# luoao-kddi/SCP

Measured on AMD Instinct MI355X. Metric: KITTI frames/sec encode (SCP-EHEM, level 16) + bpp match vs ref, higher is better.
Workload: dtype f32 (dense layers and attention as bf16x3 split on bf16 MFMA, feature kNN as f16x3 split on f16 MFMA, fp32 accumulate; position kNN / CDF in fp32); 1 GPU; SCP-EHEM KITTI-like synthetic 120k-pt frames, --spher --mullevel lidar_level=16 (BASELINE.json configs[2]), seeded random weights; nodes_per_frame=577403, windows_per_frame=100, frames_per_gpu=46, frames_in_flight=4, frames_per_launch_sequence=1, transform=host-numpy on a prefetch thread (strict identity: the reference's integers), parallelism=frame-sharded x1, rank_cores=256, rank_cores_pinned=False

## Files before the change

### include/scp.h

```cpp
#ifndef SCP_H
#define SCP_H
#include <stddef.h>
#include <stdint.h>

#ifdef __cplusplus
extern "C" {
#endif

#define SCP_API __attribute__((visibility("default")))

#define SCP_OK 0
#define SCP_EINVAL (-1)
#define SCP_ENOMEM (-2)
#define SCP_ESMALL (-3)
#define SCP_EHIP (-4)
#define SCP_ESTATE (-5)

#define SCP_MAX_DEPTH 21
#define SCP_MAX_SEGMENTS 62

#define SCP_ABI_VERSION 220
SCP_API int scp_version(void);
SCP_API int scp_last_hip_error(void);
SCP_API int scp_device_count(void);
// ... 279 lines not shown

enum { SCP_TIE_MEAN_NORMAL = 0, SCP_TIE_PLANE_ERROR = 1 };
SCP_API int scp_estimate_normals_f64(const double *xyz, int64_t n, double radius, int32_t max_nn, const double *view, double *normals,
                                     int32_t *count, int32_t *idx, void *stream);
SCP_API int scp_nn_tieset_f64(int32_t mode, const double *q, int64_t nq, const double *p, int64_t np, const double *dmin, const double *nrm,
                              double *out, void *stream);

#define SCP_DIST_MAX_RINGS 64
#define SCP_DIST_MAX_BINS 4096
#define SCP_DIST_MAX_POINTS (1ll << 30)
enum { SCP_DIST_FLAG_AXIS = 1, SCP_DIST_FLAG_GROUP_CLAMPED = 2, SCP_DIST_FLAG_NO_NEIGHBOUR = 4 };
typedef struct scp_dist_seg {
    int64_t rows, axis_rows;
    double sum_sq, sum_r2, sum_phi2, sum_theta2, sum_r, max_sq;
    int64_t hist[64];
} scp_dist_seg;
SCP_API int scp_nn_error_split_f64(const double *a, int64_t na, const double *b, int64_t nb, const double *view, const double *edges_sq,
                                   int32_t n_rings, const int32_t *group , int32_t n_groups, int32_t *idx_out, double *d2_out,
                                   double *comp_out , int32_t *bin_out, uint8_t *flag_out, void *stream);
SCP_API int scp_dist_segments_f64(const double *d2, const double *comp, const uint8_t *flag, const int64_t *order , int64_t n,
                                  const int64_t *seg_off, int32_t n_bins, scp_dist_seg *out, void *stream);

#define SCP_SHARE_MAX_NODES (1ll << 30)
typedef struct scp_share_seg {
    int64_t leaves;
    double ideal_bits, table_bits, max_ideal_bits;
} scp_share_seg;
SCP_API int64_t scp_rate_leaf_share_workspace_bytes(int64_t total_nodes, int32_t nseg);
SCP_API int scp_rate_leaf_share(const uint8_t *occ, const uint8_t *level, const int32_t *parent, int64_t total_nodes, const double *bits_ideal,
                                const double *bits_table, const int64_t *segs , int32_t nseg, int64_t total_leaves,
                                int64_t *leaves, double *cost_ideal, double *cost_table, void *workspace, int64_t workspace_bytes, void *stream);
SCP_API int scp_ring_bins_f64(const double *xyz, int64_t n, const double *view, const double *edges_sq, int32_t n_rings,
                              const int32_t *group , int32_t n_groups, int32_t *bin_out, uint8_t *flag_out , void *stream);
SCP_API int scp_share_segments_f64(const double *cost_ideal, const double *cost_table, const int64_t *order , int64_t n,
                                   const int64_t *seg_off, int32_t n_bins, scp_share_seg *out, void *stream);

SCP_API int64_t scp_rate_depth_share_workspace_bytes(int64_t total_nodes, int32_t nseg);
SCP_API int scp_rate_depth_share(const uint8_t *occ, const uint8_t *level, const int32_t *parent, int64_t total_nodes, const double *bits_ideal,
                                 const double *bits_table, const int64_t *segs , int32_t nseg, int64_t total_leaves,
                                 int32_t max_drop, int64_t *leaves, double *cost_ideal, double *cost_table, void *workspace,
                                 int64_t workspace_bytes, void *stream);
SCP_API int scp_share_segments_depth_f64(const double *cost_ideal, const double *cost_table, const int64_t *order , int64_t n,
                                         const int64_t *seg_off, int32_t n_bins, int32_t n_depths, int64_t plane_stride, scp_share_seg *out,
                                         void *stream);

SCP_API int scp_embed_gather(const uint8_t *ctx, const float *pos, const int64_t *inmap, int64_t n_tokens, const float *occ_enc,
                     const float *level_enc, const float *octant_enc, float *x, float *pos_out, int64_t *occ_self, int64_t rows,
                     void *stream);

SCP_API int scp_packed_plan_sizes(const int64_t *lengths, int32_t W, int64_t *rows_out);
SCP_API int scp_packed_plan(const int64_t *lengths, int32_t W, int64_t *tables_dev, void *const *outs, int32_t n_outs, void *stream);

SCP_API int scp_decode_expand(const int64_t *sym, const int64_t *cum, const int32_t *pos, const uint8_t *anc, const uint8_t *octant, int64_t n,
                              int32_t L, int32_t shift, int32_t lv_next, int32_t lv_clamp, int32_t polar, double mn, double den, int32_t *cpos,
                              uint8_t *canc, uint8_t *coct, uint8_t *cctx, float *cposn, uint8_t *occ8, void *stream);

typedef struct scp_expand_seg {
    int64_t first, count, cfirst, coded;
    int32_t L, shift, lv_next, lv_clamp, polar, reserved;
    double mn, den;
} scp_expand_seg;
SCP_API int scp_decode_expand_batch(const int64_t *sym, const int64_t *cum, const int32_t *pos, const uint8_t *anc, const uint8_t *octant,
                                    int64_t n, const scp_expand_seg *seg, int32_t S, int32_t cs, const int64_t *wbase, int32_t K, int64_t M,
                                    int64_t T, void *table_dev, int32_t *cpos, uint8_t *canc, uint8_t *coct, uint8_t *cctx, float *cposn,
                                    uint8_t *occ8, void *stream);

SCP_API int scp_swin_ln_linear(const float *x, int64_t ldx, const float *valid, const void *Whi, const void *Wlo, const float *bias,
                               const float *wbeta, float eps, float *out, int64_t ldo, int32_t M, int32_t N, void *stream);
SCP_API int scp_swin_post_attn(const void *Ohi, const void *Olo, int64_t ldo_in, const float *x, int64_t ldx, const void *W, const float *bp,
                               const float *b1, const float *b2, float eps, float *out, int64_t ldc, int32_t M, const int32_t *tile_list,
                               int32_t n_tiles, void *stream);
SCP_API int64_t scp_swin_post_attn_weight_bytes(void);
SCP_API double scp_gelu_prescale(void);

SCP_API int scp_swin_merge(const float *x, int64_t ldx, int64_t n_src, const int64_t *ia, const int64_t *ib, const void *W, const float *wbeta,
                           float eps, float *out, int64_t ldo, int32_t M, void *stream);

SCP_API int scp_geo_edge_mlps(const float *pos1, int64_t ld1, const float *pos2, int64_t ld2, const float *pos3, int64_t ld3, const void *W,
                              const float *bias, float *out, int64_t ldo, int32_t M, void *stream);
SCP_API int scp_mlp3_rows(const float *x, int64_t ldx, int64_t n_src, const int64_t *in_map, const void *W, const float *bias, float *out, int64_t ldo,
                          const int64_t *out_map, int32_t M, int32_t N, void *stream);

#define SCP_LDO_FRAG 0
SCP_API int scp_swin_kv_planes(const float *k, const float *v, int64_t ldkv, int64_t rows, void *khi, void *klo, void *vthi, void *vtlo, void *stream);
SCP_API int scp_swin_ln_qkv(const float *x, int64_t ldx, const float *valid, const void *Whi, const void *Wlo, const float *bias, const float *wbeta,
                            float eps, float *q, int64_t ldq, void *planes, int64_t Tp, int32_t M, int32_t N, void *stream);
SCP_API int scp_swin_attention_packed_planes(const float *q, const void *khi, const void *klo, const void *vthi, const void *vtlo,
                                             const float *bias_table, const int32_t *wtab, int32_t total_windows, int32_t shift, int32_t ldq,
                                             float *out, void *ohi, void *olo, int64_t ldo, const float *valid, void *stream);

#ifdef __cplusplus
}
#endif
#endif
```

### scp_amd/build.py

```python
import os
import subprocess
import sys

HERE = os.path.dirname(os.path.abspath(__file__))
CSRC = os.path.join(HERE, "csrc")
LIB = os.path.join(HERE, "libscp_hip.so")
SOURCES = ["api.cpp", "geom.hip", "sort_u64.hip", "cdf.hip", "rangecoder.cpp", "legacy_octree.cpp",
           "knn.hip", "edge.hip", "attn.hip", "octattn.hip", "octattn_f16.hip", "octattn_embed.hip", "octattn_rowinv.hip", "gemm.hip", "gemm_split.hip", "rowchain.hip", "lnlin2.hip", "fused.hip", "metrics.hip", "plan.hip", "normals.hip", "rate.hip", "distreport.hip", "ringrate.hip", "temper.hip", "ringlod.hip", "attr.hip", "color.hip", "ac_chunks.hip"]
HIPCC = os.environ.get("HIPCC", "/opt/rocm/bin/hipcc")
FLAGS = ["-O3", "--offload-arch=gfx950", "-fPIC", "-std=c++17", "-Wall", "-Wno-unused-function",
         "-Wno-unused-result", "-fvisibility=hidden", "-x", "hip"]


EXTRA = {"geom.hip": ["-ffp-contract=off"], "knn.hip": ["-ffp-contract=off"], "cdf.hip": ["-ffp-contract=off"],
         "edge.hip": ["-ffp-contract=off"], "metrics.hip": ["-ffp-contract=off"], "octattn_embed.hip": ["-ffp-contract=off"],
         "octattn_rowinv.hip": ["-ffp-contract=off"], "normals.hip": ["-ffp-contract=off"], "rate.hip": ["-ffp-contract=off"],
         "distreport.hip": ["-ffp-contract=off"], "ringrate.hip": ["-ffp-contract=off"], "temper.hip": ["-ffp-contract=off"]}
if os.environ.get("SCP_ATTN_DEFS"):
    EXTRA["attn.hip"] = os.environ["SCP_ATTN_DEFS"].split()
if os.environ.get("SCP_KNN_DEFS"):
    EXTRA["knn.hip"] = EXTRA["knn.hip"] + os.environ["SCP_KNN_DEFS"].split()
if os.environ.get("SCP_RC_DEFS"):
    EXTRA["rowchain.hip"] = os.environ["SCP_RC_DEFS"].split()
EXTRA["lnlin2.hip"] = EXTRA.get("rowchain.hip", [])


def _stale(target, deps):
    if not os.path.exists(target):
        return True
    t = os.path.getmtime(target)
    return any(os.path.getmtime(d) > t for d in deps)


def build(force=False, verbose=False):
    srcs = [os.path.join(CSRC, s) for s in SOURCES if os.path.exists(os.path.join(CSRC, s))]
    hdrs = [os.path.join(CSRC, f) for f in os.listdir(CSRC) if f.endswith(".h")] + [os.path.join(HERE, "..", "include", "scp.h")]
    objs = []
    os.makedirs(os.path.join(CSRC, "build"), exist_ok=True)
    procs = []
    for s in srcs:
        o = os.path.join(CSRC, "build", os.path.basename(s) + ".o")
        objs.append(o)
        cmd = [HIPCC] + FLAGS + EXTRA.get(os.path.basename(s), []) + ["-c", s, "-o", o]
        stamp, line = o + ".cmd", " ".join(cmd)
        same_cmd = os.path.exists(stamp) and open(stamp).read() == line
        if force or not same_cmd or _stale(o, [s] + hdrs):
            for stale in (stamp, o):
                if os.path.exists(stale):
                    os.remove(stale)
            if verbose:
                print(" ".join(cmd), file=sys.stderr)
            procs.append((s, subprocess.Popen(cmd), stamp, line))
    bad = []
    for s, p, stamp, line in procs:
        if p.wait() != 0:
            bad.append(s)
            continue
        with open(stamp, "w") as f:
            f.write(line)
    if bad:
        raise RuntimeError("hipcc failed for: " + ", ".join(bad))
    if force or procs or _stale(LIB, objs):
        cmd = [HIPCC, "--offload-arch=gfx950", "-shared", "-fPIC", "-o", LIB] + objs
        if verbose:
            print(" ".join(cmd), file=sys.stderr)
        subprocess.check_call(cmd)
    return LIB


if __name__ == "__main__":
    print(build(force="--force" in sys.argv, verbose=True))
```

### scp_amd/csrc/lnlin2.hip

```cpp
#include <stdlib.h>
#include <type_traits>
#include "rc_common.h"

#define L2_Q 16384
#define L2_OFF_BOUNCE (3 * L2_Q)
#define L2_OFF_BIAS (L2_OFF_BOUNCE + 4 * RC_BOUNCE)
#define L2_LDS (L2_OFF_BIAS + 8192)
static_assert(L2_LDS <= 80 * 1024, "two workgroups per CU: at most half of the 160 KiB");
#define L2_LDS_ONE (160 * 1024)

__device__ __forceinline__ void l2_issue(const RcLane &L, __amdgpu_buffer_rsrc_t wr_hi, __amdgpu_buffer_rsrc_t wr_lo, int j, int qt, char *dst) {
#pragma unroll
    for (int i = 0; i < 4; ++i) {
        const int b = i >> 1, plane = i & 1;
        const int soff = ((2 * j + b) * 16 + (L.w >> 1) * 8 + qt * 2 + (L.w & 1)) * 1024;
        __builtin_amdgcn_raw_ptr_buffer_load_lds(plane ? wr_lo : wr_hi, (rc_lds_ptr_t)(dst + (L.w + 4 * i) * 1024), 16, L.lane * 16, soff, 0, 0);
    }
}

#define L2_READ4(d0, d1, d2, d3, addr, o0, o1, o2, o3)                                                                                  \
    asm volatile("ds_read_b128 %0, %4 offset:%5\n\tds_read_b128 %1, %4 offset:%6\n\tds_read_b128 %2, %4 offset:%7\n\t"                      \
                 "ds_read_b128 %3, %4 offset:%8\n\ts_waitcnt lgkmcnt(0)"                                                                  \
                 : "=&v"(d0), "=&v"(d1), "=&v"(d2), "=&v"(d3) : "v"(addr), "n"(o0), "n"(o1), "n"(o2), "n"(o3) : "memory")
#define L2_READ4_AHEAD(d0, d1, d2, d3, addr, o0, o1, o2, o3)                                                                            \
    asm volatile("ds_read_b128 %0, %4 offset:%5\n\tds_read_b128 %1, %4 offset:%6\n\tds_read_b128 %2, %4 offset:%7\n\t"                      \
                 "ds_read_b128 %3, %4 offset:%8"                                                                                         \
                 : "=&v"(d0), "=&v"(d1), "=&v"(d2), "=&v"(d3) : "v"(addr), "n"(o0), "n"(o1), "n"(o2), "n"(o3) : "memory")
#define L2_WAIT4(d0, d1, d2, d3) asm volatile("s_waitcnt lgkmcnt(0)" : "+v"(d0), "+v"(d1), "+v"(d2), "+v"(d3) :: "memory")
#define L2_TOP(N) asm volatile("s_waitcnt vmcnt(" #N ") lgkmcnt(0)\n\ts_barrier" ::: "memory")

template <bool SWAP, int Q>
__device__ __forceinline__ void l2_quarter(unsigned ad0, unsigned ad1, rf32x16 &c0, rf32x16 &c1, const rbf16x8 (&Xh)[16], const rbf16x8 (&Xl)[16]) {
#define L2_MFMA(c, wf, xf) c = SWAP ? __builtin_amdgcn_mfma_f32_32x32x16_bf16(xf, wf, c, 0, 0, 0) : __builtin_amdgcn_mfma_f32_32x32x16_bf16(wf, xf, c, 0, 0, 0)
#define L2_FRAGS(M, A, ad, s) M(A[1], A[3], A[0], A[2], ad, 4096 + ((s) >> 1) * 1024, 12288 + ((s) >> 1) * 1024, ((s) >> 1) * 1024, 8192 + ((s) >> 1) * 1024)
    rbf16x8 A[2][4];
    L2_FRAGS(L2_READ4, A[0], ad0, 0);
#pragma unroll
    for (int s = 0; s < 4; ++s) {
        const int k = 4 * Q + s, n = (s + 1) & 1;
        if (s < 3) {
            if (n) L2_FRAGS(L2_READ4_AHEAD, A[1], ad1, s + 1);
            else L2_FRAGS(L2_READ4_AHEAD, A[0], ad0, s + 1);
        }
        __builtin_amdgcn_sched_barrier(0);
        L2_MFMA(c0, A[s & 1][1], Xh[k]);
        L2_MFMA(c1, A[s & 1][3], Xh[k]);
        L2_MFMA(c0, A[s & 1][0], Xl[k]);
        L2_MFMA(c1, A[s & 1][2], Xl[k]);
        L2_MFMA(c0, A[s & 1][0], Xh[k]);
        L2_MFMA(c1, A[s & 1][2], Xh[k]);
        __builtin_amdgcn_sched_barrier(0);
        if (s < 3) L2_WAIT4(A[n][0], A[n][1], A[n][2], A[n][3]);
    }
#undef L2_FRAGS
#undef L2_MFMA
}

__device__ __forceinline__ unsigned l2_split_pair(float x0, float x1, int plane) {
    const unsigned hh = rc_pack2(x0, x1);
    return plane ? rc_pack2(x0 - __builtin_bit_cast(float, hh << 16), x1 - __builtin_bit_cast(float, hh & 0xffff0000u)) : hh;
}

__device__ __forceinline__ void l2_store_k(const RcLane &L, char *bounce, const rf32x16 &c0, const rf32x16 &c1, __amdgpu_buffer_rsrc_t prs, int kvoff,
                                           int pbytes, int head) {
    ri32x4 y[2][4];
    int col = L.col;
    asm volatile("" : "+v"(col));
#pragma unroll
    for (int plane = 0; plane < 2; ++plane) {
#pragma unroll
        for (int b = 0; b < 2; ++b)
#pragma unroll
            for (int q = 0; q < 4; ++q) {
                const rf32x16 &c = b ? c1 : c0;
                *(ru32x2 *)(bounce + col * 128 + (((4 * b + q) ^ (col & 7)) << 4) + 8 * L.h) =
                    (ru32x2){l2_split_pair(c[4 * q], c[4 * q + 1], plane), l2_split_pair(c[4 * q + 2], c[4 * q + 3], plane)};
            }
#pragma unroll
        for (int it = 0; it < 4; ++it) y[plane][it] = *(const ri32x4 *)(bounce + it * 1024 + L.lane * 16);
    }
#pragma unroll
    for (int plane = 0; plane < 2; ++plane)
#pragma unroll
        for (int it = 0; it < 4; ++it)
            __builtin_amdgcn_raw_buffer_store_b128(y[plane][it], prs, kvoff, it * 8 * 512 + head * 128 + plane * pbytes, 0);
    asm volatile("s_waitcnt lgkmcnt(0)" ::: "memory");
}

__device__ __forceinline__ void l2_store_v(const RcLane &L, char *bounce, const rf32x16 &c0, const rf32x16 &c1, __amdgpu_buffer_rsrc_t prs, int vblk,
                                           int pbytes, int head) {
    ri32x4 y[2][4];
    int col = L.col;
    asm volatile("" : "+v"(col));
#pragma unroll
    for (int plane = 0; plane < 2; ++plane) {
#pragma unroll
        for (int b = 0; b < 2; ++b)
#pragma unroll
            for (int cc = 0; cc < 2; ++cc) {
                const rf32x16 &c = b ? c1 : c0;
                const int d = col + 32 * b, R = d >> 1, sl = (d & 1) * 4 + 2 * cc + L.h;
                *(ru32x4 *)(bounce + R * 128 + ((sl ^ (R & 7)) << 4)) =
                    (ru32x4){l2_split_pair(c[8 * cc], c[8 * cc + 1], plane), l2_split_pair(c[8 * cc + 2], c[8 * cc + 3], plane),
                             l2_split_pair(c[8 * cc + 4], c[8 * cc + 5], plane), l2_split_pair(c[8 * cc + 6], c[8 * cc + 7], plane)};
            }
#pragma unroll
        for (int it = 0; it < 4; ++it) y[plane][it] = *(const ri32x4 *)(bounce + it * 1024 + L.lane * 16);
    }
#pragma unroll
    for (int plane = 0; plane < 2; ++plane)
#pragma unroll
        for (int it = 0; it < 4; ++it)
            __builtin_amdgcn_raw_buffer_store_b128(y[plane][it], prs, L.lane * 16, it * 1024 + (vblk + head) * 4096 + (2 + plane) * pbytes, 0);
    asm volatile("s_waitcnt lgkmcnt(0)" ::: "memory");
}

template <bool KV>
__global__ __launch_bounds__(256, 2) void ln2_proj_kernel(const RcLnLinArgs a) {
    extern __shared__ __attribute__((aligned(1024))) char smem[];
    const RcLane L = rc_lane();
    const int ntiles = (a.M + RC_ROWS - 1) / RC_ROWS;
    const int nsteps = a.N >> 6;
    const int nq = KV ? a.nq : nsteps;
    char *bounce = smem + L2_OFF_BOUNCE + L.w * RC_BOUNCE;
    const unsigned ab = (unsigned)(uintptr_t)(rc_lds_ptr_t)smem + L.rg * 2048;
    const unsigned af0 = ab + L.frag, af1 = ab + (L.frag ^ 32);
    const unsigned asb = (unsigned)(uintptr_t)(rc_lds_ptr_t)(smem + L2_OFF_BIAS);
    const int ldo_bytes = (int)(a.ldo * 4);
    const int voff = (32 * L.w + (L.lane >> 3)) * ldo_bytes + (L.lane & 7) * 16;
    const int pbytes = (int)a.plane_bytes;
    const __amdgpu_buffer_rsrc_t prs = __builtin_amdgcn_make_buffer_rsrc((void *)a.planes, 0, (KV && !(a.probe & 1)) ? (int)(4 * a.plane_bytes) : 0, 0x00020000);
    const bool dma = !(a.probe & 2);

    const int wbytes = ((a.N + 255) & ~255) * 512;
    const __amdgpu_buffer_rsrc_t wr_hi = __builtin_amdgcn_make_buffer_rsrc((void *)a.Whi, 0, wbytes, 0x00020000);
    const __amdgpu_buffer_rsrc_t wr_lo = __builtin_amdgcn_make_buffer_rsrc((void *)a.Wlo, 0, wbytes, 0x00020000);

    float *sb = (float *)(smem + L2_OFF_BIAS), *sbw = sb + 1024;
    for (int i = threadIdx.x; i < a.N; i += 256) {
        const float b = a.bias ? a.bias[i] : 0.f;
        sb[i] = b; sbw[i] = b + (a.wbeta ? a.wbeta[i] : 0.f);
    }
    __syncthreads();
    int slot = 0;
    if (dma) { l2_issue(L, wr_hi, wr_lo, 0, 0, smem); l2_issue(L, wr_hi, wr_lo, 0, 1, smem + L2_Q); }
    for (int tile = blockIdx.x; tile < ntiles; tile += (int)gridDim.x) {
        const int m0 = tile * RC_ROWS;
        const int row = m0 + 32 * L.w + L.col;
        const int rowc = row < a.M ? row : a.M - 1;
        float keep = (row < a.M) ? 1.0f : 0.0f;
        if (a.valid) keep *= a.valid[rowc];
        rbf16x8 Xh[16], Xl[16];
        {
            float v[128];
            const float *src = a.x + (int64_t)((a.probe & 4) ? (rowc & 127) % a.M : rowc) * a.ldx + 8 * L.h;
#pragma unroll
            for (int s = 0; s < 16; ++s) {
                const rf32x4 q0 = *(const rf32x4 *)(src + 16 * s), q1 = *(const rf32x4 *)(src + 16 * s + 4);
#pragma unroll
                for (int u = 0; u < 4; ++u) { v[8 * s + u] = q0[u]; v[8 * s + 4 + u] = q1[u]; }
            }
            float mean, rstd;
            rc_ln_stats(v, a.eps, mean, rstd);
            const float sc = rstd * keep;
#pragma unroll
            for (int s = 0; s < 16; ++s) {
                float f[8];
#pragma unroll
                for (int i = 0; i < 8; ++i) f[i] = (v[8 * s + i] - mean) * sc;
                rc_split8(f, Xh[s], Xl[s]);
            }
        }
        const bool kept = keep != 0.f;
        const int64_t rows_left = (int64_t)a.M - m0;
        const int64_t span = (rows_left < RC_ROWS ? rows_left : RC_ROWS) * a.ldo * 4;
        const __amdgpu_buffer_rsrc_t rs = __builtin_amdgcn_make_buffer_rsrc(a.out + (int64_t)m0 * a.ldo, 0, (a.probe & 1) ? 0 : (int)span, 0x00020000);
        const unsigned kmask = (unsigned)__builtin_amdgcn_ballot_w64(kept);
        const unsigned maskh = kmask >> (4 * L.h);
        const int kvoff = (m0 + 32 * L.w + (L.lane >> 3)) * 512 + (L.lane & 7) * 16;
        const int vblk = ((m0 >> 5) + L.w) * 4;

        const unsigned atb = asb + (kept ? 4096 : 0) + 16 * L.h, atv = asb + 4 * L.col;
        rf32x16 c0, c1;
        auto bias_start = [&](int j) {
            if (KV && j >= nq + 4) {
                float bb[2], bwv[2];
                const unsigned ad = atv + 256 * j;
                asm volatile("ds_read_b32 %0, %4\n\tds_read_b32 %1, %4 offset:128\n\tds_read_b32 %2, %4 offset:4096\n\tds_read_b32 %3, %4 offset:4224\n\t"
                             "s_waitcnt lgkmcnt(0)" : "=&v"(bb[0]), "=&v"(bb[1]), "=&v"(bwv[0]), "=&v"(bwv[1]) : "v"(ad) : "memory");
#pragma unroll
                for (int blk = 0; blk < 2; ++blk) {
                    rf32x16 &c = blk ? c1 : c0;
#pragma unroll
                    for (int r = 0; r < 16; ++r) c[r] = ((maskh >> (8 * (r >> 2) + (r & 3))) & 1u) ? bwv[blk] : bb[blk];
                }
            } else {
                const unsigned ad = atb + 256 * j;
                rf32x4 t[2][4];
                L2_READ4(t[0][0], t[0][1], t[0][2], t[0][3], ad, 0, 32, 64, 96);
                L2_READ4(t[1][0], t[1][1], t[1][2], t[1][3], ad, 128, 160, 192, 224);
#pragma unroll
                for (int q = 0; q < 4; ++q)
#pragma unroll
                    for (int u = 0; u < 4; ++u) { c0[4 * q + u] = t[0][q][u]; c1[4 * q + u] = t[1][q][u]; }
            }
        };
        bias_start(0);
        SCP_WAIT_DMA(0);
        auto steps = [&](auto sw, int ja, int jb) {
        constexpr bool SW = decltype(sw)::value;
        for (int j = ja; j < jb; ++j) {
            const int jn = j + 1 < nsteps ? j + 1 : 0;
#define L2_QUARTER(Q, N)                                                                                                                \
            {                                                                                                                           \
                L2_TOP(N);                                                                                                              \
                const int sl2 = slot == 0 ? 2 : slot - 1;                    \
                if (dma) l2_issue(L, wr_hi, wr_lo, Q < 2 ? j : jn, (Q + 2) & 3, smem + sl2 * L2_Q);                                       \
                __builtin_amdgcn_sched_barrier(0);                                                                                      \
                const unsigned a0 = af0 + slot * L2_Q, a1 = af1 + slot * L2_Q;                                                          \
                l2_quarter<SW, Q>(a0, a1, c0, c1, Xh, Xl);                                                                              \
                slot = slot == 2 ? 0 : slot + 1;                                                                                        \
            }
            L2_QUARTER(0, 12)
            L2_QUARTER(1, 12)
            L2_QUARTER(2, 4)
            L2_QUARTER(3, 4)
#undef L2_QUARTER
            __builtin_amdgcn_sched_barrier(0);
            if (!SW && j < nq) {
#pragma unroll
                for (int blk = 0; blk < 2; ++blk) {
                    rf32x4 o[4];
#pragma unroll
                    for (int q = 0; q < 4; ++q)
#pragma unroll
                        for (int u = 0; u < 4; ++u) o[q][u] = (blk ? c1 : c0)[4 * q + u];
                    rc_store_block(L, bounce, o, rs, ldo_bytes, voff, 64 * j + 32 * blk);
                }
            } else if (!SW) {
                l2_store_k(L, bounce, c0, c1, prs, kvoff, pbytes, j - nq);
            } else {
                l2_store_v(L, bounce, c0, c1, prs, vblk, pbytes, j - nq - 4);
            }
            if (j + 1 < nsteps) bias_start(jn);
        }
        };
        if (KV) { steps(std::false_type(), 0, nq + 4); steps(std::true_type(), nq + 4, nsteps); }
        else steps(std::false_type(), 0, nsteps);
    }
    SCP_WAIT_DMA(0);
}

int scp_lnlin2_mode() {
    static int mode = -1;
    if (mode < 0) { const char *e = getenv("SCP_LNLIN"); mode = e ? atoi(e) : 0; if (mode < 0 || mode > 2) mode = 0; }
    return mode;
}

int scp_lnlin2_launch(RcLnLinArgs a, bool kv, int ncu, hipStream_t stream) {
    static int one = -1, probe = -1;
    if (one < 0) { const char *e = getenv("SCP_LNLIN_ONE"); one = (e && e[0] == '1') ? 1 : 0; }
    if (probe < 0) { const char *e = getenv("SCP_RC_PROBE"); probe = e ? atoi(e) : 0; }
    static bool configured = false;
    if (!configured) {
        HIP_TRY(hipFuncSetAttribute((const void *)ln2_proj_kernel<false>, hipFuncAttributeMaxDynamicSharedMemorySize, one ? L2_LDS_ONE : L2_LDS));
        HIP_TRY(hipFuncSetAttribute((const void *)ln2_proj_kernel<true>, hipFuncAttributeMaxDynamicSharedMemorySize, one ? L2_LDS_ONE : L2_LDS));
        configured = true;
    }
    a.ngroups = 1; a.probe = probe; a.dbg = nullptr;
    const int ntiles = (a.M + RC_ROWS - 1) / RC_ROWS;
    const int wgs = (one ? 1 : 2) * ncu;
    const dim3 grid((unsigned)(ntiles < wgs ? ntiles : wgs));
    if (kv) hipLaunchKernelGGL(ln2_proj_kernel<true>, grid, dim3(256), one ? L2_LDS_ONE : L2_LDS, stream, a);
    else hipLaunchKernelGGL(ln2_proj_kernel<false>, grid, dim3(256), one ? L2_LDS_ONE : L2_LDS, stream, a);
    LAUNCH_CHECK();
    return SCP_OK;
}
```

### scp_amd/csrc/rc_common.h

```cpp
#pragma once
#include "scp_internal.h"

typedef __bf16 rbf16x8 __attribute__((ext_vector_type(8)));
typedef float rf32x16 __attribute__((ext_vector_type(16)));
typedef float rf32x4 __attribute__((ext_vector_type(4)));
typedef int ri32x4 __attribute__((ext_vector_type(4)));
typedef __attribute__((address_space(3))) void *rc_lds_ptr_t;
typedef const __attribute__((address_space(1))) void *rc_glb_ptr_t;

#define RC_ROWS 128
#define RC_BOUNCE 4096

__device__ __forceinline__ void rc_dma16(const void *g, char *l) {
    __builtin_amdgcn_global_load_lds((rc_glb_ptr_t)g, (rc_lds_ptr_t)l, 16, 0, 0);
}

typedef float rf32x2 __attribute__((ext_vector_type(2)));
typedef __bf16 rbf16x2 __attribute__((ext_vector_type(2)));
typedef unsigned ru32x4 __attribute__((ext_vector_type(4)));
typedef unsigned ru32x2 __attribute__((ext_vector_type(2)));
__device__ __forceinline__ unsigned rc_pack2(float a, float b) {
    const rf32x2 v = {a, b};
    return __builtin_bit_cast(unsigned, __builtin_convertvector(v, rbf16x2));
}
__device__ __forceinline__ void rc_split2(float a, float b, unsigned &hi, unsigned &lo) {
    asm volatile("" : "+v"(a), "+v"(b));
    hi = rc_pack2(a, b);
    lo = rc_pack2(a - __builtin_bit_cast(float, hi << 16), b - __builtin_bit_cast(float, hi & 0xffff0000u));
}
__device__ __forceinline__ void rc_split8(const float *f, rbf16x8 &hi, rbf16x8 &lo) {
    ru32x4 h, l;
#pragma unroll
    for (int i = 0; i < 4; ++i) { unsigned a, b; rc_split2(f[2 * i], f[2 * i + 1], a, b); h[i] = a; l[i] = b; }
    hi = __builtin_bit_cast(rbf16x8, h);
    lo = __builtin_bit_cast(rbf16x8, l);
}

struct RcLane {
    int lane, col, h, w;
    int frag;
    int rg;
};

__device__ __forceinline__ RcLane rc_lane() {
    RcLane L;
    const int tid = threadIdx.x;
    L.lane = tid & 63; L.col = L.lane & 31; L.h = L.lane >> 5;
    L.w = __builtin_amdgcn_readfirstlane(tid >> 6);
    L.frag = (L.col & 15) * 64 + ((L.h ^ ((L.col >> 2) & 3)) << 4);
    L.rg = L.col >> 4;
    return L;
}

__device__ __forceinline__ void rc_store_block(const RcLane &L, char *bounce, const rf32x4 v[4], __amdgpu_buffer_rsrc_t rs, int ldo_bytes, int voff,
                                               int ch0) {
#pragma unroll
    for (int q = 0; q < 4; ++q)
        *(rf32x4 *)(bounce + L.col * 128 + (((2 * q + L.h) ^ (L.col & 7)) << 4)) = v[q];
    asm volatile("s_waitcnt lgkmcnt(0)" ::: "memory");
    rf32x4 y[4];
#pragma unroll
    for (int it = 0; it < 4; ++it) {
        const int rho = 8 * it + (L.lane >> 3), kap = L.lane & 7;
        y[it] = *(const rf32x4 *)(bounce + rho * 128 + ((kap ^ (rho & 7)) << 4));
    }
#pragma unroll
    for (int it = 0; it < 4; ++it) __builtin_amdgcn_raw_buffer_store_b128(__builtin_bit_cast(ri32x4, y[it]), rs, voff, it * 8 * ldo_bytes + ch0 * 4, 0);
    asm volatile("s_waitcnt lgkmcnt(0)" ::: "memory");
}

__device__ __forceinline__ void rc_ln_stats(const float *v , float eps, float &mean, float &rstd) {
    float s = 0.f;
#pragma unroll
    for (int i = 0; i < 128; i += 4) s += (v[i] + v[i + 1]) + (v[i + 2] + v[i + 3]);
    s += __shfl_xor(s, 32);
    mean = s * (1.0f / 256.0f);
    float q = 0.f;
#pragma unroll
    for (int i = 0; i < 128; ++i) { const float d = v[i] - mean; q += d * d; }
    q += __shfl_xor(q, 32);
    rstd = rsqrtf(q * (1.0f / 256.0f) + eps);
}

struct RcLnLinArgs {
    const float *x; int64_t ldx;
    const float *valid;
    const __bf16 *Whi, *Wlo;
    const float *bias, *wbeta;
    float *out; int64_t ldo;
    int M, N;
    float eps;
    int probe;
    unsigned long long *dbg;
    __bf16 *planes; int64_t plane_bytes; int nq;
    int ngroups;
};

int scp_lnlin2_mode();
int scp_lnlin2_launch(RcLnLinArgs a, bool kv, int ncu, hipStream_t stream);
```

### scp_amd/csrc/rowchain.hip

```cpp
#include <stdlib.h>
#include "scp_internal.h"
#include "rc_common.h"

#define RC_SLOT 32768
#define RC_RING (4 * RC_SLOT)
#define RC_OFF_BOUNCE RC_RING
#define RC_OFF_BIAS (RC_RING + 4 * RC_BOUNCE)
#define RC_LDS (RC_OFF_BIAS + 16384)

__device__ __forceinline__ void rc_issue_rowchunk(const RcLane &L, const __bf16 *Whi, const __bf16 *Wlo, int g, char *slot) {
#pragma unroll
    for (int j = 0; j < 4; ++j) {
        const int p = L.w + 4 * j;
        const int64_t off = ((int64_t)g * 16 + p) * 512 + L.lane * 8;
        rc_dma16(Whi + off, slot + p * 1024);
        rc_dma16(Wlo + off, slot + 16384 + p * 1024);
    }
}

__device__ __forceinline__ void rc_issue_kchunk(const RcLane &L, const __bf16 *Whi, const __bf16 *Wlo, int c, int nks, char *slot) {
#pragma unroll
    for (int j = 0; j < 4; ++j) {
        const int p = L.w + 4 * j;
        const int64_t off = ((int64_t)p * nks + c) * 512 + L.lane * 8;
// ... 498 lines not shown
    return;
#endif
    switch (st) {
    case 0: g.ea = -ya * ya; g.eb = -yb * yb; break;
    case 1: g.ea = __builtin_amdgcn_exp2f(g.ea); g.eb = __builtin_amdgcn_exp2f(g.eb); break;
    case 2: g.pa = fmaf(SCP_GELU_C4, __builtin_fabsf(ya), SCP_GELU_C3); g.pb = fmaf(SCP_GELU_C4, __builtin_fabsf(yb), SCP_GELU_C3); break;
    case 3: g.pa = fmaf(g.pa, __builtin_fabsf(ya), SCP_GELU_C2); g.pb = fmaf(g.pb, __builtin_fabsf(yb), SCP_GELU_C2); break;
    case 4: g.pa = fmaf(g.pa, __builtin_fabsf(ya), SCP_GELU_C1); g.pb = fmaf(g.pb, __builtin_fabsf(yb), SCP_GELU_C1); break;
    case 5: g.pa = fmaf(g.pa, __builtin_fabsf(ya), SCP_GELU_C0); g.pb = fmaf(g.pb, __builtin_fabsf(yb), SCP_GELU_C0); break;
    case 6: g.pa = __builtin_amdgcn_rcpf(g.pa); g.pb = __builtin_amdgcn_rcpf(g.pb); break;
    case 7: g.wa = __builtin_fabsf(ya) * g.ea; g.wb = __builtin_fabsf(yb) * g.eb; break;
    case 8: asm("v_max_f32_e32 %0, 0, %1" : "=v"(g.xa) : "v"(ya)); asm("v_max_f32_e32 %0, 0, %1" : "=v"(g.xb) : "v"(yb)); break;
    case 9: g.ga = fmaf(-g.wa, g.pa, g.xa); g.gb = fmaf(-g.wb, g.pb, g.xb); break;
    case 10: g.hw = rc_pack2(g.ga, g.gb); wh = g.hw; break;
    default: wl = rc_pack2(g.ga - __builtin_bit_cast(float, g.hw << 16), g.gb - __builtin_bit_cast(float, g.hw & 0xffff0000u)); break;
    }
    switch (st) {
    case 0: case 1: asm volatile("" : "+v"(g.ea), "+v"(g.eb)); break;
    case 2: case 3: case 4: case 5: case 6: asm volatile("" : "+v"(g.pa), "+v"(g.pb)); break;
    case 7: asm volatile("" : "+v"(g.wa), "+v"(g.wb)); break;
    case 8: asm volatile("" : "+v"(g.xa), "+v"(g.xb)); break;
    case 9: asm volatile("" : "+v"(g.ga), "+v"(g.gb)); break;
    case 10: asm volatile("" : "+v"(g.ga), "+v"(g.gb), "+v"(g.hw)); break;
    default: break;
    }
}

template <bool HAS_P1, bool HAS_GELU, int NEXT>
__device__ __forceinline__ void rc_body_step(const RcLane &L, char *smem, int half, rf32x16 (&Y)[8], rf32x16 &a1n, const rf32x16 &a1g,
                                             const ru32x4 (&Hch)[2], const ru32x4 (&Hcl)[2], ru32x4 (&Hnh)[2],
                                             ru32x4 (&Hnl)[2], const rbf16x8 (&Xh)[16], const rbf16x8 (&Xl)[16], rbf16x8 (&A)[2][4],
                                             __amdgpu_buffer_rsrc_t wr, const RcSlotSrc &n0, const RcSlotSrc &n1) {
    const RcFragAddr f = rc_frag_addr(L, smem + half * (2 * RC_SLOT)), fn = rc_frag_addr(L, smem + (half ^ 1) * (2 * RC_SLOT));
    char *nxt = smem + (half ^ 1) * (2 * RC_SLOT);
    RcGelu g;
#pragma unroll
    for (int s = 0; s < 16; ++s) {
        if (s == 15) RC_STEP_BARRIER("vmcnt(0) lgkmcnt(0)", L.w);
        RC_SB;
        const int nb = (s + 1) & 1, ns = (s + 1) & 15;
        const int blk = s >> 1, t = s & 1;
#pragma unroll
        for (int gap = 0; gap < 6; ++gap) {
            if (HAS_P1 && gap < 4 && RC_PROBE_FRAG_ON) { RC_FRAG_WAIT(); RC_SB; }
            if (!HAS_P1 && (gap == 1 || gap == 3) && RC_PROBE_FRAG_ON) { asm volatile("s_waitcnt lgkmcnt(1)" ::: "memory"); RC_SB; }
            if (gap == 0 && HAS_P1) RC_MFMA_AVA(a1n, A[s & 1][1], Xh[s]);
            if (gap == 1) RC_MFMA_AVV(Y[blk], A[s & 1][3], Hch[t]);
            if (gap == 2 && HAS_P1) RC_MFMA_AVV(a1n, A[s & 1][0], Xl[s]);
            if (gap == 3) RC_MFMA_AVV(Y[blk], A[s & 1][2], Hcl[t]);
            if (gap == 4 && HAS_P1) RC_MFMA_AVA(a1n, A[s & 1][0], Xh[s]);
            if (gap == 5) RC_MFMA_AVV(Y[blk], A[s & 1][2], Hch[t]);
            RC_SB;
            if (s < 15 && RC_PROBE_FRAG_ON) {
                if (gap == 0 && HAS_P1) RC_DS_READ(A[nb][1], (ns & 1) ? f.r1 : f.r0, 16384 + (ns >> 1) * 1024);
                if (gap == 1) RC_DS_READ(A[nb][3], (ns & 1) ? f.k1 : f.k0, RC_SLOT + 16384 + (ns >> 1) * 2048);
                if (gap == 2 && HAS_P1) RC_DS_READ(A[nb][0], (ns & 1) ? f.r1 : f.r0, (ns >> 1) * 1024);
                if (gap == 3) RC_DS_READ(A[nb][2], (ns & 1) ? f.k1 : f.k0, RC_SLOT + (ns >> 1) * 2048);
            }
            if (RC_DMA_HERE(s, gap) && RC_PROBE_DMA_ON) rc_dma_piece(L, wr, RC_DMA_SLOT(s, gap) ? n1 : n0, nxt + RC_DMA_SLOT(s, gap) * RC_SLOT, RC_DMA_IDX(s, gap), RC_DMA_PLANE(s, gap));
            if (HAS_GELU) {
                const int k = s >> 1, st = (s & 1) * 6 + gap;
                unsigned wh = 0, wl = 0;
                rc_gelu_stage(st, g, a1g[2 * k], a1g[2 * k + 1], wh, wl);
                if (st == 10) Hnh[k >> 2][k & 3] = wh;
                if (st == 11) Hnl[k >> 2][k & 3] = wl;
            }
            RC_SB;
        }
    }
    if (NEXT == 0) RC_DS_READ4_WAIT(A[0][1], fn.r0, 16384, A[0][3], fn.k0, RC_SLOT + 16384, A[0][0], fn.r0, 0, A[0][2], fn.k0, RC_SLOT);
    else RC_DS_READ4_WAIT(A[0][1], fn.r0, 16384, A[0][3], fn.r0, RC_SLOT + 16384, A[0][0], fn.r0, 0, A[0][2], fn.r0, RC_SLOT);
}

__device__ __forceinline__ void rc_load_o_frag(const __bf16 *Ohi, const __bf16 *Olo, int tile, int r, int h, rbf16x8 (&Bh)[16], rbf16x8 (&Bl)[16]) {
    const __amdgpu_buffer_rsrc_t rh = __builtin_amdgcn_make_buffer_rsrc((void *)(Ohi + (int64_t)tile * (RC_ROWS * 256)), 0, RC_ROWS * 512, 0x00020000);
    const __amdgpu_buffer_rsrc_t rl = __builtin_amdgcn_make_buffer_rsrc((void *)(Olo + (int64_t)tile * (RC_ROWS * 256)), 0, RC_ROWS * 512, 0x00020000);
    const int v = (r & (RC_ROWS - 1)) * 16 + h * 2048;
#pragma unroll
    for (int s = 0; s < 16; ++s) Bh[s] = __builtin_bit_cast(rbf16x8, __builtin_amdgcn_raw_buffer_load_b128(rh, v, 4096 * s, 0));
#pragma unroll
    for (int s = 0; s < 16; ++s) Bl[s] = __builtin_bit_cast(rbf16x8, __builtin_amdgcn_raw_buffer_load_b128(rl, v, 4096 * s, 0));
}

template <bool OFRAG>
__global__ __launch_bounds__(256, 1) void rc_post_attn_kernel(const RcPostArgs a) {
    extern __shared__ __attribute__((aligned(1024))) char smem[];
    const RcLane L = rc_lane();
    const int ntiles = (a.M + RC_ROWS - 1) / RC_ROWS;
    float *sbp = (float *)(smem + RC_OFF_BIAS), *sb2 = sbp + 256, *sb1 = sbp + 512;
    for (int i = threadIdx.x; i < 256; i += 256) { sbp[i] = a.bp[i]; sb2[i] = a.b2[i]; }
    for (int i = threadIdx.x; i < 1024; i += 256) sb1[i] = a.b1[i];
    __syncthreads();
    const int nlist = a.tile_list ? a.n_list : ntiles;
    auto tile_of = [&](int i) { return a.tile_list ? a.tile_list[i] : i; };
    int ti = blockIdx.x;
    if (ti >= nlist) return;
    int tile = tile_of(ti);
    char *bounce = smem + RC_OFF_BOUNCE + L.w * RC_BOUNCE;
    const int ldc_bytes = (int)(a.ldc * 4);
    const int voff = (32 * L.w + (L.lane >> 3)) * ldc_bytes + (L.lane & 7) * 16;

    const __amdgpu_buffer_rsrc_t wr = __builtin_amdgcn_make_buffer_rsrc((void *)a.W, 0, 2 * RC_W_PLANE, 0x00020000);
    auto src_p = [&](int g) { RcSlotSrc r = {RC_W_PROJ + g * 16384, 1024}; return r; };
    auto src_1 = [&](int c) { RcSlotSrc r = {RC_W_FC1 + c * 16384, 1024}; return r; };
    auto src_2 = [&](int c) { RcSlotSrc r = {RC_W_FC2 + c * 1024, 32 * 1024}; return r; };

    unsigned long long t_p0 = 0, t_ln = 0, t_mlp = 0, t_epi = 0, t_prev = 0, n_tiles = 0;
    const bool DBG = a.dbg != nullptr;
    unsigned long long t_first = 0, r_first = 0;
    if (DBG) { t_prev = t_first = __builtin_amdgcn_s_memtime(); r_first = __builtin_amdgcn_s_memrealtime(); }
    auto stamp = [&](unsigned long long &acc_t) { if (DBG) { const unsigned long long t = __builtin_amdgcn_s_memtime(); acc_t += t - t_prev; t_prev = t; } };

    {
        const RcSlotSrc s0 = src_p(0), s1 = src_p(1);
#pragma unroll
        for (int q = 0; q < 4; ++q)
#pragma unroll
            for (int plane = 0; plane < 2; ++plane) { rc_dma_piece(L, wr, s0, smem, q, plane); rc_dma_piece(L, wr, s1, smem + RC_SLOT, q, plane); }
    }
    rbf16x8 Bh[16], Bl[16];
    auto load_o = [&](int t) {
        if (OFRAG) {
            const int r = t * RC_ROWS + 32 * L.w + L.col;
            rc_load_o_frag(a.Ohi, a.Olo, t, r < a.M ? r : a.M - 1, L.h, Bh, Bl);
            return;
        }
        const int r0 = t * RC_ROWS + 32 * L.w + (L.lane >> 3);
#pragma unroll
        for (int it = 0; it < 4; ++it) {
            const int r = r0 + 8 * it;
            const int64_t o = (int64_t)(r < a.M ? r : a.M - 1) * a.ldo_in + (L.lane & 7) * 8;
#pragma unroll
            for (int pp = 0; pp < 4; ++pp) { Bh[4 * pp + it] = *(const rbf16x8 *)(a.Ohi + o + 64 * pp); Bl[4 * pp + it] = *(const rbf16x8 *)(a.Olo + o + 64 * pp); }
        }
    };
    auto transpose_o = [&]() {
        if (OFRAG) {
#pragma unroll
            for (int s = 0; s < 16; ++s) asm volatile("" : "+v"(Bh[s]), "+v"(Bl[s]));
            return;
        }
#pragma unroll
        for (int plane = 0; plane < 2; ++plane)
#pragma unroll
            for (int pp = 0; pp < 4; ++pp) {
#pragma unroll
                for (int it = 0; it < 4; ++it) {
                    const int rho = 8 * it + (L.lane >> 3), kap = L.lane & 7;
                    *(rbf16x8 *)(bounce + rho * 128 + ((kap ^ (rho & 7)) << 4)) = plane ? Bl[4 * pp + it] : Bh[4 * pp + it];
                }
                asm volatile("s_waitcnt lgkmcnt(0)" ::: "memory");
#pragma unroll
                for (int q = 0; q < 4; ++q) {
                    const rbf16x8 fr = *(const rbf16x8 *)(bounce + L.col * 128 + (((2 * q + L.h) ^ (L.col & 7)) << 4));
                    if (plane) Bl[4 * pp + q] = fr; else Bh[4 * pp + q] = fr;
                }
                asm volatile("s_waitcnt lgkmcnt(0)" ::: "memory");
            }
    };
    load_o(tile);
    transpose_o();
    rbf16x8 A[2][4];
    {
        SCP_BARRIER_DMA(0);
        const RcFragAddr f = rc_frag_addr(L, smem);
        RC_DS_READ4_WAIT(A[0][1], f.r0, 16384, A[0][3], f.r0, RC_SLOT + 16384, A[0][0], f.r0, 0, A[0][2], f.r0, RC_SLOT);
    }
    int gstep = 0;
    for (; ti < nlist; ti += gridDim.x) {
        tile = tile_of(ti);
        const int m0 = tile * RC_ROWS;
        const bool more = ti + (int)gridDim.x < nlist;
        const int tile_next = more ? tile_of(ti + (int)gridDim.x) : tile;
        rf32x16 Y[8];
        const int xrow = m0 + 32 * L.w + (L.lane >> 3);
        const float *xsrc = a.x + (L.lane & 7) * 4;
        for (int j = 0; j < 4; ++j) {
            rf32x4 xc[2][4];
#pragma unroll
            for (int b = 0; b < 2; ++b)
#pragma unroll
                for (int it = 0; it < 4; ++it) {
                    const int r = xrow + 8 * it;
                    xc[b][it] = *(const rf32x4 *)(xsrc + (int64_t)(r < a.M ? r : a.M - 1) * a.ldx + 64 * j + 32 * b);
                }
            rf32x16 c0, c1;
#pragma unroll
            for (int r = 0; r < 16; ++r) { c0[r] = 0.f; c1[r] = 0.f; }
            rc_gemm_step<false>(L, smem, gstep & 1, c0, c1, Bh, Bl, A, wr, j < 3 ? src_p(2 * j + 2) : src_1(0), j < 3 ? src_p(2 * j + 3) : src_1(1));
            ++gstep;
#pragma unroll
            for (int b = 0; b < 2; ++b) {
#pragma unroll
                for (int it = 0; it < 4; ++it) {
                    const int rho = 8 * it + (L.lane >> 3), kap = L.lane & 7;
                    *(rf32x4 *)(bounce + rho * 128 + ((kap ^ (rho & 7)) << 4)) = xc[b][it];
                }
                asm volatile("s_waitcnt lgkmcnt(0)" ::: "memory");
#pragma unroll
                for (int q = 0; q < 4; ++q) {
                    const rf32x4 xq = *(const rf32x4 *)(bounce + L.col * 128 + (((2 * q + L.h) ^ (L.col & 7)) << 4));
                    const rf32x4 bq = *(const rf32x4 *)(sbp + 64 * j + 32 * b + 8 * q + 4 * L.h);
#pragma unroll
                    for (int u = 0; u < 4; ++u) {
                        if (b == 0) c0[4 * q + u] += xq[u] + bq[u];
                        else c1[4 * q + u] += xq[u] + bq[u];
                    }
                }
                asm volatile("s_waitcnt lgkmcnt(0)" ::: "memory");
            }
            asm volatile("s_waitcnt lgkmcnt(0)" ::: "memory");
            switch (j) {
            case 0: Y[0] = c0; Y[1] = c1; break;
            case 1: Y[2] = c0; Y[3] = c1; break;
            case 2: Y[4] = c0; Y[5] = c1; break;
            default: Y[6] = c0; Y[7] = c1; break;
            }
        }
        stamp(t_p0);
        float sum = 0.f;
#pragma unroll
        for (int b = 0; b < 8; ++b)
#pragma unroll
            for (int r = 0; r < 16; r += 4) sum += (Y[b][r] + Y[b][r + 1]) + (Y[b][r + 2] + Y[b][r + 3]);
        sum += __shfl_xor(sum, 32);
        const float mean = sum * (1.0f / 256.0f);
        float sq = 0.f;
#pragma unroll
        for (int b = 0; b < 8; ++b)
#pragma unroll
            for (int r = 0; r < 16; ++r) { const float d = Y[b][r] - mean; sq += d * d; }
        sq += __shfl_xor(sq, 32);
        const float rstd = rsqrtf(sq * (1.0f / 256.0f) + a.eps);
#pragma unroll
        for (int b = 0; b < 8; ++b) {
#pragma unroll
            for (int t = 0; t < 2; ++t) {
                float fr[8];
#pragma unroll
                for (int i = 0; i < 8; ++i) fr[i] = (Y[b][8 * t + i] - mean) * rstd;
                rc_split8(fr, Bh[2 * b + t], Bl[2 * b + t]);
            }
#pragma unroll
            for (int q = 0; q < 4; ++q) {
                const rf32x4 bb = *(const rf32x4 *)(sb2 + 32 * b + 8 * q + 4 * L.h);
#pragma unroll
                for (int u = 0; u < 4; ++u) Y[b][4 * q + u] += bb[u];
            }
        }
        asm volatile("s_waitcnt lgkmcnt(0)" ::: "memory");
        stamp(t_ln);
        if (a.dbg_mode) {
#pragma unroll
            for (int b = 0; b < 8; ++b)
#pragma unroll
                for (int r = 0; r < 16; ++r) {
                    const int t = r >> 3, i = r & 7;
                    Y[b][r] = (a.dbg_mode == 1) ? (float)Bh[2 * b + t][i] + (float)Bl[2 * b + t][i] : (r == 0 ? mean : rstd);
                }
        }
        rf32x16 a1[2];
        auto bias_into = [&](rf32x16 &acc, int c) {
#pragma unroll
            for (int q = 0; q < 4; ++q) {
                const rf32x4 bq = *(const rf32x4 *)(sb1 + 32 * c + 8 * q + 4 * L.h);
#pragma unroll
                for (int u = 0; u < 4; ++u) acc[4 * q + u] = bq[u];
            }
        };
        bias_into(a1[0], 0);
        bias_into(a1[1], 1);
        asm volatile("s_waitcnt lgkmcnt(0)" ::: "memory");
        if (!a.dbg_mode) {
        rc_gemm_step<true>(L, smem, gstep & 1, a1[0], a1[1], Bh, Bl, A, wr, src_1(2), src_2(0)); ++gstep;
        ru32x4 Hh[1][2], Hl[1][2];
        {
            RcGelu g;
#pragma unroll
            for (int k = 0; k < 8; ++k)
#pragma unroll
                for (int st = 0; st < 12; ++st)
                {
                    unsigned wh = 0, wl = 0;
                    rc_gelu_stage(st, g, a1[0][2 * k], a1[0][2 * k + 1], wh, wl);
                    if (st == 10) Hh[0][k >> 2][k & 3] = wh;
                    if (st == 11) Hl[0][k >> 2][k & 3] = wl;
                }
        }
        ru32x4 Hnh[2], Hnl[2];
        for (int c = 0; c < 30; ++c) {
            rf32x16 a1n;
            bias_into(a1n, c + 2);
            asm volatile("s_waitcnt lgkmcnt(0)" ::: "memory");
            rc_body_step<true, true, 0>(L, smem, gstep & 1, Y, a1n, a1[1], Hh[0], Hl[0], Hnh, Hnl, Bh, Bl, A, wr,
                                        c + 3 < 32 ? src_1(c + 3) : src_2(c + 1), src_2(c + 1));
            ++gstep;
            a1[1] = a1n;
#pragma unroll
            for (int t = 0; t < 2; ++t) { Hh[0][t] = Hnh[t]; Hl[0][t] = Hnl[t]; }
        }
        load_o(tile_next);
        rc_body_step<false, true, 0>(L, smem, gstep & 1, Y, a1[0], a1[1], Hh[0], Hl[0], Hnh, Hnl, Bh, Bl, A, wr, src_2(31), src_2(31));
        ++gstep;
        rc_body_step<false, false, 1>(L, smem, gstep & 1, Y, a1[0], a1[1], Hnh, Hnl, Hh[0], Hl[0], Bh, Bl, A, wr, src_p(0), src_p(1));
        ++gstep;
        }
        stamp(t_mlp);
        asm volatile("s_waitcnt lgkmcnt(0)" ::: "memory");
        const int64_t rows_left = (int64_t)a.M - m0;
        const int64_t span = (rows_left < RC_ROWS ? rows_left : RC_ROWS) * a.ldc * 4;
#ifdef RC_EPI_NOSTORE
        const __amdgpu_buffer_rsrc_t rs = __builtin_amdgcn_make_buffer_rsrc(a.out, 0, 0, 0x00020000);
#else
        const __amdgpu_buffer_rsrc_t rs = __builtin_amdgcn_make_buffer_rsrc(a.out + (int64_t)m0 * a.ldc, 0, (int)span, 0x00020000);
#endif
#pragma unroll
        for (int b = 0; b < 8; ++b) {
            rf32x4 o[4];
#pragma unroll
            for (int q = 0; q < 4; ++q)
#pragma unroll
                for (int u = 0; u < 4; ++u) o[q][u] = Y[b][4 * q + u];
            rc_store_block(L, bounce, o, rs, ldc_bytes, voff, 32 * b);
        }
        transpose_o();
        stamp(t_epi);
        ++n_tiles;
    }
    if (DBG && L.lane == 0) {
        unsigned long long *o = a.dbg + ((size_t)blockIdx.x * 4 + L.w) * 8;
        o[0] = t_p0; o[1] = t_mlp; o[2] = t_ln; o[3] = t_epi; o[4] = n_tiles;
        o[5] = __builtin_amdgcn_s_memtime() - t_first; o[6] = __builtin_amdgcn_s_memrealtime() - r_first;
    }
    SCP_WAIT_DMA(0);
}

#ifndef RCW_D1
#define RCW_D1 4
#endif
#ifndef RCW_D2
#define RCW_D2 2
#endif
#define RCW_H_BYTES (32 * 4096)
template <bool OFRAG>
__global__ __launch_bounds__(256, 1) void rc_post_attn_wide_kernel(const RcPostArgs a) {
    extern __shared__ __attribute__((aligned(1024))) char smem[];
    const RcLane L = rc_lane();
    float *sbp = (float *)(smem + RC_OFF_BIAS), *sb2 = sbp + 256, *sb1 = sbp + 512;
    for (int i = threadIdx.x; i < 256; i += 256) { sbp[i] = a.bp[i]; sb2[i] = a.b2[i]; }
    for (int i = threadIdx.x; i < 1024; i += 256) sb1[i] = a.b1[i];
    __syncthreads();
    const int n128 = a.tile_list ? a.n_list : (a.M + RC_ROWS - 1) / RC_ROWS;
    char *bounce = smem + RC_OFF_BOUNCE + L.w * RC_BOUNCE;
    char *hbuf = smem;
    const int ldc_bytes = (int)(a.ldc * 4);
    const int voff = (L.lane >> 3) * ldc_bytes + (L.lane & 7) * 16;
    const __amdgpu_buffer_rsrc_t wr = __builtin_amdgcn_make_buffer_rsrc((void *)a.W, 0, 2 * RC_W_PLANE, 0x00020000);
    const int vrc0 = L.rg * 8192 + L.frag, vrc1 = L.rg * 8192 + (L.frag ^ 32);
    const int vkc0 = L.rg * 32768 + L.frag, vkc1 = L.rg * 32768 + (L.frag ^ 32);
    auto wload = [&](int voff, int soff) { return __builtin_bit_cast(rbf16x8, __builtin_amdgcn_raw_buffer_load_b128(wr, voff, soff, 0)); };
    for (int item = blockIdx.x; item < 4 * n128; item += gridDim.x) {
        const int t128 = a.tile_list ? a.tile_list[item >> 2] : (item >> 2);
        const int m0 = t128 * RC_ROWS + 32 * (item & 3);
        if (m0 >= a.M) continue;
        rbf16x8 Bh[16], Bl[16];
        if (OFRAG) {
            const int r = m0 + L.col;
            rc_load_o_frag(a.Ohi, a.Olo, t128, r < a.M ? r : a.M - 1, L.h, Bh, Bl);
        } else {
            const int r0 = m0 + (L.lane >> 3);
#pragma unroll
            for (int it = 0; it < 4; ++it) {
                const int r = r0 + 8 * it;
                const int64_t o = (int64_t)(r < a.M ? r : a.M - 1) * a.ldo_in + (L.lane & 7) * 8;
#pragma unroll
                for (int pp = 0; pp < 4; ++pp) { Bh[4 * pp + it] = *(const rbf16x8 *)(a.Ohi + o + 64 * pp); Bl[4 * pp + it] = *(const rbf16x8 *)(a.Olo + o + 64 * pp); }
            }
#pragma unroll
            for (int plane = 0; plane < 2; ++plane)
#pragma unroll
                for (int pp = 0; pp < 4; ++pp) {
#pragma unroll
                    for (int it = 0; it < 4; ++it) {
                        const int rho = 8 * it + (L.lane >> 3), kap = L.lane & 7;
                        *(rbf16x8 *)(bounce + rho * 128 + ((kap ^ (rho & 7)) << 4)) = plane ? Bl[4 * pp + it] : Bh[4 * pp + it];
                    }
                    asm volatile("s_waitcnt lgkmcnt(0)" ::: "memory");
#pragma unroll
                    for (int q = 0; q < 4; ++q) {
                        const rbf16x8 fr = *(const rbf16x8 *)(bounce + L.col * 128 + (((2 * q + L.h) ^ (L.col & 7)) << 4));
                        if (plane) Bl[4 * pp + q] = fr; else Bh[4 * pp + q] = fr;
                    }
                    asm volatile("s_waitcnt lgkmcnt(0)" ::: "memory");
                }
        }
        rf32x16 c0, c1;
#pragma unroll
        for (int r = 0; r < 16; ++r) { c0[r] = 0.f; c1[r] = 0.f; }
        {
            const int w0 = RC_W_PROJ + (2 * L.w) * 16384, w1 = w0 + 16384;
            constexpr int D = RCW_D1;
            rbf16x8 F[D][4];
            auto fetch = [&](int s, rbf16x8 (&d)[4]) {
                const int v = (s & 1) ? vrc1 : vrc0, o = (s >> 1) * 1024;
                d[0] = wload(v, w0 + o); d[1] = wload(v, w0 + RC_W_PLANE + o);
                d[2] = wload(v, w1 + o); d[3] = wload(v, w1 + RC_W_PLANE + o);
// ... 501 lines not shown
        to_frags();
        RC_LAYER3(1)
        to_frags();
        const int kap = L.lane & 7;
        float *orow[4];
#pragma unroll
        for (int it = 0; it < 4; ++it) {
            const int r = m0 + 32 * L.w + 8 * it + (L.lane >> 3);
            const int64_t o = r < a.M ? (a.out_map ? a.out_map[r] : (int64_t)r) : -1;
            orow[it] = o >= 0 ? a.out + o * a.ldo + 4 * kap : nullptr;
        }
        auto store_block = [&](const rf32x16 &c, int ch0) {
#pragma unroll
            for (int q = 0; q < 4; ++q) {
                rf32x4 v;
#pragma unroll
                for (int u = 0; u < 4; ++u) v[u] = c[4 * q + u];
                *(rf32x4 *)(bounce + L.col * 128 + (((2 * q + L.h) ^ (L.col & 7)) << 4)) = v;
            }
            asm volatile("s_waitcnt lgkmcnt(0)" ::: "memory");
            rf32x4 y[4];
#pragma unroll
            for (int it = 0; it < 4; ++it) {
                const int rho = 8 * it + (L.lane >> 3);
                y[it] = *(const rf32x4 *)(bounce + rho * 128 + ((kap ^ (rho & 7)) << 4));
            }
            asm volatile("s_waitcnt lgkmcnt(0)" ::: "memory");
#pragma unroll
            for (int it = 0; it < 4; ++it)
                if (orow[it] && ch0 + 4 * kap < a.N) *(rf32x4 *)(orow[it] + ch0) = y[it];
        };
        for (int g = 0; g < 4; ++g) {
            RC_BIAS3(2)
            RC_STEP3()
            store_block(c0, 64 * g);
            store_block(c1, 64 * g + 32);
        }
#undef RC_LAYER3
#undef RC_BIAS3
#undef RC_STEP3
    }
    SCP_WAIT_DMA(0);
}

extern "C" SCP_API double scp_gelu_prescale(void) { return (double)SCP_GELU_S; }

static int rc_ll_groups(int ntiles, int nsteps, int ncu) {
    static int on = -1;
    if (on < 0) { const char *e = getenv("SCP_RC_GROUPS"); on = (e && e[0] == '0') ? 0 : 1; }
    int best = 1;
    if (on)
        for (int g = 2; g <= nsteps / 2; ++g)
            if ((nsteps / 2) % g == 0 && (int64_t)ntiles * g <= ncu) best = g;
    return best;
}

static unsigned long long *g_rc_dbg = nullptr;
extern "C" SCP_API int scp_rc_debug_buffer(unsigned long long *dev_buf) { g_rc_dbg = dev_buf; return SCP_OK; }

static int g_rc_num_cu = 0, g_rc_grid = 0;
static int g_rc_wide = -2;
static int rc_wide_mode() {
    if (g_rc_wide == -2) { const char *e = getenv("SCP_RC_WIDE"); g_rc_wide = e ? atoi(e) : -1; if (g_rc_wide < -1 || g_rc_wide > 1) g_rc_wide = -1; }
    return g_rc_wide;
}
extern "C" SCP_API int scp_rc_set_wide(int32_t mode) { g_rc_wide = (mode < -1 || mode > 1) ? -1 : mode; return SCP_OK; }
extern "C" SCP_API int scp_rc_set_grid(int32_t workgroups) { g_rc_grid = workgroups > 0 ? workgroups : 0; return SCP_OK; }
static int rc_num_cu() {
    if (g_rc_grid) return g_rc_grid;
    if (!g_rc_num_cu) {
        int dev = 0;
        hipDeviceProp_t p;
        if (hipGetDevice(&dev) != hipSuccess || hipGetDeviceProperties(&p, dev) != hipSuccess) return 256;
        g_rc_num_cu = p.multiProcessorCount > 0 ? p.multiProcessorCount : 256;
    }
    return g_rc_num_cu;
}

static bool rc_lnlin2_here(int ntiles, int ncu) {
    const int mode = scp_lnlin2_mode();
    return mode == 2 || (mode == 0 && 4 * (int64_t)ntiles >= 3 * (int64_t)ncu);
}

extern "C" SCP_API int scp_swin_ln_linear(const float *x, int64_t ldx, const float *valid, const void *Whi, const void *Wlo, const float *bias,
                                          const float *wbeta, float eps, float *out, int64_t ldo, int32_t M, int32_t N, void *stream) {
    if (!x || !Whi || !Wlo || !out || M <= 0 || N <= 0 || (N & 127) || N > 1024 || ldx < 256 || (ldx & 3) || ldo < N || (ldo & 3) ||
        (((uintptr_t)x | (uintptr_t)out | (uintptr_t)Whi | (uintptr_t)Wlo) & 15) || (int64_t)RC_ROWS * ldo * 4 > 0x7fffffffLL)
        return SCP_EINVAL;
    static bool configured = false;
    if (!configured) {
        HIP_TRY(hipFuncSetAttribute((const void *)rc_ln_linear_kernel<0>, hipFuncAttributeMaxDynamicSharedMemorySize, RC_LDS));
        configured = true;
    }
    RcLnLinArgs a;
    a.x = x; a.ldx = ldx; a.valid = valid; a.Whi = (const __bf16 *)Whi; a.Wlo = (const __bf16 *)Wlo; a.bias = bias; a.wbeta = wbeta;
    a.out = out; a.ldo = ldo; a.M = M; a.N = N; a.eps = eps;
    a.planes = nullptr; a.plane_bytes = 0; a.nq = 0;
    { static int pr = -1; if (pr < 0) { const char *e = getenv("SCP_RC_PROBE"); pr = e ? atoi(e) : 0; } a.probe = pr; }
    if (a.probe) { const char *e = getenv("SCP_RC_PROBE"); a.probe = e ? atoi(e) : 0; }
    a.dbg = g_rc_dbg;
    const int ntiles = (M + RC_ROWS - 1) / RC_ROWS;
    const int ncu = rc_num_cu();
    SCP_PROF(SCP_PROF_LN_LINEAR, stream, 2.0 * M * 256.0 * N);
    if (rc_lnlin2_here(ntiles, ncu)) return scp_lnlin2_launch(a, false, ncu, (hipStream_t)stream);
    a.ngroups = rc_ll_groups(ntiles, N / 64, ncu);
    hipLaunchKernelGGL(rc_ln_linear_kernel<0>, dim3((unsigned)(a.ngroups > 1 ? ntiles * a.ngroups : (ntiles < ncu ? ntiles : ncu))), dim3(256), RC_LDS, (hipStream_t)stream, a);
    LAUNCH_CHECK();
    return SCP_OK;
}

extern "C" SCP_API int scp_swin_ln_qkv(const float *x, int64_t ldx, const float *valid, const void *Whi, const void *Wlo, const float *bias,
                                       const float *wbeta, float eps, float *q, int64_t ldq, void *planes, int64_t Tp, int32_t M, int32_t N, void *stream) {
    if (!x || !Whi || !Wlo || !planes || M <= 0 || (M & 127) || (N != 768 && N != 512) || (N == 768 && (!q || ldq < 256 || (ldq & 3))) || ldx < 256 ||
        (ldx & 3) || Tp < M || (Tp & 31) || (((uintptr_t)x | (uintptr_t)q | (uintptr_t)Whi | (uintptr_t)Wlo | (uintptr_t)planes) & 15) ||
        (q && (int64_t)RC_ROWS * ldq * 4 > 0x7fffffffLL) || 4 * Tp * 512 > 0x7fffffffLL)
        return SCP_EINVAL;
    static bool configured = false;
    if (!configured) {
        HIP_TRY(hipFuncSetAttribute((const void *)rc_ln_linear_kernel<0, true>, hipFuncAttributeMaxDynamicSharedMemorySize, RC_LDS));
        configured = true;
    }
    RcLnLinArgs a;
    a.x = x; a.ldx = ldx; a.valid = valid; a.Whi = (const __bf16 *)Whi; a.Wlo = (const __bf16 *)Wlo; a.bias = bias; a.wbeta = wbeta;
    a.out = q; a.ldo = q ? ldq : 256; a.M = M; a.N = N; a.eps = eps; a.probe = 0; a.dbg = nullptr;
    a.planes = (__bf16 *)planes; a.plane_bytes = Tp * 512; a.nq = N / 64 - 8;
    const int ntiles = M / RC_ROWS, ncu = rc_num_cu();
    SCP_PROF(SCP_PROF_LN_LINEAR, stream, 2.0 * M * 256.0 * N);
    if (rc_lnlin2_here(ntiles, ncu)) return scp_lnlin2_launch(a, true, ncu, (hipStream_t)stream);
    a.ngroups = rc_ll_groups(ntiles, N / 64, ncu);
    hipLaunchKernelGGL((rc_ln_linear_kernel<0, true>), dim3((unsigned)(a.ngroups > 1 ? ntiles * a.ngroups : (ntiles < ncu ? ntiles : ncu))), dim3(256), RC_LDS, (hipStream_t)stream, a);
    LAUNCH_CHECK();
    return SCP_OK;
}

extern "C" SCP_API int scp_swin_post_attn(const void *Ohi, const void *Olo, int64_t ldo_in, const float *x, int64_t ldx, const void *W, const float *bp,
                                          const float *b1, const float *b2, float eps, float *out, int64_t ldc, int32_t M, const int32_t *tile_list,
                                          int32_t n_tiles, void *stream) {
    if (!Ohi || !Olo || !x || !W || !bp || !b1 || !b2 || !out || M <= 0 || (tile_list && (n_tiles <= 0 || n_tiles > (M + RC_ROWS - 1) / RC_ROWS)) || (ldo_in != SCP_LDO_FRAG && (ldo_in < 256 || (ldo_in & 7))) || ldx < 256 || (ldx & 3) || ldc < 256 ||
        (ldc & 3) || (((uintptr_t)Ohi | (uintptr_t)Olo | (uintptr_t)x | (uintptr_t)out | (uintptr_t)W) & 15) ||
        (int64_t)RC_ROWS * ldc * 4 > 0x7fffffffLL)
        return SCP_EINVAL;
    static bool configured = false;
    if (!configured) {
        HIP_TRY(hipFuncSetAttribute((const void *)rc_post_attn_kernel<true>, hipFuncAttributeMaxDynamicSharedMemorySize, RC_LDS));
        HIP_TRY(hipFuncSetAttribute((const void *)rc_post_attn_kernel<false>, hipFuncAttributeMaxDynamicSharedMemorySize, RC_LDS));
        HIP_TRY(hipFuncSetAttribute((const void *)rc_post_attn_wide_kernel<true>, hipFuncAttributeMaxDynamicSharedMemorySize, RC_LDS));
        HIP_TRY(hipFuncSetAttribute((const void *)rc_post_attn_wide_kernel<false>, hipFuncAttributeMaxDynamicSharedMemorySize, RC_LDS));
        configured = true;
    }
    RcPostArgs a;
    a.Ohi = (const __bf16 *)Ohi; a.Olo = (const __bf16 *)Olo; a.ldo_in = ldo_in; a.x = x; a.ldx = ldx; a.W = W;
    a.bp = bp; a.b1 = b1; a.b2 = b2; a.out = out; a.ldc = ldc; a.M = M; a.eps = eps;
    a.dbg = g_rc_dbg;
    { const char *e = getenv("SCP_RC_DUMP"); a.dbg_mode = e ? atoi(e) : 0; }
    a.tile_list = tile_list; a.n_list = tile_list ? n_tiles : 0;
    const bool frag = ldo_in == SCP_LDO_FRAG;
    const int ntiles = tile_list ? n_tiles : (M + RC_ROWS - 1) / RC_ROWS;
    const int ncu = rc_num_cu();
    SCP_PROF(SCP_PROF_POST_ATTN, stream, 2.0 * (tile_list ? (double)n_tiles * RC_ROWS : (double)M) * (256.0 * 256.0 + 2.0 * 256.0 * 1024.0));
    if (rc_wide_mode() == 1 || (rc_wide_mode() < 0 && !g_rc_dbg && !a.dbg_mode && 4 * (int64_t)ntiles <= (int64_t)ncu)) {
        const int items = 4 * ntiles;
        if (frag) hipLaunchKernelGGL(rc_post_attn_wide_kernel<true>, dim3((unsigned)(items < 2 * ncu ? items : 2 * ncu)), dim3(256), RC_LDS, (hipStream_t)stream, a);
        else hipLaunchKernelGGL(rc_post_attn_wide_kernel<false>, dim3((unsigned)(items < 2 * ncu ? items : 2 * ncu)), dim3(256), RC_LDS, (hipStream_t)stream, a);
        LAUNCH_CHECK();
        return SCP_OK;
    }
    if (frag) hipLaunchKernelGGL(rc_post_attn_kernel<true>, dim3((unsigned)(ntiles < ncu ? ntiles : ncu)), dim3(256), RC_LDS, (hipStream_t)stream, a);
    else hipLaunchKernelGGL(rc_post_attn_kernel<false>, dim3((unsigned)(ntiles < ncu ? ntiles : ncu)), dim3(256), RC_LDS, (hipStream_t)stream, a);
    LAUNCH_CHECK();
    return SCP_OK;
}

extern "C" SCP_API int64_t scp_swin_post_attn_weight_bytes(void) { return 2 * (int64_t)RC_W_PLANE; }

extern "C" SCP_API int scp_geo_edge_mlps(const float *pos1, int64_t ld1, const float *pos2, int64_t ld2, const float *pos3, int64_t ld3, const void *W,
                                         const float *bias, float *out, int64_t ldo, int32_t M, void *stream) {
    if (!pos1 || !pos2 || !pos3 || !W || !bias || !out || M <= 0 || ld1 < 64 || ld2 < 128 || ld3 < 256 || ((ld1 | ld2 | ld3) & 3) || ldo < 128 || (ldo & 3) ||
        (((uintptr_t)pos1 | (uintptr_t)pos2 | (uintptr_t)pos3 | (uintptr_t)out | (uintptr_t)W) & 15) || (int64_t)RC_ROWS * ldo * 4 > 0x7fffffffLL)
        return SCP_EINVAL;
    static bool configured = false;
    if (!configured) {
        HIP_TRY(hipFuncSetAttribute((const void *)rc_edge_mlp_kernel, hipFuncAttributeMaxDynamicSharedMemorySize, RC_LDS));
        configured = true;
    }
    RcEdgeArgs a;
    a.p1 = pos1; a.p2 = pos2; a.p3 = pos3; a.ld1 = ld1; a.ld2 = ld2; a.ld3 = ld3; a.W = W; a.bias = bias; a.out = out; a.ldo = ldo; a.M = M;
    const int ntiles = (M + RC_ROWS - 1) / RC_ROWS, ncu = rc_num_cu();
    SCP_PROF(SCP_PROF_EDGE_MLP, stream, 2.0 * M * (448.0 * 256 + 2.0 * 256 * 256 + 512.0 * 256 + 256.0 * 256 + 256.0 * 128));
    hipLaunchKernelGGL(rc_edge_mlp_kernel, dim3((unsigned)(ntiles < ncu ? ntiles : ncu)), dim3(256), RC_LDS, (hipStream_t)stream, a);
    LAUNCH_CHECK();
    return SCP_OK;
}

extern "C" SCP_API int scp_mlp3_rows(const float *x, int64_t ldx, int64_t n_src, const int64_t *in_map, const void *W, const float *bias, float *out, int64_t ldo,
                                     const int64_t *out_map, int32_t M, int32_t N, void *stream) {
    if (!x || !W || !bias || !out || M <= 0 || n_src <= 0 || N <= 0 || N > 256 || (N & 3) || ldx < 256 || (ldx & 3) || ldo < N || (ldo & 3) ||
        (((uintptr_t)x | (uintptr_t)out | (uintptr_t)W) & 15))
        return SCP_EINVAL;
    static bool configured = false;
    if (!configured) {
        HIP_TRY(hipFuncSetAttribute((const void *)rc_mlp3_kernel, hipFuncAttributeMaxDynamicSharedMemorySize, RC_LDS));
        configured = true;
    }
    RcMlp3Args a;
    a.x = x; a.ldx = ldx; a.in_map = in_map; a.n_src = n_src; a.W = W; a.bias = bias; a.out = out; a.ldo = ldo; a.out_map = out_map; a.M = M; a.N = N;
    const int ntiles = (M + RC_ROWS - 1) / RC_ROWS, ncu = rc_num_cu();
    SCP_PROF(SCP_PROF_MLP3, stream, 2.0 * M * 3.0 * 256.0 * 256.0);
    hipLaunchKernelGGL(rc_mlp3_kernel, dim3((unsigned)(ntiles < ncu ? ntiles : ncu)), dim3(256), RC_LDS, (hipStream_t)stream, a);
    LAUNCH_CHECK();
    return SCP_OK;
}

extern "C" SCP_API int scp_swin_merge(const float *x, int64_t ldx, int64_t n_src, const int64_t *ia, const int64_t *ib, const void *W, const float *wbeta,
                                      float eps, float *out, int64_t ldo, int32_t M, void *stream) {
    if (!x || !ia || !ib || !W || !out || M <= 0 || n_src <= 0 || ldx < 256 || (ldx & 3) || ldo < 256 || (ldo & 3) ||
        (((uintptr_t)x | (uintptr_t)out | (uintptr_t)W) & 15) || (int64_t)RC_ROWS * ldo * 4 > 0x7fffffffLL)
        return SCP_EINVAL;
    static bool configured = false;
    if (!configured) {
        HIP_TRY(hipFuncSetAttribute((const void *)rc_merge_kernel, hipFuncAttributeMaxDynamicSharedMemorySize, RC_LDS));
        configured = true;
    }
    RcMergeArgs a;
    a.x = x; a.ldx = ldx; a.n_src = n_src; a.ia = ia; a.ib = ib; a.W = W; a.wbeta = wbeta; a.out = out; a.ldo = ldo; a.M = M; a.eps = eps;
    const int ntiles = (M + RC_ROWS - 1) / RC_ROWS, ncu = rc_num_cu();
    SCP_PROF(SCP_PROF_MERGE, stream, 2.0 * M * 512.0 * 256.0);
    hipLaunchKernelGGL(rc_merge_kernel, dim3((unsigned)(ntiles < ncu ? ntiles : ncu)), dim3(256), RC_LDS, (hipStream_t)stream, a);
    LAUNCH_CHECK();
    return SCP_OK;
}
```

### scp_amd/models/packed.py

```python
import numpy as np
import torch
import torch.nn.functional as F

from .. import native
from ..ops import linear_s, leaky_mlp3_s, split_cat, linear, layer_norm, leaky_mlp3, _split, derived, frozen_epoch
from .ehem import SHIFT, WINDOW, _edge_conv_packed, qkv_fused


def _ceil512(a):
    return (a + WINDOW - 1) // WINDOW * WINDOW


def _tokens(L):
    wid = torch.repeat_interleave(torch.arange(L.numel(), device=L.device), L)
    first = torch.cumsum(L, 0) - L
    return wid, torch.arange(int(L.sum()), device=L.device) - first[wid]


class StageLayout:

    def __init__(self, L):
        self.L = L
        self.Lp = _ceil512(L)
        self.base = torch.cumsum(self.Lp, 0) - self.Lp
# ... 36 lines not shown
def _concat_map(l0, ls, s):
    m = torch.zeros(l0.rows, dtype=torch.int64, device=l0.L.device)
    m[l0.real_rows] = ls.base[l0.wid] + (l0.t >> s)
    return m


class PackedPlan:

    def __init__(self, lengths, n_self=5, n_cross=4, device=None, use_native=True):
        dev = device if device is not None else torch.device("cuda", torch.cuda.current_device())
        dev = torch.device(dev)
        if use_native and dev.type == "cuda" and n_self == 5 and n_cross == 4:
            self.c = torch.as_tensor(np.asarray(lengths, np.int64))
            self.n_tokens = int(np.asarray(lengths, np.int64).sum())
            self.rows, self.d = native.packed_plan(lengths, dev)
            return
        c = torch.as_tensor(np.asarray(lengths, np.int64), device=dev)
        self.c = c
        e = c + (c & 1)
        self.self_layouts = [StageLayout(e)]
        for _ in range(n_self - 1):
            self.self_layouts.append(StageLayout((self.self_layouts[-1].L + 1) // 2))
        self.cross_layouts = [StageLayout(e // 2)]
        for _ in range(n_cross - 1):
            self.cross_layouts.append(StageLayout((self.cross_layouts[-1].L + 1) // 2))
        P0, Q0 = self.self_layouts[0], self.cross_layouts[0]
        self.n_tokens = int(c.sum())
        inmap = torch.full((P0.rows,), self.n_tokens, dtype=torch.int64, device=dev)
        inmap[P0.row_index(c)] = torch.arange(self.n_tokens, device=dev)
        a1 = torch.zeros(Q0.rows, dtype=torch.int64, device=dev)
        a2 = torch.zeros(Q0.rows, dtype=torch.int64, device=dev)
        a1[Q0.real_rows] = P0.base[Q0.wid] + 2 * Q0.t
        a2[Q0.real_rows] = P0.base[Q0.wid] + 2 * Q0.t + 1
        ne, no = (c + 1) // 2, c // 2
        coded = torch.cumsum(c, 0) - c
        we, te = _tokens(ne)
        wo, to = _tokens(no)
        self.d = dict(
            inmap=inmap, a1map=a1, a2map=a2, even_rows=Q0.row_index(ne), odd_rows=Q0.row_index(no),
            even_dst=coded[we] + te, odd_dst=coded[wo] + ne[wo] + to,
            self_merge=[_merge_maps(self.self_layouts[s], self.self_layouts[s + 1]) for s in range(n_self - 1)],
            cross_merge=[_merge_maps(self.cross_layouts[s], self.cross_layouts[s + 1]) for s in range(n_cross - 1)],
            self_concat=[_concat_map(P0, self.self_layouts[s], s) for s in range(1, n_self)],
            cross_concat=[_concat_map(Q0, self.cross_layouts[s], s) for s in range(1, n_cross)],
            self_tab=[l.table() for l in self.self_layouts], cross_tab=[l.table() for l in self.cross_layouts],
            knn_tab=P0.table(real=True),
            self_valid=[l.valid().contiguous() for l in self.self_layouts], cross_valid=[l.valid().contiguous() for l in self.cross_layouts],
            self_parent=[_concat_map(self.self_layouts[s], self.self_layouts[s + 1], 1) for s in range(n_self - 1)],
            cross_parent=[_concat_map(self.cross_layouts[s], self.cross_layouts[s + 1], 1) for s in range(n_cross - 1)],
            even_out=_out_map(Q0, ne, coded), odd_out=_out_map(Q0, no, coded + ne))


def _rowchain_weights(layer, cross):
    att = layer.attention.self
    lnb, lna = layer.layernorm_before, layer.layernorm_after
    W, b = qkv_fused(layer, cross)
    fc1, fc2, proj = layer.intermediate.dense, layer.output.dense, layer.attention.output.dense
    srcs = [W, b, lnb.weight, lnb.bias, lna.weight, lna.bias, fc1.weight, fc1.bias, fc2.weight, fc2.bias, proj.weight, proj.bias]
    if cross:
        srcs += [att.query.weight, att.query.bias]

    def build():
        out = dict(kv=native.LnFoldedWeight(W, lnb.weight, lnb.bias), b=b,
                   post=native.PostAttnWeights(proj.weight, proj.bias, lna.weight, lna.bias, fc1.weight, fc1.bias, fc2.weight, fc2.bias))
        if cross:
            out["q"] = native.LnFoldedWeight(att.query.weight, lnb.weight, lnb.bias)
        return out
    return derived(layer, "rowchain+" if cross else "rowchain", srcs, build)


def _block_consts(layer, cross):
    ep = frozen_epoch()
    key = "_scp_fast_x" if cross else "_scp_fast"
    fast = layer.__dict__.get(key) if ep else None
    if fast is not None and fast[0] == ep:
        return fast[1:]
    att = layer.attention.self
    out = (_rowchain_weights(layer, cross), att.relative_position_bias_table, (att.query.bias if cross else None), layer.layernorm_before.eps, layer.layernorm_after.eps)
    if ep:
        layer.__dict__[key] = (ep,) + out
    return out


def _swin_layer_rowchain(layer, x, valid, wtab, shift, query=None, tiles=None, q_pre=None):
    cross = query is not None
    w, table, qbias, eps_b, eps_a = _block_consts(layer, cross)
    v1 = None if valid is None else valid.reshape(-1)
    if native.attention_bf16x3():
        if not cross:
            q, kvp = native.swin_ln_qkv(x, w["kv"], w["b"], eps_b, v1)
        else:
            q = q_pre if q_pre is not None else native.swin_ln_linear(query, w["q"], qbias, eps_b, v1)
            _, kvp = native.swin_ln_qkv(x, w["kv"], w["b"], eps_b, v1)
        o = native.swin_attention_packed_planes(q, kvp, table, wtab, shift, split=native.attn_o_split(), valid=v1 if tiles is not None else None)
        if tiles is not None and tiles.shape[0] > 0:
            return native.swin_post_attn(o, x, w["post"], eps_a, out=x, tiles=tiles)
        return native.swin_post_attn(o, x, w["post"], eps_a)
    att, lnb = layer.attention.self, layer.layernorm_before
    if not cross:
        qkv = native.swin_ln_linear(x, w["kv"], w["b"], lnb.eps, v1)
        q, k, v = qkv[:, :256], qkv[:, 256:512], qkv[:, 512:]
    else:
        q = q_pre if q_pre is not None else native.swin_ln_linear(query, w["q"], att.query.bias, lnb.eps, v1)
        kv = native.swin_ln_linear(x, w["kv"], w["b"], lnb.eps, v1)
        k, v = kv[:, :256], kv[:, 256:]
    o = native.swin_attention_packed(q, k, v, att.relative_position_bias_table, wtab, shift, split=True)
    return native.swin_post_attn(o, x, w["post"], layer.layernorm_after.eps)


def _swin_layer(layer, x, valid, wtab, shift, query=None, tiles=None, q_pre=None):
    fc1, fc2 = layer.intermediate.dense, layer.output.dense
    if x.shape[1] != 256 or fc1.weight.shape != (1024, 256) or fc2.weight.shape != (256, 1024):
        raise native.ScpError("EHEM's Swin blocks are 256 wide with a 1024-wide MLP (configs/model/ehem.yaml); other widths are not built")
    return _swin_layer_rowchain(layer, x, valid, wtab, shift, query, tiles, q_pre)


def _merge(m, x, maps):
    ev, od = maps
    if x.shape[1] != 256 or m.reduction.weight.shape != (256, 512) or m.reduction.bias is not None:
        raise native.ScpError("SwinPatchMerging: 2 x 256 -> 256 without bias expected")
    mw = derived(m, "rowchain_merge", [m.reduction.weight, m.norm.weight, m.norm.bias],
                 lambda: native.MergeWeights(m.reduction.weight, m.norm.weight, m.norm.bias))
    return native.swin_merge(x, ev, od, mw, m.norm.eps)


def _encoder(enc, x, valids, tabs, merges, query=None, tiles=None, q_pre=None):
    hs = [x]
    for s, stage in enumerate(enc.layers):
        for b, blk in enumerate(stage.blocks):
            x = _swin_layer(blk, x, valids[s], tabs[s], SHIFT if b % 2 else 0, query, None if tiles is None else tiles[s],
                            None if q_pre is None else q_pre[s][b])
        hs.append(x)
        if s < len(enc.layers) - 1:
            x = _merge(stage.downsample, x, merges[s])
            if query is not None and q_pre is None:
                query = _merge(stage.downsample, query, merges[s])
    return hs


def _concat(hs, cmaps, extra=None):
    n = len(hs) - 1 + (1 if extra is not None else 0)
    out = native.SplitAct.empty(hs[1].shape[0], 256 * n, hs[1].device)
    native.split_rows(hs[1], out=out.cols(0, 256))
    for s in range(1, len(hs) - 1):
        native.split_rows(hs[s + 1], idx=cmaps[s - 1], out=out.cols(256 * s, 256 * (s + 1)))
    if extra is not None:
        k = len(hs) - 1
        native.split_rows(extra[0], idx=extra[1], out=out.cols(256 * k, 256 * (k + 1)))
    return out


HIER = True


FUSE2 = __import__("os").environ.get("SCP_CONCAT_FUSE2", "1")[:1] != "0"


def _concat_layer(lin, hs, parents, extra=None, grand=None, a0_pre=None):
    n = len(hs) - 1
    def build():
        W = lin.weight.detach()
        slabs = [W[:, 256 * s:256 * (s + 1)].contiguous() for s in range(n)]
        if extra is not None:
            slabs[0] = torch.cat((slabs[0], W[:, 256 * n:256 * (n + 1)]), 1).contiguous()
        return slabs
    cache = derived(lin, "slabs+" if extra is not None else "slabs", (lin.weight,), build)
    fused = FUSE2 and n >= 3 and grand is not None and native.WTILE and hs[1].shape[0] % 256 == 0
    z = None
    for s in range(n - 1, 1 if fused else 0, -1):
        z = linear_s(native.split_rows(hs[s + 1]), cache[s], None, residual=z, res_map=None if z is None else parents[s], res_first=z is not None)
    if a0_pre is not None:
        native.split_rows(hs[1], out=a0_pre.cols(0, 256))
        a0 = a0_pre
    else:
        a0 = native.split_rows(hs[1]) if extra is None else split_cat((hs[1], extra))
    if fused:
        return native.linear_split_hier2(a0, _split(cache[0]), native.split_rows(hs[2]), _split(cache[1]), parents[0], lin.bias, native.ACT_LEAKY,
                                         residual=z, res_map=grand)
    return linear_s(a0, cache[0], lin.bias, act="leaky", residual=z, res_map=None if z is None else parents[0], res_first=z is not None,
                    want="split")


def _mlp_over_concat(seq, hs, parents, extra=None, grand=None, a0_pre=None):
    a = _concat_layer(seq[0], hs, parents, extra, grand, a0_pre)
    a = linear_s(a, seq[2].weight, seq[2].bias, act="leaky", want="split")
    return linear_s(a, seq[4].weight, seq[4].bias)


CHAIN_HEADS = __import__("os").environ.get("SCP_HEADS", "chain") != "split"


def _mlp3_weights(owner, name, seq):
    return derived(owner, "mlp3_" + name, [seq[i].weight for i in (0, 2, 4)] + [seq[i].bias for i in (0, 2, 4)], lambda: native.Mlp3Weights(seq))


def _head3(model, name, a, out=None, out_map=None, ncols=None):
    seq = getattr(model, name)
    N = seq[4].weight.shape[0]
    if CHAIN_HEADS:
        if out is None:
            out = torch.empty((a.shape[0], -(-N // 4) * 4), dtype=torch.float32, device=a.device)
        native.mlp3_rows(a, _mlp3_weights(model, name, seq), out, out_map=out_map, ncols=ncols)
        return out[:, :N] if out_map is None else None
    sa = native.split_rows(a)
    if out_map is not None:
        sa = linear_s(sa, seq[0].weight, seq[0].bias, act="leaky", want="split")
        sa = linear_s(sa, seq[2].weight, seq[2].bias, act="leaky", want="split")
        native.linear_split_scatter(sa, _split(seq[4].weight), seq[4].bias, out_map, out)
        return None
    return leaky_mlp3_s(seq, sa, out=out)


def _head_to_table(model, a, out_map, table):
    if CHAIN_HEADS and table.stride(0) < 256:
# ... 116 lines not shown
```

### scp_amd/native.py

```python
import ctypes as C
import os

import numpy as np
import torch

HERE = os.path.dirname(os.path.abspath(__file__))
LIB_PATH = os.path.join(HERE, "libscp_hip.so")
MAX_DEPTH = 21

CART, SPHER, CYLIN = 0, 1, 2
POS_MINMAX, POS_MINMAX_MUL, POS_POW2 = 0, 1, 2
_ERR = {-1: "SCP_EINVAL", -2: "SCP_ENOMEM", -3: "SCP_ESMALL", -4: "SCP_EHIP", -5: "SCP_ESTATE"}


class ScpError(RuntimeError):
    pass


class QuantInfo(C.Structure):
    _fields_ = [("bin_num", C.c_double), ("qs", C.c_double * 3), ("offset", C.c_double * 3),
                ("max_coord", C.c_int32), ("min_coord", C.c_int32)]


class Segment(C.Structure):
    _fields_ = [("point_begin", C.c_int64), ("point_count", C.c_int64), ("path_len", C.c_int32),
                ("path_bits", C.c_int32), ("drop_last", C.c_int32), ("reserved", C.c_int32)]


class SegmentInfo(C.Structure):
    _fields_ = [("depth", C.c_int32), ("max_coord", C.c_int32), ("n_leaves", C.c_int64), ("n_nodes", C.c_int64),
                ("node_base", C.c_int64), ("level_count", C.c_int64 * (MAX_DEPTH + 1))]


_lib = None
_vp = C.c_void_p


ABI_VERSION = 220


def lib():
    global _lib
    if _lib is not None:
        return _lib
    if not os.path.exists(LIB_PATH):
        raise ScpError(f"{LIB_PATH} is missing: run `python scp_amd/build.py` (hipcc, gfx950). "
                       "The SCP hot path has no CPU fallback.")
    L = C.CDLL(LIB_PATH)
    i32, i64 = C.c_int32, C.c_int64
    sig = {
        "scp_version": (C.c_int, []),
        "scp_geo_edge_mlps": (C.c_int, [_vp, i64, _vp, i64, _vp, i64, _vp, _vp, _vp, i64, i32, _vp]),
        "scp_mlp3_rows": (C.c_int, [_vp, i64, i64, _vp, _vp, _vp, _vp, i64, _vp, i32, i32, _vp]),
        "scp_swin_merge": (C.c_int, [_vp, i64, i64, _vp, _vp, _vp, _vp, C.c_float, _vp, i64, i32, _vp]),
        "scp_swin_ln_qkv": (C.c_int, [_vp, i64, _vp, _vp, _vp, _vp, _vp, C.c_float, _vp, i64, _vp, i64, i32, i32, _vp]),
        "scp_swin_kv_planes": (C.c_int, [_vp, _vp, i64, i64, _vp, _vp, _vp, _vp, _vp]),
        "scp_swin_attention_packed_planes": (C.c_int, [_vp, _vp, _vp, _vp, _vp, _vp, _vp, i32, i32, i32, _vp, _vp, _vp, i64, _vp, _vp]),
        "scp_split_rows_f16": (C.c_int, [_vp, i64, i32, i32, _vp, _vp, i64, _vp, _vp, _vp]),
        "scp_linear_split_f16": (C.c_int, [_vp, _vp, i64, _vp, _vp, _vp, _vp, i32, i32, _vp, _vp, i64, _vp, i64, i32, i32, i32, i32, i32, _vp]),
        "scp_last_hip_error": (C.c_int, []),
        "scp_device_count": (C.c_int, []),
        "scp_device_name": (C.c_int, [C.c_char_p, C.c_int]),
        "scp_quantize": (C.c_int, [_vp, i64, i32, C.c_double, C.c_double, _vp, _vp, C.POINTER(QuantInfo), _vp]),
        "scp_geom_create": (C.c_int, [C.POINTER(_vp)]),
        "scp_geom_destroy": (C.c_int, [_vp]),
        "scp_geom_build": (C.c_int, [_vp, _vp, i64, C.POINTER(Segment), i32, C.POINTER(SegmentInfo), _vp]),
        "scp_geom_build_xyz": (C.c_int, [_vp, _vp, _vp, i32, i32, _vp, i32, C.c_double, C.POINTER(Segment), _vp, C.POINTER(QuantInfo),
                                         C.POINTER(SegmentInfo), _vp]),
        "scp_geom_context_ehem_all": (C.c_int, [_vp, i32, i32, i32, _vp, _vp, _vp, _vp, _vp]),
        "scp_geom_emit_nodes": (C.c_int, [_vp, _vp, _vp, _vp, _vp, _vp, _vp]),
        "scp_geom_emit_leaves": (C.c_int, [_vp, i32, _vp, _vp]),
        "scp_geom_krecords_i64": (C.c_int, [_vp, i32, _vp, _vp]),
        "scp_geom_context_ehem": (C.c_int, [_vp, i32, i32, i32, _vp, _vp, _vp, _vp, _vp]),
        "scp_geom_context_octattn": (C.c_int, [_vp, i32, _vp, _vp, _vp, _vp]),
        "scp_knn_topk": (C.c_int, [_vp, i32, i32, i32, i32, _vp, _vp]),
        "scp_knn_topk_packed": (C.c_int, [_vp, _vp, i32, i32, _vp, _vp]),
        "scp_knn_topk_packed_bounded": (C.c_int, [_vp, _vp, i32, i32, _vp, _vp, _vp]),
        "scp_swin_attention_packed": (C.c_int, [_vp, _vp, _vp, _vp, _vp, i32, i32, i32, i32, _vp, _vp]),
        "scp_swin_attention_packed_split": (C.c_int, [_vp, _vp, _vp, _vp, _vp, i32, i32, i32, i32, _vp, _vp, i64, _vp]),
        "scp_set_attention_mode": (C.c_int, [i32]),
        "scp_set_attention_variant": (C.c_int, [i32]),
        "scp_get_attention_variant": (C.c_int, []),
        "scp_ctx_create": (C.c_int, [C.POINTER(_vp)]),
        "scp_ctx_destroy": (C.c_int, [_vp]),
        "scp_ctx_set": (C.c_int, [_vp, i32, i32]),
        "scp_ctx_get": (C.c_int, [_vp, i32]),
        "scp_ctx_make_current": (C.c_int, [_vp]),
        "scp_rc_debug_buffer": (C.c_int, [_vp]),
        "scp_rc_set_wide": (C.c_int, [i32]),
        "scp_prof_enable": (C.c_int, [i32]),
        "scp_prof_count": (C.c_int, []),
        "scp_prof_read": (C.c_int, [i32, _vp, _vp, _vp]),
        "scp_set_knn_mode": (C.c_int, [i32]),
        "scp_row_scale_f16": (C.c_int, [_vp, i64, i32, i32, _vp, _vp, _vp]),
        "scp_row_scale_from_max": (C.c_int, [_vp, i32, _vp, _vp, _vp]),
        "scp_linear_split_f16_max": (C.c_int, [_vp, _vp, i64, _vp, _vp, _vp, _vp, i32, i32, _vp, _vp, i64, _vp, i64, i32, i32, i32, i32, i32, _vp, _vp, i32, i32, i32, _vp]),
        "scp_octattn_attention_f16x3_vmax": (C.c_int, [_vp, _vp, _vp, _vp, _vp, i64, i32, i32, i32, i32, _vp, _vp, _vp, i64, _vp, _vp]),
        "scp_linear_f16x3_scaled": (C.c_int, [_vp, i64, _vp, _vp, _vp, i32, _vp, _vp, i64, _vp, i64, i32, i32, i32, i32, _vp, _vp, _vp]),
        "scp_layernorm_add": (C.c_int, [_vp, _vp, i64, i32, _vp, _vp, C.c_float, _vp, _vp]),
        "scp_layernorm_add_split_f16": (C.c_int, [_vp, _vp, i64, i32, _vp, _vp, C.c_float, _vp, _vp, _vp, i64, _vp, _vp, _vp]),
        "scp_set_knn_workgroup": (C.c_int, [i32]),
        "scp_knn_debug_buffer": (C.c_int, [_vp]),
        "scp_nn_sqdist_f64": (C.c_int, [_vp, i64, _vp, i64, _vp, _vp]),
        "scp_estimate_normals_f64": (C.c_int, [_vp, i64, C.c_double, i32, _vp, _vp, _vp, _vp, _vp]),
        "scp_nn_tieset_f64": (C.c_int, [i32, _vp, i64, _vp, i64, _vp, _vp, _vp, _vp]),
        "scp_edge_gather_max_ld": (C.c_int, [_vp, i64, _vp, i64, _vp, _vp, _vp, i32, i32, i32, i32, _vp, i32, _vp]),
        "scp_embed_gather": (C.c_int, [_vp, _vp, _vp, i64, _vp, _vp, _vp, _vp, _vp, _vp, i64, _vp]),
        "scp_packed_plan_sizes": (C.c_int, [_vp, i32, _vp]),
        "scp_packed_plan": (C.c_int, [_vp, i32, _vp, _vp, i32, _vp]),
        "scp_decode_expand": (C.c_int, [_vp, _vp, _vp, _vp, _vp, i64, i32, i32, i32, i32, i32, C.c_double, C.c_double, _vp, _vp, _vp, _vp, _vp, _vp, _vp]),
        "scp_edge_gather_max": (C.c_int, [_vp, _vp, _vp, _vp, _vp, i32, i32, i32, i32, _vp, i32, _vp]),
        "scp_swin_attention": (C.c_int, [_vp, _vp, _vp, _vp, i32, i32, i32, i32, i32, _vp, _vp]),
        "scp_octattn_attention": (C.c_int, [_vp, _vp, _vp, _vp, _vp, i32, i32, i32, i32, _vp, _vp, _vp]),
        "scp_octattn_f16x3_ws_bytes": (C.c_int64, [i32, i32, i32]),
        "scp_octattn_embed": (C.c_int, [_vp, _vp, i64, i32, _vp, i32, _vp, i32, i32, _vp, i32, _vp, _vp, i32, _vp, i32, _vp, _vp, _vp, i64, _vp, _vp, _vp]),
        "scp_octattn_attention_f16x3": (C.c_int, [_vp, _vp, _vp, _vp, _vp, i64, i32, i32, i32, i32, _vp, _vp, _vp, i64, _vp]),
        "scp_octattn_attention_rowinv": (C.c_int, [_vp, i64, i64, _vp, _vp, i64, i64, _vp, _vp, i64, i64, _vp, _vp, i64, i64, i32, i32, i32, i32, i32,
                                                   i32, _vp]),
        "scp_octattn_attention_rowinv_step": (C.c_int, [_vp, i64, _vp, _vp, i64, i64, i32, i32, _vp, _vp, i64, _vp, _vp, i64, _vp, _vp, i32, i32, i32,
                                                        _vp]),
        "scp_decode_expand_octattn": (C.c_int, [_vp, _vp, _vp, _vp, i64, i32, i32, i32, _vp, _vp, _vp, _vp, _vp]),
        "scp_decode_expand_batch": (C.c_int, [_vp, _vp, _vp, _vp, _vp, i64, _vp, i32, i32, _vp, i32, i64, i64, _vp, _vp, _vp, _vp, _vp, _vp, _vp, _vp]),
        "scp_split_weight_bf16": (C.c_int, [_vp, i32, i32, i32, i32, _vp, _vp, _vp]),
        "scp_linear_bf16x3": (C.c_int, [_vp, i64, _vp, _vp, i32, _vp, _vp, i64, _vp, i64, i32, i32, i32, i32, _vp]),
        "scp_split_weight_f16": (C.c_int, [_vp, i32, i32, i32, i32, _vp, _vp, _vp, _vp]),
        "scp_linear_f16x3": (C.c_int, [_vp, i64, _vp, _vp, _vp, i32, _vp, _vp, i64, _vp, i64, i32, i32, i32, i32, _vp, _vp]),
        "scp_linear_split": (C.c_int, [_vp, _vp, i64, _vp, _vp, i32, i32, _vp, _vp, i64, _vp, i64, _vp, _vp, i64, i32, i32, i32, i32, i32, _vp]),
        "scp_tile_weight_bf16": (C.c_int, [_vp, i32, i32, _vp, _vp]),
        "scp_swin_ln_linear": (C.c_int, [_vp, i64, _vp, _vp, _vp, _vp, _vp, C.c_float, _vp, i64, i32, i32, _vp]),
        "scp_swin_post_attn": (C.c_int, [_vp, _vp, i64, _vp, i64, _vp, _vp, _vp, _vp, C.c_float, _vp, i64, i32, _vp, i32, _vp]),
        "scp_swin_post_attn_weight_bytes": (C.c_int64, []),
        "scp_gelu_prescale": (C.c_double, []),
        "scp_split_rows": (C.c_int, [_vp, i64, i64, _vp, i32, _vp, _vp, i64, i64, _vp]),
        "scp_linear_split_scatter": (C.c_int, [_vp, _vp, i64, _vp, _vp, i32, i32, _vp, _vp, _vp, i64, i32, i32, i32, i32, i32, _vp]),
        "scp_linear_split_gather": (C.c_int, [_vp, _vp, i64, _vp, _vp, i32, i32, _vp, _vp, i64, _vp, _vp, i64, _vp, _vp, i64, i32, i32, i32, i32, i32, _vp]),
        "scp_linear_split_hier2": (C.c_int, [_vp, _vp, i64, i32, _vp, _vp, i64, i64, _vp, _vp, _vp, _vp, i32, _vp, _vp, _vp, i64, _vp, _vp, _vp, i64, i32, i32, i32, _vp]),
        "scp_layernorm_rows": (C.c_int, [_vp, i64, i64, _vp, _vp, i32, _vp, _vp, _vp, C.c_float, _vp, i64, i64, _vp]),
        "scp_layernorm_rows_split": (C.c_int, [_vp, i64, i64, _vp, _vp, i32, _vp, _vp, _vp, C.c_float, _vp, _vp, i64, i64, _vp]),
        "scp_gather_rows": (C.c_int, [_vp, i64, _vp, i32, _vp, i64, i64, _vp]),
        "scp_linear_f32": (C.c_int, [_vp, i64, _vp, _vp, _vp, i64, i32, i32, i32, i32, _vp]),
        "scp_softmax_cdf": (C.c_int, [_vp, i64, i64, i32, _vp, _vp, _vp, _vp, _vp]),
        "scp_pmf_cdf": (C.c_int, [_vp, i64, i32, _vp, _vp, _vp, _vp]),
        "scp_rate_workspace_bytes": (C.c_int64, [i64, i32]),
        "scp_rate_segments": (C.c_int, [_vp, i64, i64, i32, _vp, _vp, _vp, i32, _vp, _vp, _vp, _vp, i64, _vp]),
        "scp_temper_workspace_bytes": (C.c_int64, [i64, i32, i32]),
        "scp_temper_sweep": (C.c_int, [_vp, i64, i64, i32, _vp, _vp, i32, _vp, i32, _vp, _vp, _vp, _vp, i64, _vp]),
        "scp_temper_choose": (C.c_int, [_vp, _vp, _vp, i64, _vp, i32, i32, _vp, i32, i32, C.c_double, _vp, _vp, _vp, _vp]),
        "scp_scale_rows": (C.c_int, [_vp, i64, _vp, i64, i64, i32, _vp, _vp, i32, _vp]),
        "scp_ringlod_workspace_bytes": (C.c_int64, [i32, i32]),
        "scp_ringlod_cells": (C.c_int, [_vp, i64, i32, _vp, _vp, i32, _vp, _vp, i32, i32, _vp, _vp, _vp, i64, _vp]),
        "scp_force_rows": (C.c_int, [_vp, i64, i64, i32, _vp, _vp, _vp, _vp]),
        "scp_nn_error_split_f64": (C.c_int, [_vp, i64, _vp, i64, _vp, _vp, i32, _vp, i32, _vp, _vp, _vp, _vp, _vp, _vp]),
        "scp_dist_segments_f64": (C.c_int, [_vp, _vp, _vp, _vp, i64, _vp, i32, _vp, _vp]),
        "scp_rate_leaf_share_workspace_bytes": (C.c_int64, [i64, i32]),
        "scp_rate_leaf_share": (C.c_int, [_vp, _vp, _vp, i64, _vp, _vp, _vp, i32, i64, _vp, _vp, _vp, _vp, i64, _vp]),
        "scp_ring_bins_f64": (C.c_int, [_vp, i64, _vp, _vp, i32, _vp, i32, _vp, _vp, _vp]),
        "scp_share_segments_f64": (C.c_int, [_vp, _vp, _vp, i64, _vp, i32, _vp, _vp]),
        "scp_rate_depth_share_workspace_bytes": (C.c_int64, [i64, i32]),
        "scp_rate_depth_share": (C.c_int, [_vp, _vp, _vp, i64, _vp, _vp, _vp, i32, i64, i32, _vp, _vp, _vp, _vp, i64, _vp]),
        "scp_share_segments_depth_f64": (C.c_int, [_vp, _vp, _vp, i64, _vp, i32, i32, i64, _vp, _vp]),
        "scp_ac_encode_cdf": (C.c_int, [_vp, _vp, i64, i32, _vp, C.c_size_t, C.POINTER(C.c_size_t)]),
        "scp_ac_encode_lohi": (C.c_int, [_vp, i64, _vp, C.c_size_t, C.POINTER(C.c_size_t)]),
        "scp_ac_dec_new": (C.c_int, [C.POINTER(_vp), _vp, C.c_size_t, i32]),
        "scp_ac_dec_next": (C.c_int, [_vp, _vp]),
        "scp_ac_dec_run": (C.c_int, [_vp, _vp, i64, _vp]),
        "scp_ac_dec_free": (C.c_int, [_vp]),
        "scp_ac_dec_run_ctx": (C.c_int, [_vp, _vp, i32, _vp, i64, _vp]),
        "scp_attr_leaf_values_workspace_bytes": (C.c_int64, [i64]),
        "scp_attr_forward_workspace_bytes": (C.c_int64, [i64, i32]),
        "scp_attr_inverse_workspace_bytes": (C.c_int64, [i64, i32]),
        "scp_attr_leaf_values": (C.c_int, [_vp, _vp, i64, _vp, i64, i32, i32, _vp, _vp, _vp, i64, _vp]),
        "scp_attr_forward": (C.c_int, [_vp, _vp, i64, i32, i32, _vp, _vp, _vp, _vp, _vp, _vp, i64, _vp]),
# ... 231 lines not shown
def knn_topk_packed(x, ctab, thr0=None):
    T, Cc = x.shape
    idx = torch.zeros((T, 20), dtype=torch.int32, device=x.device)
    if thr0 is None:
        _check(lib().scp_knn_topk_packed(_dev(x, torch.float32), _dev(ctab, torch.int32), T, Cc, _dev(idx), _stream()), "scp_knn_topk_packed")
    else:
        _check(lib().scp_knn_topk_packed_bounded(_dev(x, torch.float32), _dev(ctab, torch.int32), T, Cc, _dev(thr0, torch.float32), _dev(idx),
                                                 _stream()), "scp_knn_topk_packed_bounded")
    return idx


def swin_attention_packed(q, k, v, bias_table, wtab, shift, split=False):
    T = q.shape[0]
    if split:
        o = SplitAct.empty(T, 256, q.device)
        rc = lib().scp_swin_attention_packed_split(q.data_ptr(), k.data_ptr(), v.data_ptr(), _dev(bias_table, torch.float32),
                                                   _dev(wtab, torch.int32), T // 512, shift, q.stride(0), k.stride(0), o.t[0].data_ptr(),
                                                   o.t[1].data_ptr(), o.t.stride(1), _stream())
        _check(rc, "scp_swin_attention_packed_split")
        return o
    out = torch.empty((T, 256), dtype=torch.float32, device=q.device)
    rc = lib().scp_swin_attention_packed(q.data_ptr(), k.data_ptr(), v.data_ptr(), _dev(bias_table, torch.float32),
                                         _dev(wtab, torch.int32), T // 512, shift, q.stride(0), k.stride(0), _dev(out), _stream())
    _check(rc, "scp_swin_attention_packed")
    return out


class KvPlanes:

    __slots__ = ("t",)

    def __init__(self, k=None, v=None, t=None):
        if t is None:
            T = k.shape[0]
            t = torch.empty((4, T, 256), dtype=torch.bfloat16, device=k.device)
            _check(lib().scp_swin_kv_planes(k.data_ptr(), v.data_ptr(), k.stride(0), T, t[0].data_ptr(), t[1].data_ptr(), t[2].data_ptr(),
                                            t[3].data_ptr(), _stream()), "scp_swin_kv_planes")
        self.t = t


_ATTN_O = "rows" if os.environ.get("SCP_ATTN_O", "")[:1] == "r" else "frag"
LDO_FRAG = 0


def set_attn_o(mode):
    global _ATTN_O
    if mode not in ("frag", "rows"):
        raise ScpError("attention output hand-over: 'frag' or 'rows'")
    prev, _ATTN_O = _ATTN_O, mode
    return prev


def attn_o_split():
    return "frag" if _ATTN_O == "frag" else True


class FragAct:

    __slots__ = ("t", "M", "K")

    def __init__(self, t, M):
        self.t, self.M, self.K = t, M, 256

    @staticmethod
    def empty(M, device):
        return FragAct(torch.empty((2, -(-M // 128), 32, 128, 8), dtype=torch.bfloat16, device=device), M)

    @staticmethod
    def from_rows(a):
        M = a.M
        nt = -(-M // 128)
        r = torch.zeros((2, nt * 128, 256), dtype=torch.bfloat16, device=a.t.device)
        r[:, :M] = a.t[:, :, :256]
        return FragAct(r.view(2, nt, 128, 32, 8).permute(0, 1, 3, 2, 4).contiguous(), M)

    def rows(self):
        nt = self.t.shape[1]
        return SplitAct(self.t.permute(0, 1, 3, 2, 4).reshape(2, nt * 128, 256)[:, :self.M].contiguous(), 256)

    def float(self):
        return self.rows().float()


def swin_attention_packed_planes(q, kv, bias_table, wtab, shift, split=False, valid=None):
    T = q.shape[0]
    p = kv.t
    vp = None if valid is None else _dev(valid, torch.float32)
    if isinstance(split, str):
        if split != "frag":
            raise ScpError("swin_attention_packed_planes: split is False, True or 'frag'")
        o = FragAct.empty(T, q.device)
        rc = lib().scp_swin_attention_packed_planes(q.data_ptr(), p[0].data_ptr(), p[1].data_ptr(), p[2].data_ptr(), p[3].data_ptr(),
                                                    _dev(bias_table, torch.float32), _dev(wtab, torch.int32), T // 512, shift, q.stride(0), None,
                                                    o.t[0].data_ptr(), o.t[1].data_ptr(), LDO_FRAG, vp, _stream())
        _check(rc, "scp_swin_attention_packed_planes")
        return o
    if split:
        o = SplitAct.empty(T, 256, q.device)
        rc = lib().scp_swin_attention_packed_planes(q.data_ptr(), p[0].data_ptr(), p[1].data_ptr(), p[2].data_ptr(), p[3].data_ptr(),
                                                    _dev(bias_table, torch.float32), _dev(wtab, torch.int32), T // 512, shift, q.stride(0), None,
                                                    o.t[0].data_ptr(), o.t[1].data_ptr(), o.t.stride(1), vp, _stream())
        _check(rc, "scp_swin_attention_packed_planes")
        return o
    out = torch.empty((T, 256), dtype=torch.float32, device=q.device)
    rc = lib().scp_swin_attention_packed_planes(q.data_ptr(), p[0].data_ptr(), p[1].data_ptr(), p[2].data_ptr(), p[3].data_ptr(),
                                                _dev(bias_table, torch.float32), _dev(wtab, torch.int32), T // 512, shift, q.stride(0), _dev(out), None,
                                                None, 0, vp, _stream())
    _check(rc, "scp_swin_attention_packed_planes")
    return out


def nn_sqdist(a, b):
    a = _dev_f64(a)
    b = _dev_f64(b)
    out = torch.empty((a.shape[0],), dtype=torch.float64, device=a.device)
    _check(lib().scp_nn_sqdist_f64(a.data_ptr(), a.shape[0], b.data_ptr(), b.shape[0], out.data_ptr(), _stream()), "scp_nn_sqdist_f64")
    return out


def _dev_f64(t):
    if not t.is_cuda:
        raise ScpError("device tensor required (there is no CPU path in the product)")
    return t.to(torch.float64).contiguous()


TIE_MEAN_NORMAL, TIE_PLANE_ERROR = 0, 1


def estimate_normals(xyz, radius=1.0, max_nn=30, view=(0.0, 0.0, 0.0), want_idx=False):
    x = _dev_f64(xyz)
    n = x.shape[0]
    normals = torch.empty((n, 3), dtype=torch.float64, device=x.device)
    count = torch.empty((n,), dtype=torch.int32, device=x.device)
    idx = torch.empty((n, int(max_nn)), dtype=torch.int32, device=x.device) if want_idx else None
    v = (C.c_double * 3)(*[float(c) for c in view])
    _check(lib().scp_estimate_normals_f64(x.data_ptr(), n, float(radius), int(max_nn), C.cast(v, _vp), normals.data_ptr(), count.data_ptr(),
                                          None if idx is None else idx.data_ptr(), _stream()), "scp_estimate_normals_f64")
    return normals, count, idx


def nn_tieset(mode, q, p, dmin, nrm):
    q, p, dmin, nrm = _dev_f64(q), _dev_f64(p), _dev_f64(dmin), _dev_f64(nrm)
    nq, np_ = q.shape[0], p.shape[0]
    if nrm.shape != (np_, 3) or dmin.shape != ((np_,) if mode == TIE_MEAN_NORMAL else (nq,)):
        raise ScpError(f"nn_tieset: dmin {tuple(dmin.shape)} / normals {tuple(nrm.shape)} do not fit {nq} queries against {np_} points")
    out = torch.empty((nq, 3) if mode == TIE_MEAN_NORMAL else (nq,), dtype=torch.float64, device=q.device)
    _check(lib().scp_nn_tieset_f64(int(mode), q.data_ptr(), nq, p.data_ptr(), np_, dmin.data_ptr(), nrm.data_ptr(), out.data_ptr(), _stream()),
           "scp_nn_tieset_f64")
    return out


def embed_gather(ctx, pos, inmap, occ_enc, level_enc, octant_enc):
    rows = inmap.shape[0]
    dev = ctx.device
    x = torch.empty((rows, 80), dtype=torch.float32, device=dev)
    p = torch.empty((rows, 3), dtype=torch.float32, device=dev)
    o = torch.empty((rows,), dtype=torch.int64, device=dev)
    _check(lib().scp_embed_gather(_dev(ctx, torch.uint8), _dev(pos, torch.float32), _dev(inmap, torch.int64), ctx.shape[0], _dev(occ_enc),
                                  _dev(level_enc), _dev(octant_enc), x.data_ptr(), p.data_ptr(), o.data_ptr(), rows, _stream()),
           "scp_embed_gather")
    return x, p, o


_POPC = {}


# ... 488 lines not shown
            pb = getattr(sw, "_bias_pad", None)
            ver = (bias._version, bias.data_ptr())
            if pb is None or pb[0] is not bias or pb[2] != ver:
                pb = (bias, torch.cat((bias.detach().float(), torch.zeros(Np - N, dtype=torch.float32, device=bias.device))).contiguous(), ver)
                sw._bias_pad = pb
                note_cache_fill()
            bias = pb[1]
        N = Np
    _check(lib().scp_linear_split_scatter(t[0].data_ptr(), t[1].data_ptr(), t.stride(1), sw.tiled()[0].data_ptr(), sw.tiled()[1].data_ptr(), sw.Npad, sw.Kpad,
                                          _opt(bias), _dev(out_map, torch.int64), table.data_ptr(), table.stride(0), a.M, N, sw.K, act, cfg,
                                          _stream()), "scp_linear_split_scatter")


def split_rows(x, idx=None, out=None):
    Cc = x.shape[1]
    rows = x.shape[0] if idx is None else idx.shape[0]
    if out is None:
        out = SplitAct.empty(rows, Cc, x.device)
    if x.stride(1) != 1:
        x = x.contiguous()
    t = out.t
    _check(lib().scp_split_rows(x.data_ptr(), x.stride(0), x.shape[0], _opt(idx), Cc, t[0].data_ptr(), t[1].data_ptr(), t.stride(1), rows,
                                _stream()), "scp_split_rows")
    return out


def linear_split(a, sw, bias=None, act=ACT_NONE, residual=None, out=None, out_split=None, want="f32", cfg=0, res_map=None, res_first=False):
    M, N, K = a.M, sw.N, sw.K
    if a.K != K:
        raise ScpError("linear_split: K mismatch %d vs %d" % (a.K, K))
    t = a.t
    c = o = None
    if want in ("f32", "both"):
        c = out if out is not None else torch.empty((M, N), dtype=torch.float32, device=t.device)
    if want in ("split", "both"):
        o = out_split if out_split is not None else SplitAct.empty(M, N, t.device)
    r2 = residual
    if res_map is not None or res_first:
        rc = lib().scp_linear_split_gather(t[0].data_ptr(), t[1].data_ptr(), t.stride(1), sw.tiled()[0].data_ptr(), sw.tiled()[1].data_ptr(), sw.Npad, sw.Kpad,
                                           _opt(bias), None if r2 is None else r2.data_ptr(), 0 if r2 is None else r2.stride(0),
                                           None if res_map is None else _dev(res_map, torch.int64),
                                           None if c is None else c.data_ptr(), 0 if c is None else c.stride(0),
                                           None if o is None else o.t[0].data_ptr(), None if o is None else o.t[1].data_ptr(),
                                           0 if o is None else o.t.stride(1), M, N, K, act, cfg, _stream())
        _check(rc, "scp_linear_split_gather")
        return c if want == "f32" else (o if want == "split" else (c, o))
    rc = lib().scp_linear_split(t[0].data_ptr(), t[1].data_ptr(), t.stride(1), sw.tiled()[0].data_ptr(), sw.tiled()[1].data_ptr(), sw.Npad, sw.Kpad, _opt(bias),
                                None if r2 is None else r2.data_ptr(), 0 if r2 is None else r2.stride(0),
                                None if c is None else c.data_ptr(), 0 if c is None else c.stride(0),
                                None if o is None else o.t[0].data_ptr(), None if o is None else o.t[1].data_ptr(),
                                0 if o is None else o.t.stride(1), M, N, K, act, cfg, _stream())
    _check(rc, "scp_linear_split")
    return c if want == "f32" else (o if want == "split" else (c, o))


def linear_split_hier2(a0, sw0, a1, sw1, parent, bias=None, act=ACT_NONE, residual=None, res_map=None, out_split=None):
    if not WTILE:
        raise ScpError("linear_split_hier2 reads tiled weight planes (SCP_WTILE=0 is not supported by it)")
    M, N = a0.M, sw0.N
    if a0.K != sw0.K or a1.K != sw1.K or sw1.K != 256 or sw1.N != N or sw1.Npad != sw0.Npad or parent.shape[0] != M:
        raise ScpError("linear_split_hier2: operand shapes do not match")
    o = out_split if out_split is not None else SplitAct.empty(M, N, a0.t.device)
    t0, t1 = a0.t, a1.t
    rc = lib().scp_linear_split_hier2(t0[0].data_ptr(), t0[1].data_ptr(), t0.stride(1), sw0.Kpad, t1[0].data_ptr(), t1[1].data_ptr(), t1.stride(1), a1.M,
                                      sw0.tiled()[0].data_ptr(), sw0.tiled()[1].data_ptr(), sw1.tiled()[0].data_ptr(), sw1.tiled()[1].data_ptr(), sw0.Npad,
                                      _dev(parent, torch.int64), _opt(bias), None if residual is None else residual.data_ptr(),
                                      0 if residual is None else residual.stride(0), None if (residual is None or res_map is None) else _dev(res_map, torch.int64),
                                      o.t[0].data_ptr(), o.t[1].data_ptr(), o.t.stride(1), M, N, act, _stream())
    _check(rc, "scp_linear_split_hier2")
    return o


class LnFoldedWeight:

    def __init__(self, w, gamma, beta):
        w64 = w.detach().double()
        self.sw = SplitWeight((w64 * gamma.detach().double()[None, :]).float())
        self.planes = _tiled_planes_always(self.sw)
        self.wbeta = (w64 @ beta.detach().double()).float().contiguous()
        self.N, self.K = self.sw.N, self.sw.K
        note_cache_fill()


def swin_ln_linear(x, fw, bias, eps=1e-5, valid=None, out=None):
    M = x.shape[0]
    if x.shape[1] != 256 or fw.K != 256 or x.stride(1) != 1:
        raise ScpError("swin_ln_linear: 256-channel rows expected")
    if out is None:
        out = torch.empty((M, fw.N), dtype=torch.float32, device=x.device)
    t = fw.planes
    rc = lib().scp_swin_ln_linear(x.data_ptr(), x.stride(0), None if valid is None else _dev(valid, torch.float32), t[0].data_ptr(), t[1].data_ptr(),
                                  _opt(bias), _dev(fw.wbeta), float(eps), out.data_ptr(), out.stride(0), M, fw.N, _stream())
    _check(rc, "scp_swin_ln_linear")
    return out


def swin_ln_qkv(x, fw, bias, eps=1e-5, valid=None):
    M = x.shape[0]
    if x.shape[1] != 256 or fw.K != 256 or x.stride(1) != 1 or fw.N not in (512, 768) or (M & 127):
        raise ScpError("swin_ln_qkv: 256-channel rows in multiples of 128, N = 768 or 512 expected")
    q = torch.empty((M, 256), dtype=torch.float32, device=x.device) if fw.N == 768 else None
    pl = torch.empty((4, M, 256), dtype=torch.bfloat16, device=x.device)
    t = fw.planes
    rc = lib().scp_swin_ln_qkv(x.data_ptr(), x.stride(0), None if valid is None else _dev(valid, torch.float32), t[0].data_ptr(), t[1].data_ptr(),
                               _opt(bias), _dev(fw.wbeta), float(eps), None if q is None else q.data_ptr(), 256, pl.data_ptr(), M, M, fw.N, _stream())
    _check(rc, "scp_swin_ln_qkv")
    return q, KvPlanes(t=pl)


class EdgeMlpWeights:

    def __init__(self, mlp1, mlp2):
        w11, w12, w13 = (mlp1[i].weight.detach().float() for i in (0, 2, 4))
        w21, w22, w23 = (mlp2[i].weight.detach().float() for i in (0, 2, 4))
        if tuple(w11.shape) != (256, 448) or tuple(w12.shape) != (256, 256) or tuple(w13.shape) != (256, 256) or tuple(w21.shape) != (256, 512) or \
                tuple(w22.shape) != (256, 256) or tuple(w23.shape) != (128, 256):
            raise ScpError("EdgeMlpWeights: unexpected layer shapes")
        dev = w11.device
        P = rc_perm16(256, dev)
        z = torch.zeros((256, 64), dtype=torch.float32, device=dev)
        mats = [w11[:, :256], torch.cat((w11[:, 256:], z), 1), w12[:, P], w13[:, P], w21[:, 256:][:, P], w21[:, :256], w22[:, P],
                torch.cat((w23[:, P], torch.zeros((128, 256), dtype=torch.float32, device=dev)), 0)]
        nbytes = lib().scp_swin_post_attn_weight_bytes()
        buf = torch.zeros((nbytes // 2,), dtype=torch.bfloat16, device=dev)
        half = nbytes // 4
        for m, w in enumerate(mats):
            hi, lo = _tiled_planes_always(SplitWeight(w.contiguous()))
            buf[m * 65536:(m + 1) * 65536] = hi.reshape(-1)[:65536]
            buf[half + m * 65536:half + (m + 1) * 65536] = lo.reshape(-1)[:65536]
        self.packed = buf
        self.bias = torch.cat([mlp1[i].bias.detach().float() for i in (0, 2, 4)] + [mlp2[i].bias.detach().float() for i in (0, 2, 4)]).contiguous()
        note_cache_fill()


def geo_edge_mlps(pos1, pos2, pos3, ew, out):
    M = pos1.shape[0]
    if pos1.shape[1] != 64 or pos2.shape[1] != 128 or pos3.shape[1] != 256 or pos1.stride(1) != 1 or pos2.stride(1) != 1 or pos3.stride(1) != 1 or out.stride(1) != 1:
        raise ScpError("geo_edge_mlps: [M, 64], [M, 128], [M, 256] rows expected")
    rc = lib().scp_geo_edge_mlps(pos1.data_ptr(), pos1.stride(0), pos2.data_ptr(), pos2.stride(0), pos3.data_ptr(), pos3.stride(0), ew.packed.data_ptr(),
                                 ew.bias.data_ptr(), out.data_ptr(), out.stride(0), M, _stream())
    _check(rc, "scp_geo_edge_mlps")
    return out


class Mlp3Weights:

    def __init__(self, seq):
        ws = [seq[i].weight.detach().float() for i in (0, 2, 4)]
        bs = [seq[i].bias.detach().float() for i in (0, 2, 4)]
        if ws[0].shape[1] != 256 or any(w.shape[0] > 256 or w.shape[1] > 256 for w in ws) or ws[1].shape[1] != ws[0].shape[0] or ws[2].shape[1] != ws[1].shape[0]:
            raise ScpError("Mlp3Weights: a 256 -> (<= 256) -> (<= 256) -> (<= 256) head expected")
        dev = ws[0].device
        P = rc_perm16(256, dev)
        nbytes = lib().scp_swin_post_attn_weight_bytes()
        buf = torch.zeros((nbytes // 2,), dtype=torch.bfloat16, device=dev)
        half = nbytes // 4
        bias = torch.zeros((3, 256), dtype=torch.float32, device=dev)
        for m, (w, b) in enumerate(zip(ws, bs)):
            full = torch.zeros((256, 256), dtype=torch.float32, device=dev)
            full[:w.shape[0], :w.shape[1]] = w
            if m:
                full = full[:, P]
            hi, lo = _tiled_planes_always(SplitWeight(full.contiguous()))
            buf[m * 65536:(m + 1) * 65536] = hi.reshape(-1)[:65536]
            buf[half + m * 65536:half + (m + 1) * 65536] = lo.reshape(-1)[:65536]
            bias[m, :b.shape[0]] = b
        self.packed, self.bias, self.N = buf, bias.reshape(-1).contiguous(), int(ws[2].shape[0])
        note_cache_fill()


def mlp3_rows(x, mw, out, in_map=None, out_map=None, ncols=None):
    M = x.shape[0] if in_map is None else in_map.shape[0]
    if out_map is not None and out_map.shape[0] != M:
        raise ScpError("mlp3_rows: out_map must have one entry per row")
    if x.shape[1] != 256 or x.stride(1) != 1 or out.stride(1) != 1:
        raise ScpError("mlp3_rows: [n, 256] rows with unit channel stride expected")
    N = -(-mw.N // 4) * 4 if ncols is None else int(ncols)
    if out_map is None and out.shape[0] < M:
        raise ScpError("mlp3_rows: output has too few rows")
    _check(lib().scp_mlp3_rows(x.data_ptr(), x.stride(0), x.shape[0], None if in_map is None else _dev(in_map, torch.int64), mw.packed.data_ptr(), mw.bias.data_ptr(),
                               out.data_ptr(), out.stride(0), None if out_map is None else _dev(out_map, torch.int64), M, N, _stream()), "scp_mlp3_rows")
    return out


class MergeWeights:

    def __init__(self, w, gamma, beta):
        w64 = w.detach().double()
        wf = (w64 * gamma.detach().double()[None, :]).float()
        self.wbeta = (w64 @ beta.detach().double()).float().contiguous()
        nbytes = lib().scp_swin_post_attn_weight_bytes()
        buf = torch.zeros((nbytes // 2,), dtype=torch.bfloat16, device=w.device)
        half = nbytes // 4
        for kh in range(2):
            hi, lo = _tiled_planes_always(SplitWeight(wf[:, 256 * kh:256 * (kh + 1)].contiguous()))
            buf[kh * 65536:(kh + 1) * 65536] = hi.reshape(-1)[:65536]
            buf[half + kh * 65536:half + (kh + 1) * 65536] = lo.reshape(-1)[:65536]
        self.packed = buf
        note_cache_fill()


def swin_merge(x, ia, ib, mw, eps=1e-5):
    M = ia.shape[0]
    if x.shape[1] != 256 or x.stride(1) != 1:
        raise ScpError("swin_merge: 256-channel rows expected")
    out = torch.empty((M, 256), dtype=torch.float32, device=x.device)
    rc = lib().scp_swin_merge(x.data_ptr(), x.stride(0), x.shape[0], _dev(ia, torch.int64), _dev(ib, torch.int64), mw.packed.data_ptr(), _dev(mw.wbeta),
                              float(eps), out.data_ptr(), out.stride(0), M, _stream())
    _check(rc, "scp_swin_merge")
    return out


def rc_perm16(n, device):
    p = torch.arange(n, device=device)
    q = p & 15
    return (p & ~15) | (q & 3) | ((q & 4) << 1) | ((q & 8) >> 1)


class PostAttnWeights:

    def __init__(self, wp, bp, gamma, beta, w1, b1, w2, b2):
        dev = wp.device
        perm_k, perm_h = rc_perm16(256, dev), rc_perm16(w1.shape[0], dev)
        w1d = w1.detach().double()
        s = float(lib().scp_gelu_prescale())
        swp = SplitWeight(wp.detach().float().contiguous())
        sw1 = SplitWeight((w1d * gamma.detach().double()[None, :] * s).float()[:, perm_k].contiguous())
        sw2 = SplitWeight((w2.detach().double() / s).float()[:, perm_h].contiguous())
        tiles = [_tiled_planes_always(w) for w in (swp, sw1, sw2)]
        self.packed = torch.cat([t[0].reshape(-1) for t in tiles] + [t[1].reshape(-1) for t in tiles]).contiguous()
        if self.packed.numel() * 2 != lib().scp_swin_post_attn_weight_bytes():
            raise ScpError("swin_post_attn: 256 -> 1024 -> 256 blocks only")
        self.bp = bp.detach().float().contiguous()
        self.b1 = ((b1.detach().double() + w1d @ beta.detach().double()) * s).float().contiguous()
        self.b2 = b2.detach().float().contiguous()
        note_cache_fill()


def swin_post_attn(o, x, pw, eps=1e-5, out=None, tiles=None):
    M = x.shape[0]
    if o.K != 256 or o.M != M or x.shape[1] != 256 or x.stride(1) != 1:
        raise ScpError("swin_post_attn: [M, 256] operands expected")
    if out is None:
        out = torch.empty((M, 256), dtype=torch.float32, device=x.device)
    t = o.t
    ldo = LDO_FRAG if isinstance(o, FragAct) else t.stride(1)
    rc = lib().scp_swin_post_attn(t[0].data_ptr(), t[1].data_ptr(), ldo, x.data_ptr(), x.stride(0), pw.packed.data_ptr(), _dev(pw.bp),
                                  _dev(pw.b1), _dev(pw.b2), float(eps), out.data_ptr(), out.stride(0), M,
                                  None if tiles is None else _dev(tiles, torch.int32), 0 if tiles is None else int(tiles.shape[0]), _stream())
    _check(rc, "scp_swin_post_attn")
    return out


def layernorm_rows(x, gamma, beta, eps=1e-5, valid=None, ia=None, ib=None, out=None, split=False):
    Cc = gamma.shape[0]
    rows = x.shape[0] if ia is None else ia.shape[0]
    if split:
        o = SplitAct.empty(rows, Cc, x.device)
        rc = lib().scp_layernorm_rows_split(x.data_ptr(), x.stride(0), x.shape[0], None if ia is None else _dev(ia, torch.int64),
                                            None if ib is None else _dev(ib, torch.int64), Cc, _dev(gamma), _dev(beta),
                                            None if valid is None else _dev(valid, torch.float32), float(eps), o.t[0].data_ptr(),
                                            o.t[1].data_ptr(), o.t.stride(1), rows, _stream())
        _check(rc, "scp_layernorm_rows_split")
        return o
    if out is None:
        out = torch.empty((rows, Cc), dtype=torch.float32, device=x.device)
    rc = lib().scp_layernorm_rows(x.data_ptr(), x.stride(0), x.shape[0], None if ia is None else _dev(ia, torch.int64),
                                  None if ib is None else _dev(ib, torch.int64), Cc, _dev(gamma), _dev(beta),
                                  None if valid is None else _dev(valid, torch.float32), float(eps), out.data_ptr(), out.stride(0),
                                  rows, _stream())
    _check(rc, "scp_layernorm_rows")
    return out


def layernorm_add(a, b, gamma, beta, eps=1e-5, planes=False):
    Cc = a.shape[-1]
    if not a.is_contiguous() or (b is not None and (not b.is_contiguous() or b.shape != a.shape)):
        raise ScpError("layernorm_add: contiguous operands of one shape expected")
    out = torch.empty_like(a)
    if planes:
        M, ld = a.numel() // Cc, -(-Cc // 32) * 32
        pl = torch.empty((2, M, ld), dtype=torch.float16, device=a.device)
        ws = torch.empty((2, M), dtype=torch.float32, device=a.device)
        _check(lib().scp_layernorm_add_split_f16(_dev(a, torch.float32), None if b is None else _dev(b, torch.float32), M, Cc, _dev(gamma), _dev(beta),
                                                 float(eps), out.data_ptr(), pl[0].data_ptr(), pl[1].data_ptr(), ld, ws[0].data_ptr(), ws[1].data_ptr(),
                                                 _stream()), "scp_layernorm_add_split_f16")
        return out, SplitActF16(parts=(pl[0], pl[1], ws[0], ws[1], Cc))
    _check(lib().scp_layernorm_add(_dev(a, torch.float32), None if b is None else _dev(b, torch.float32), a.numel() // Cc, Cc, _dev(gamma), _dev(beta),
                                   float(eps), out.data_ptr(), _stream()), "scp_layernorm_add")
    return out


def gather_rows(src, idx, out):
    Cc = out.shape[1]
    rc = lib().scp_gather_rows(src.data_ptr(), src.stride(0), _dev(idx, torch.int64), Cc, out.data_ptr(), out.stride(0), idx.shape[0],
                               _stream())
    _check(rc, "scp_gather_rows")
    return out


def linear_f32(x, w, bias=None, act=ACT_NONE):
    K = w.shape[1]
    N = w.shape[0]
    lead = x.shape[:-1]
    x2 = x.reshape(-1, K) if x.is_contiguous() else x.contiguous().reshape(-1, K)
    M = x2.shape[0]
    out = torch.empty((M, N), dtype=torch.float32, device=x.device)
    wc = w if w.is_contiguous() else w.contiguous()
    rc = lib().scp_linear_f32(x2.data_ptr(), x2.stride(0), _dev(wc.detach(), torch.float32), _opt(bias), out.data_ptr(), N, M, N, K, act,
                              _stream())
    _check(rc, "scp_linear_f32")
    return out.reshape(*lead, N)


OCTATTN_MODE = os.environ.get("SCP_OCTATTN", "f16x3")


def octattn_attention(q_u, k, k_u, v, v_u, heads, out=None, out_u=None, vmax=None):
    B, c, D = q_u.shape
    if out is None:
        out, out_u = torch.empty_like(q_u), torch.empty_like(q_u)
    elif not (out.is_contiguous() and out_u.is_contiguous() and out.shape == q_u.shape and out_u.shape == q_u.shape):
        raise ScpError("octattn_attention: out / out_u must be contiguous [B, c, D] float32")
    hd = D // heads
    ld = k.stride(-2)
    strided_ok = all(t.is_cuda and t.dtype == torch.float32 and t.stride(-1) == 1 and t.stride(-2) == ld and (t.dim() == 2 or t.stride(0) == c * ld)
                     for t in (k, k_u, v, v_u))
    if OCTATTN_MODE == "f16x3" and hd == 150 and (D & 3) == 0 and strided_ok:
        nb = lib().scp_octattn_f16x3_ws_bytes(B, c, heads)
        ws = torch.empty((nb + 1024,), dtype=torch.uint8, device=q_u.device)
        off = (-ws.data_ptr()) % 1024
# ... 850 lines not shown
```

Before: 16.06 frames/s.

## Pass Swin residual stream between blocks in fragment-ordered tiles

Adds a fragment-ordered layout for the fp32 residual stream, [tiles,32,128,8], that the post-attention kernel writes and the next block's LN+QKV/LN+linear kernels read directly. The LN-projection kernel body moves into a shared header and gains a second instantiation compiled for this layout. The aim is to remove uncoalesced row-strided loads and stores of the residual between consecutive Swin blocks within a stage. It adds new kernel variants, a mode switch on by default, and more code paths whose layout must match exactly.

```diff
diff --git a/include/scp.h b/include/scp.h
--- a/include/scp.h
+++ b/include/scp.h
@@ -385,6 +385,8 @@
                           const int64_t *out_map, int32_t M, int32_t N, void *stream);
 
 #define SCP_LDO_FRAG 0
+#define SCP_LDX_FRAG 0
+SCP_API int scp_swin_x_frag_ok(int32_t M, int32_t n_tiles);
 SCP_API int scp_swin_kv_planes(const float *k, const float *v, int64_t ldkv, int64_t rows, void *khi, void *klo, void *vthi, void *vtlo, void *stream);
 SCP_API int scp_swin_ln_qkv(const float *x, int64_t ldx, const float *valid, const void *Whi, const void *Wlo, const float *bias, const float *wbeta,
                             float eps, float *q, int64_t ldq, void *planes, int64_t Tp, int32_t M, int32_t N, void *stream);
diff --git a/scp_amd/build.py b/scp_amd/build.py
--- a/scp_amd/build.py
+++ b/scp_amd/build.py
@@ -6,7 +6,7 @@
 CSRC = os.path.join(HERE, "csrc")
 LIB = os.path.join(HERE, "libscp_hip.so")
 SOURCES = ["api.cpp", "geom.hip", "sort_u64.hip", "cdf.hip", "rangecoder.cpp", "legacy_octree.cpp",
-           "knn.hip", "edge.hip", "attn.hip", "octattn.hip", "octattn_f16.hip", "octattn_embed.hip", "octattn_rowinv.hip", "gemm.hip", "gemm_split.hip", "rowchain.hip", "lnlin2.hip", "fused.hip", "metrics.hip", "plan.hip", "normals.hip", "rate.hip", "distreport.hip", "ringrate.hip", "temper.hip", "ringlod.hip", "attr.hip", "color.hip", "ac_chunks.hip"]
+           "knn.hip", "edge.hip", "attn.hip", "octattn.hip", "octattn_f16.hip", "octattn_embed.hip", "octattn_rowinv.hip", "gemm.hip", "gemm_split.hip", "rowchain.hip", "lnlin2.hip", "lnlin2_xfrag.hip", "fused.hip", "metrics.hip", "plan.hip", "normals.hip", "rate.hip", "distreport.hip", "ringrate.hip", "temper.hip", "ringlod.hip", "attr.hip", "color.hip", "ac_chunks.hip"]
 HIPCC = os.environ.get("HIPCC", "/opt/rocm/bin/hipcc")
 FLAGS = ["-O3", "--offload-arch=gfx950", "-fPIC", "-std=c++17", "-Wall", "-Wno-unused-function",
          "-Wno-unused-result", "-fvisibility=hidden", "-x", "hip"]
@@ -23,6 +23,7 @@
 if os.environ.get("SCP_RC_DEFS"):
     EXTRA["rowchain.hip"] = os.environ["SCP_RC_DEFS"].split()
 EXTRA["lnlin2.hip"] = EXTRA.get("rowchain.hip", [])
+EXTRA["lnlin2_xfrag.hip"] = EXTRA["lnlin2.hip"]
 
 
 def _stale(target, deps):
diff --git a/scp_amd/csrc/lnlin2.hip b/scp_amd/csrc/lnlin2.hip
--- a/scp_amd/csrc/lnlin2.hip
+++ b/scp_amd/csrc/lnlin2.hip
@@ -1,255 +1,7 @@
-#include <stdlib.h>
-#include <type_traits>
-#include "rc_common.h"
-
-#define L2_Q 16384
-#define L2_OFF_BOUNCE (3 * L2_Q)
-#define L2_OFF_BIAS (L2_OFF_BOUNCE + 4 * RC_BOUNCE)
-#define L2_LDS (L2_OFF_BIAS + 8192)
-static_assert(L2_LDS <= 80 * 1024, "two workgroups per CU: at most half of the 160 KiB");
-#define L2_LDS_ONE (160 * 1024)
-
-__device__ __forceinline__ void l2_issue(const RcLane &L, __amdgpu_buffer_rsrc_t wr_hi, __amdgpu_buffer_rsrc_t wr_lo, int j, int qt, char *dst) {
-#pragma unroll
-    for (int i = 0; i < 4; ++i) {
-        const int b = i >> 1, plane = i & 1;
-        const int soff = ((2 * j + b) * 16 + (L.w >> 1) * 8 + qt * 2 + (L.w & 1)) * 1024;
-        __builtin_amdgcn_raw_ptr_buffer_load_lds(plane ? wr_lo : wr_hi, (rc_lds_ptr_t)(dst + (L.w + 4 * i) * 1024), 16, L.lane * 16, soff, 0, 0);
-    }
-}
-
-#define L2_READ4(d0, d1, d2, d3, addr, o0, o1, o2, o3)                                                                                  \
-    asm volatile("ds_read_b128 %0, %4 offset:%5\n\tds_read_b128 %1, %4 offset:%6\n\tds_read_b128 %2, %4 offset:%7\n\t"                      \
-                 "ds_read_b128 %3, %4 offset:%8\n\ts_waitcnt lgkmcnt(0)"                                                                  \
-                 : "=&v"(d0), "=&v"(d1), "=&v"(d2), "=&v"(d3) : "v"(addr), "n"(o0), "n"(o1), "n"(o2), "n"(o3) : "memory")
-#define L2_READ4_AHEAD(d0, d1, d2, d3, addr, o0, o1, o2, o3)                                                                            \
-    asm volatile("ds_read_b128 %0, %4 offset:%5\n\tds_read_b128 %1, %4 offset:%6\n\tds_read_b128 %2, %4 offset:%7\n\t"                      \
-                 "ds_read_b128 %3, %4 offset:%8"                                                                                         \
-                 : "=&v"(d0), "=&v"(d1), "=&v"(d2), "=&v"(d3) : "v"(addr), "n"(o0), "n"(o1), "n"(o2), "n"(o3) : "memory")
-#define L2_WAIT4(d0, d1, d2, d3) asm volatile("s_waitcnt lgkmcnt(0)" : "+v"(d0), "+v"(d1), "+v"(d2), "+v"(d3) :: "memory")
-#define L2_TOP(N) asm volatile("s_waitcnt vmcnt(" #N ") lgkmcnt(0)\n\ts_barrier" ::: "memory")
-
-template <bool SWAP, int Q>
-__device__ __forceinline__ void l2_quarter(unsigned ad0, unsigned ad1, rf32x16 &c0, rf32x16 &c1, const rbf16x8 (&Xh)[16], const rbf16x8 (&Xl)[16]) {
-#define L2_MFMA(c, wf, xf) c = SWAP ? __builtin_amdgcn_mfma_f32_32x32x16_bf16(xf, wf, c, 0, 0, 0) : __builtin_amdgcn_mfma_f32_32x32x16_bf16(wf, xf, c, 0, 0, 0)
-#define L2_FRAGS(M, A, ad, s) M(A[1], A[3], A[0], A[2], ad, 4096 + ((s) >> 1) * 1024, 12288 + ((s) >> 1) * 1024, ((s) >> 1) * 1024, 8192 + ((s) >> 1) * 1024)
-    rbf16x8 A[2][4];
-    L2_FRAGS(L2_READ4, A[0], ad0, 0);
-#pragma unroll
-    for (int s = 0; s < 4; ++s) {
-        const int k = 4 * Q + s, n = (s + 1) & 1;
-        if (s < 3) {
-            if (n) L2_FRAGS(L2_READ4_AHEAD, A[1], ad1, s + 1);
-            else L2_FRAGS(L2_READ4_AHEAD, A[0], ad0, s + 1);
-        }
-        __builtin_amdgcn_sched_barrier(0);
-        L2_MFMA(c0, A[s & 1][1], Xh[k]);
-        L2_MFMA(c1, A[s & 1][3], Xh[k]);
-        L2_MFMA(c0, A[s & 1][0], Xl[k]);
-        L2_MFMA(c1, A[s & 1][2], Xl[k]);
-        L2_MFMA(c0, A[s & 1][0], Xh[k]);
-        L2_MFMA(c1, A[s & 1][2], Xh[k]);
-        __builtin_amdgcn_sched_barrier(0);
-        if (s < 3) L2_WAIT4(A[n][0], A[n][1], A[n][2], A[n][3]);
-    }
-#undef L2_FRAGS
-#undef L2_MFMA
-}
-
-__device__ __forceinline__ unsigned l2_split_pair(float x0, float x1, int plane) {
-    const unsigned hh = rc_pack2(x0, x1);
-    return plane ? rc_pack2(x0 - __builtin_bit_cast(float, hh << 16), x1 - __builtin_bit_cast(float, hh & 0xffff0000u)) : hh;
-}
-
-__device__ __forceinline__ void l2_store_k(const RcLane &L, char *bounce, const rf32x16 &c0, const rf32x16 &c1, __amdgpu_buffer_rsrc_t prs, int kvoff,
-                                           int pbytes, int head) {
-    ri32x4 y[2][4];
-    int col = L.col;
-    asm volatile("" : "+v"(col));
-#pragma unroll
-    for (int plane = 0; plane < 2; ++plane) {
-#pragma unroll
-        for (int b = 0; b < 2; ++b)
-#pragma unroll
-            for (int q = 0; q < 4; ++q) {
-                const rf32x16 &c = b ? c1 : c0;
-                *(ru32x2 *)(bounce + col * 128 + (((4 * b + q) ^ (col & 7)) << 4) + 8 * L.h) =
-                    (ru32x2){l2_split_pair(c[4 * q], c[4 * q + 1], plane), l2_split_pair(c[4 * q + 2], c[4 * q + 3], plane)};
-            }
-#pragma unroll
-        for (int it = 0; it < 4; ++it) y[plane][it] = *(const ri32x4 *)(bounce + it * 1024 + L.lane * 16);
-    }
-#pragma unroll
-    for (int plane = 0; plane < 2; ++plane)
-#pragma unroll
-        for (int it = 0; it < 4; ++it)
-            __builtin_amdgcn_raw_buffer_store_b128(y[plane][it], prs, kvoff, it * 8 * 512 + head * 128 + plane * pbytes, 0);
-    asm volatile("s_waitcnt lgkmcnt(0)" ::: "memory");
-}
-
-__device__ __forceinline__ void l2_store_v(const RcLane &L, char *bounce, const rf32x16 &c0, const rf32x16 &c1, __amdgpu_buffer_rsrc_t prs, int vblk,
-                                           int pbytes, int head) {
-    ri32x4 y[2][4];
-    int col = L.col;
-    asm volatile("" : "+v"(col));
-#pragma unroll
-    for (int plane = 0; plane < 2; ++plane) {
-#pragma unroll
-        for (int b = 0; b < 2; ++b)
-#pragma unroll
-            for (int cc = 0; cc < 2; ++cc) {
-                const rf32x16 &c = b ? c1 : c0;
-                const int d = col + 32 * b, R = d >> 1, sl = (d & 1) * 4 + 2 * cc + L.h;
-                *(ru32x4 *)(bounce + R * 128 + ((sl ^ (R & 7)) << 4)) =
-                    (ru32x4){l2_split_pair(c[8 * cc], c[8 * cc + 1], plane), l2_split_pair(c[8 * cc + 2], c[8 * cc + 3], plane),
-                             l2_split_pair(c[8 * cc + 4], c[8 * cc + 5], plane), l2_split_pair(c[8 * cc + 6], c[8 * cc + 7], plane)};
-            }
-#pragma unroll
-        for (int it = 0; it < 4; ++it) y[plane][it] = *(const ri32x4 *)(bounce + it * 1024 + L.lane * 16);
-    }
-#pragma unroll
-    for (int plane = 0; plane < 2; ++plane)
-#pragma unroll
-        for (int it = 0; it < 4; ++it)
-            __builtin_amdgcn_raw_buffer_store_b128(y[plane][it], prs, L.lane * 16, it * 1024 + (vblk + head) * 4096 + (2 + plane) * pbytes, 0);
-    asm volatile("s_waitcnt lgkmcnt(0)" ::: "memory");
-}
+#include "lnlin2_kernel.h"
 
 template <bool KV>
-__global__ __launch_bounds__(256, 2) void ln2_proj_kernel(const RcLnLinArgs a) {
-    extern __shared__ __attribute__((aligned(1024))) char smem[];
-    const RcLane L = rc_lane();
-    const int ntiles = (a.M + RC_ROWS - 1) / RC_ROWS;
-    const int nsteps = a.N >> 6;
-    const int nq = KV ? a.nq : nsteps;
-    char *bounce = smem + L2_OFF_BOUNCE + L.w * RC_BOUNCE;
-    const unsigned ab = (unsigned)(uintptr_t)(rc_lds_ptr_t)smem + L.rg * 2048;
-    const unsigned af0 = ab + L.frag, af1 = ab + (L.frag ^ 32);
-    const unsigned asb = (unsigned)(uintptr_t)(rc_lds_ptr_t)(smem + L2_OFF_BIAS);
-    const int ldo_bytes = (int)(a.ldo * 4);
-    const int voff = (32 * L.w + (L.lane >> 3)) * ldo_bytes + (L.lane & 7) * 16;
-    const int pbytes = (int)a.plane_bytes;
-    const __amdgpu_buffer_rsrc_t prs = __builtin_amdgcn_make_buffer_rsrc((void *)a.planes, 0, (KV && !(a.probe & 1)) ? (int)(4 * a.plane_bytes) : 0, 0x00020000);
-    const bool dma = !(a.probe & 2);
-
-    const int wbytes = ((a.N + 255) & ~255) * 512;
-    const __amdgpu_buffer_rsrc_t wr_hi = __builtin_amdgcn_make_buffer_rsrc((void *)a.Whi, 0, wbytes, 0x00020000);
-    const __amdgpu_buffer_rsrc_t wr_lo = __builtin_amdgcn_make_buffer_rsrc((void *)a.Wlo, 0, wbytes, 0x00020000);
-
-    float *sb = (float *)(smem + L2_OFF_BIAS), *sbw = sb + 1024;
-    for (int i = threadIdx.x; i < a.N; i += 256) {
-        const float b = a.bias ? a.bias[i] : 0.f;
-        sb[i] = b; sbw[i] = b + (a.wbeta ? a.wbeta[i] : 0.f);
-    }
-    __syncthreads();
-    int slot = 0;
-    if (dma) { l2_issue(L, wr_hi, wr_lo, 0, 0, smem); l2_issue(L, wr_hi, wr_lo, 0, 1, smem + L2_Q); }
-    for (int tile = blockIdx.x; tile < ntiles; tile += (int)gridDim.x) {
-        const int m0 = tile * RC_ROWS;
-        const int row = m0 + 32 * L.w + L.col;
-        const int rowc = row < a.M ? row : a.M - 1;
-        float keep = (row < a.M) ? 1.0f : 0.0f;
-        if (a.valid) keep *= a.valid[rowc];
-        rbf16x8 Xh[16], Xl[16];
-        {
-            float v[128];
-            const float *src = a.x + (int64_t)((a.probe & 4) ? (rowc & 127) % a.M : rowc) * a.ldx + 8 * L.h;
-#pragma unroll
-            for (int s = 0; s < 16; ++s) {
-                const rf32x4 q0 = *(const rf32x4 *)(src + 16 * s), q1 = *(const rf32x4 *)(src + 16 * s + 4);
-#pragma unroll
-                for (int u = 0; u < 4; ++u) { v[8 * s + u] = q0[u]; v[8 * s + 4 + u] = q1[u]; }
-            }
-            float mean, rstd;
-            rc_ln_stats(v, a.eps, mean, rstd);
-            const float sc = rstd * keep;
-#pragma unroll
-            for (int s = 0; s < 16; ++s) {
-                float f[8];
-#pragma unroll
-                for (int i = 0; i < 8; ++i) f[i] = (v[8 * s + i] - mean) * sc;
-                rc_split8(f, Xh[s], Xl[s]);
-            }
-        }
-        const bool kept = keep != 0.f;
-        const int64_t rows_left = (int64_t)a.M - m0;
-        const int64_t span = (rows_left < RC_ROWS ? rows_left : RC_ROWS) * a.ldo * 4;
-        const __amdgpu_buffer_rsrc_t rs = __builtin_amdgcn_make_buffer_rsrc(a.out + (int64_t)m0 * a.ldo, 0, (a.probe & 1) ? 0 : (int)span, 0x00020000);
-        const unsigned kmask = (unsigned)__builtin_amdgcn_ballot_w64(kept);
-        const unsigned maskh = kmask >> (4 * L.h);
-        const int kvoff = (m0 + 32 * L.w + (L.lane >> 3)) * 512 + (L.lane & 7) * 16;
-        const int vblk = ((m0 >> 5) + L.w) * 4;
-
-        const unsigned atb = asb + (kept ? 4096 : 0) + 16 * L.h, atv = asb + 4 * L.col;
-        rf32x16 c0, c1;
-        auto bias_start = [&](int j) {
-            if (KV && j >= nq + 4) {
-                float bb[2], bwv[2];
-                const unsigned ad = atv + 256 * j;
-                asm volatile("ds_read_b32 %0, %4\n\tds_read_b32 %1, %4 offset:128\n\tds_read_b32 %2, %4 offset:4096\n\tds_read_b32 %3, %4 offset:4224\n\t"
-                             "s_waitcnt lgkmcnt(0)" : "=&v"(bb[0]), "=&v"(bb[1]), "=&v"(bwv[0]), "=&v"(bwv[1]) : "v"(ad) : "memory");
-#pragma unroll
-                for (int blk = 0; blk < 2; ++blk) {
-                    rf32x16 &c = blk ? c1 : c0;
-#pragma unroll
-                    for (int r = 0; r < 16; ++r) c[r] = ((maskh >> (8 * (r >> 2) + (r & 3))) & 1u) ? bwv[blk] : bb[blk];
-                }
-            } else {
-                const unsigned ad = atb + 256 * j;
-                rf32x4 t[2][4];
-                L2_READ4(t[0][0], t[0][1], t[0][2], t[0][3], ad, 0, 32, 64, 96);
-                L2_READ4(t[1][0], t[1][1], t[1][2], t[1][3], ad, 128, 160, 192, 224);
-#pragma unroll
-                for (int q = 0; q < 4; ++q)
-#pragma unroll
-                    for (int u = 0; u < 4; ++u) { c0[4 * q + u] = t[0][q][u]; c1[4 * q + u] = t[1][q][u]; }
-            }
-        };
-        bias_start(0);
-        SCP_WAIT_DMA(0);
-        auto steps = [&](auto sw, int ja, int jb) {
-        constexpr bool SW = decltype(sw)::value;
-        for (int j = ja; j < jb; ++j) {
-            const int jn = j + 1 < nsteps ? j + 1 : 0;
-#define L2_QUARTER(Q, N)                                                                                                                \
-            {                                                                                                                           \
-                L2_TOP(N);                                                                                                              \
-                const int sl2 = slot == 0 ? 2 : slot - 1;                    \
-                if (dma) l2_issue(L, wr_hi, wr_lo, Q < 2 ? j : jn, (Q + 2) & 3, smem + sl2 * L2_Q);                                       \
-                __builtin_amdgcn_sched_barrier(0);                                                                                      \
-                const unsigned a0 = af0 + slot * L2_Q, a1 = af1 + slot * L2_Q;                                                          \
-                l2_quarter<SW, Q>(a0, a1, c0, c1, Xh, Xl);                                                                              \
-                slot = slot == 2 ? 0 : slot + 1;                                                                                        \
-            }
-            L2_QUARTER(0, 12)
-            L2_QUARTER(1, 12)
-            L2_QUARTER(2, 4)
-            L2_QUARTER(3, 4)
-#undef L2_QUARTER
-            __builtin_amdgcn_sched_barrier(0);
-            if (!SW && j < nq) {
-#pragma unroll
-                for (int blk = 0; blk < 2; ++blk) {
-                    rf32x4 o[4];
-#pragma unroll
-                    for (int q = 0; q < 4; ++q)
-#pragma unroll
-                        for (int u = 0; u < 4; ++u) o[q][u] = (blk ? c1 : c0)[4 * q + u];
-                    rc_store_block(L, bounce, o, rs, ldo_bytes, voff, 64 * j + 32 * blk);
-                }
-            } else if (!SW) {
-                l2_store_k(L, bounce, c0, c1, prs, kvoff, pbytes, j - nq);
-            } else {
-                l2_store_v(L, bounce, c0, c1, prs, vblk, pbytes, j - nq - 4);
-            }
-            if (j + 1 < nsteps) bias_start(jn);
-        }
-        };
-        if (KV) { steps(std::false_type(), 0, nq + 4); steps(std::true_type(), nq + 4, nsteps); }
-        else steps(std::false_type(), 0, nsteps);
-    }
-    SCP_WAIT_DMA(0);
-}
+__global__ __launch_bounds__(256, 2) void ln2_proj_kernel(const RcLnLinArgs a) { ln2_proj_body<KV, false>(a); }
 
 int scp_lnlin2_mode() {
     static int mode = -1;
@@ -271,6 +23,7 @@
     const int ntiles = (a.M + RC_ROWS - 1) / RC_ROWS;
     const int wgs = (one ? 1 : 2) * ncu;
     const dim3 grid((unsigned)(ntiles < wgs ? ntiles : wgs));
+    if (a.ldx == SCP_LDX_FRAG) return scp_lnlin2_xfrag_launch(a, kv, grid, one ? L2_LDS_ONE : L2_LDS, stream);
     if (kv) hipLaunchKernelGGL(ln2_proj_kernel<true>, grid, dim3(256), one ? L2_LDS_ONE : L2_LDS, stream, a);
     else hipLaunchKernelGGL(ln2_proj_kernel<false>, grid, dim3(256), one ? L2_LDS_ONE : L2_LDS, stream, a);
     LAUNCH_CHECK();
diff --git a/scp_amd/csrc/lnlin2_kernel.h b/scp_amd/csrc/lnlin2_kernel.h
--- /dev/null
+++ b/scp_amd/csrc/lnlin2_kernel.h
@@ -0,0 +1,264 @@
+#pragma once
+#include <stdlib.h>
+#include <type_traits>
+#include "rc_common.h"
+
+#define L2_Q 16384
+#define L2_OFF_BOUNCE (3 * L2_Q)
+#define L2_OFF_BIAS (L2_OFF_BOUNCE + 4 * RC_BOUNCE)
+#define L2_LDS (L2_OFF_BIAS + 8192)
+static_assert(L2_LDS <= 80 * 1024, "two workgroups per CU: at most half of the 160 KiB");
+#define L2_LDS_ONE (160 * 1024)
+
+__device__ __forceinline__ void l2_issue(const RcLane &L, __amdgpu_buffer_rsrc_t wr_hi, __amdgpu_buffer_rsrc_t wr_lo, int j, int qt, char *dst) {
+#pragma unroll
+    for (int i = 0; i < 4; ++i) {
+        const int b = i >> 1, plane = i & 1;
+        const int soff = ((2 * j + b) * 16 + (L.w >> 1) * 8 + qt * 2 + (L.w & 1)) * 1024;
+        __builtin_amdgcn_raw_ptr_buffer_load_lds(plane ? wr_lo : wr_hi, (rc_lds_ptr_t)(dst + (L.w + 4 * i) * 1024), 16, L.lane * 16, soff, 0, 0);
+    }
+}
+
+#define L2_READ4(d0, d1, d2, d3, addr, o0, o1, o2, o3)                                                                                  \
+    asm volatile("ds_read_b128 %0, %4 offset:%5\n\tds_read_b128 %1, %4 offset:%6\n\tds_read_b128 %2, %4 offset:%7\n\t"                      \
+                 "ds_read_b128 %3, %4 offset:%8\n\ts_waitcnt lgkmcnt(0)"                                                                  \
+                 : "=&v"(d0), "=&v"(d1), "=&v"(d2), "=&v"(d3) : "v"(addr), "n"(o0), "n"(o1), "n"(o2), "n"(o3) : "memory")
+#define L2_READ4_AHEAD(d0, d1, d2, d3, addr, o0, o1, o2, o3)                                                                            \
+    asm volatile("ds_read_b128 %0, %4 offset:%5\n\tds_read_b128 %1, %4 offset:%6\n\tds_read_b128 %2, %4 offset:%7\n\t"                      \
+                 "ds_read_b128 %3, %4 offset:%8"                                                                                         \
+                 : "=&v"(d0), "=&v"(d1), "=&v"(d2), "=&v"(d3) : "v"(addr), "n"(o0), "n"(o1), "n"(o2), "n"(o3) : "memory")
+#define L2_WAIT4(d0, d1, d2, d3) asm volatile("s_waitcnt lgkmcnt(0)" : "+v"(d0), "+v"(d1), "+v"(d2), "+v"(d3) :: "memory")
+#define L2_TOP(N) asm volatile("s_waitcnt vmcnt(" #N ") lgkmcnt(0)\n\ts_barrier" ::: "memory")
+
+template <bool SWAP, int Q>
+__device__ __forceinline__ void l2_quarter(unsigned ad0, unsigned ad1, rf32x16 &c0, rf32x16 &c1, const rbf16x8 (&Xh)[16], const rbf16x8 (&Xl)[16]) {
+#define L2_MFMA(c, wf, xf) c = SWAP ? __builtin_amdgcn_mfma_f32_32x32x16_bf16(xf, wf, c, 0, 0, 0) : __builtin_amdgcn_mfma_f32_32x32x16_bf16(wf, xf, c, 0, 0, 0)
+#define L2_FRAGS(M, A, ad, s) M(A[1], A[3], A[0], A[2], ad, 4096 + ((s) >> 1) * 1024, 12288 + ((s) >> 1) * 1024, ((s) >> 1) * 1024, 8192 + ((s) >> 1) * 1024)
+    rbf16x8 A[2][4];
+    L2_FRAGS(L2_READ4, A[0], ad0, 0);
+#pragma unroll
+    for (int s = 0; s < 4; ++s) {
+        const int k = 4 * Q + s, n = (s + 1) & 1;
+        if (s < 3) {
+            if (n) L2_FRAGS(L2_READ4_AHEAD, A[1], ad1, s + 1);
+            else L2_FRAGS(L2_READ4_AHEAD, A[0], ad0, s + 1);
+        }
+        __builtin_amdgcn_sched_barrier(0);
+        L2_MFMA(c0, A[s & 1][1], Xh[k]);
+        L2_MFMA(c1, A[s & 1][3], Xh[k]);
+        L2_MFMA(c0, A[s & 1][0], Xl[k]);
+        L2_MFMA(c1, A[s & 1][2], Xl[k]);
+        L2_MFMA(c0, A[s & 1][0], Xh[k]);
+        L2_MFMA(c1, A[s & 1][2], Xh[k]);
+        __builtin_amdgcn_sched_barrier(0);
+        if (s < 3) L2_WAIT4(A[n][0], A[n][1], A[n][2], A[n][3]);
+    }
+#undef L2_FRAGS
+#undef L2_MFMA
+}
+
+__device__ __forceinline__ unsigned l2_split_pair(float x0, float x1, int plane) {
+    const unsigned hh = rc_pack2(x0, x1);
+    return plane ? rc_pack2(x0 - __builtin_bit_cast(float, hh << 16), x1 - __builtin_bit_cast(float, hh & 0xffff0000u)) : hh;
+}
+
+__device__ __forceinline__ void l2_store_k(const RcLane &L, char *bounce, const rf32x16 &c0, const rf32x16 &c1, __amdgpu_buffer_rsrc_t prs, int kvoff,
+                                           int pbytes, int head) {
+    ri32x4 y[2][4];
+    int col = L.col;
+    asm volatile("" : "+v"(col));
+#pragma unroll
+    for (int plane = 0; plane < 2; ++plane) {
+#pragma unroll
+        for (int b = 0; b < 2; ++b)
+#pragma unroll
+            for (int q = 0; q < 4; ++q) {
+                const rf32x16 &c = b ? c1 : c0;
+                *(ru32x2 *)(bounce + col * 128 + (((4 * b + q) ^ (col & 7)) << 4) + 8 * L.h) =
+                    (ru32x2){l2_split_pair(c[4 * q], c[4 * q + 1], plane), l2_split_pair(c[4 * q + 2], c[4 * q + 3], plane)};
+            }
+#pragma unroll
+        for (int it = 0; it < 4; ++it) y[plane][it] = *(const ri32x4 *)(bounce + it * 1024 + L.lane * 16);
+    }
+#pragma unroll
+    for (int plane = 0; plane < 2; ++plane)
+#pragma unroll
+        for (int it = 0; it < 4; ++it)
+            __builtin_amdgcn_raw_buffer_store_b128(y[plane][it], prs, kvoff, it * 8 * 512 + head * 128 + plane * pbytes, 0);
+    asm volatile("s_waitcnt lgkmcnt(0)" ::: "memory");
+}
+
+__device__ __forceinline__ void l2_store_v(const RcLane &L, char *bounce, const rf32x16 &c0, const rf32x16 &c1, __amdgpu_buffer_rsrc_t prs, int vblk,
+                                           int pbytes, int head) {
+    ri32x4 y[2][4];
+    int col = L.col;
+    asm volatile("" : "+v"(col));
+#pragma unroll
+    for (int plane = 0; plane < 2; ++plane) {
+#pragma unroll
+        for (int b = 0; b < 2; ++b)
+#pragma unroll
+            for (int cc = 0; cc < 2; ++cc) {
+                const rf32x16 &c = b ? c1 : c0;
+                const int d = col + 32 * b, R = d >> 1, sl = (d & 1) * 4 + 2 * cc + L.h;
+                *(ru32x4 *)(bounce + R * 128 + ((sl ^ (R & 7)) << 4)) =
+                    (ru32x4){l2_split_pair(c[8 * cc], c[8 * cc + 1], plane), l2_split_pair(c[8 * cc + 2], c[8 * cc + 3], plane),
+                             l2_split_pair(c[8 * cc + 4], c[8 * cc + 5], plane), l2_split_pair(c[8 * cc + 6], c[8 * cc + 7], plane)};
+            }
+#pragma unroll
+        for (int it = 0; it < 4; ++it) y[plane][it] = *(const ri32x4 *)(bounce + it * 1024 + L.lane * 16);
+    }
+#pragma unroll
+    for (int plane = 0; plane < 2; ++plane)
+#pragma unroll
+        for (int it = 0; it < 4; ++it)
+            __builtin_amdgcn_raw_buffer_store_b128(y[plane][it], prs, L.lane * 16, it * 1024 + (vblk + head) * 4096 + (2 + plane) * pbytes, 0);
+    asm volatile("s_waitcnt lgkmcnt(0)" ::: "memory");
+}
+
+template <bool KV, bool XF>
+__device__ __forceinline__ void ln2_proj_body(const RcLnLinArgs &a) {
+    extern __shared__ __attribute__((aligned(1024))) char smem[];
+    const RcLane L = rc_lane();
+    const int ntiles = (a.M + RC_ROWS - 1) / RC_ROWS;
+    const int nsteps = a.N >> 6;
+    const int nq = KV ? a.nq : nsteps;
+    char *bounce = smem + L2_OFF_BOUNCE + L.w * RC_BOUNCE;
+    const unsigned ab = (unsigned)(uintptr_t)(rc_lds_ptr_t)smem + L.rg * 2048;
+    const unsigned af0 = ab + L.frag, af1 = ab + (L.frag ^ 32);
+    const unsigned asb = (unsigned)(uintptr_t)(rc_lds_ptr_t)(smem + L2_OFF_BIAS);
+    const int ldo_bytes = (int)(a.ldo * 4);
+    const int voff = (32 * L.w + (L.lane >> 3)) * ldo_bytes + (L.lane & 7) * 16;
+    const int pbytes = (int)a.plane_bytes;
+    const __amdgpu_buffer_rsrc_t prs = __builtin_amdgcn_make_buffer_rsrc((void *)a.planes, 0, (KV && !(a.probe & 1)) ? (int)(4 * a.plane_bytes) : 0, 0x00020000);
+    const bool dma = !(a.probe & 2);
+
+    const int wbytes = ((a.N + 255) & ~255) * 512;
+    const __amdgpu_buffer_rsrc_t wr_hi = __builtin_amdgcn_make_buffer_rsrc((void *)a.Whi, 0, wbytes, 0x00020000);
+    const __amdgpu_buffer_rsrc_t wr_lo = __builtin_amdgcn_make_buffer_rsrc((void *)a.Wlo, 0, wbytes, 0x00020000);
+
+    float *sb = (float *)(smem + L2_OFF_BIAS), *sbw = sb + 1024;
+    for (int i = threadIdx.x; i < a.N; i += 256) {
+        const float b = a.bias ? a.bias[i] : 0.f;
+        sb[i] = b; sbw[i] = b + (a.wbeta ? a.wbeta[i] : 0.f);
+    }
+    __syncthreads();
+    int slot = 0;
+    if (dma) { l2_issue(L, wr_hi, wr_lo, 0, 0, smem); l2_issue(L, wr_hi, wr_lo, 0, 1, smem + L2_Q); }
+    for (int tile = blockIdx.x; tile < ntiles; tile += (int)gridDim.x) {
+        const int m0 = tile * RC_ROWS;
+        const int row = m0 + 32 * L.w + L.col;
+        const int rowc = row < a.M ? row : a.M - 1;
+        float keep = (row < a.M) ? 1.0f : 0.0f;
+        if (a.valid) keep *= a.valid[rowc];
+        rbf16x8 Xh[16], Xl[16];
+        {
+            float v[128];
+            if (XF) {
+                const __amdgpu_buffer_rsrc_t xr = rc_x_tile_rsrc(a.x, (a.probe & 4) ? 0 : tile, RC_XTILE_BYTES);
+                const int xv = rc_x_lane_off(rowc, 0) + 4096 * L.h;
+#pragma unroll
+                for (int s = 0; s < 16; ++s) {
+                    const rf32x4 q0 = rc_x_load(xr, xv, 2 * s), q1 = rc_x_load(xr, xv + 16, 2 * s);
+#pragma unroll
+                    for (int u = 0; u < 4; ++u) { v[8 * s + u] = q0[u]; v[8 * s + 4 + u] = q1[u]; }
+                }
+            } else {
+            const float *src = a.x + (int64_t)((a.probe & 4) ? (rowc & 127) % a.M : rowc) * a.ldx + 8 * L.h;
+#pragma unroll
+            for (int s = 0; s < 16; ++s) {
+                const rf32x4 q0 = *(const rf32x4 *)(src + 16 * s), q1 = *(const rf32x4 *)(src + 16 * s + 4);
+#pragma unroll
+                for (int u = 0; u < 4; ++u) { v[8 * s + u] = q0[u]; v[8 * s + 4 + u] = q1[u]; }
+            }
+            }
+            float mean, rstd;
+            rc_ln_stats(v, a.eps, mean, rstd);
+            const float sc = rstd * keep;
+#pragma unroll
+            for (int s = 0; s < 16; ++s) {
+                float f[8];
+#pragma unroll
+                for (int i = 0; i < 8; ++i) f[i] = (v[8 * s + i] - mean) * sc;
+                rc_split8(f, Xh[s], Xl[s]);
+            }
+        }
+        const bool kept = keep != 0.f;
+        const int64_t rows_left = (int64_t)a.M - m0;
+        const int64_t span = (rows_left < RC_ROWS ? rows_left : RC_ROWS) * a.ldo * 4;
+        const __amdgpu_buffer_rsrc_t rs = __builtin_amdgcn_make_buffer_rsrc(a.out + (int64_t)m0 * a.ldo, 0, (a.probe & 1) ? 0 : (int)span, 0x00020000);
+        const unsigned kmask = (unsigned)__builtin_amdgcn_ballot_w64(kept);
+        const unsigned maskh = kmask >> (4 * L.h);
+        const int kvoff = (m0 + 32 * L.w + (L.lane >> 3)) * 512 + (L.lane & 7) * 16;
+        const int vblk = ((m0 >> 5) + L.w) * 4;
+
+        const unsigned atb = asb + (kept ? 4096 : 0) + 16 * L.h, atv = asb + 4 * L.col;
+        rf32x16 c0, c1;
+        auto bias_start = [&](int j) {
+            if (KV && j >= nq + 4) {
+                float bb[2], bwv[2];
+                const unsigned ad = atv + 256 * j;
+                asm volatile("ds_read_b32 %0, %4\n\tds_read_b32 %1, %4 offset:128\n\tds_read_b32 %2, %4 offset:4096\n\tds_read_b32 %3, %4 offset:4224\n\t"
+                             "s_waitcnt lgkmcnt(0)" : "=&v"(bb[0]), "=&v"(bb[1]), "=&v"(bwv[0]), "=&v"(bwv[1]) : "v"(ad) : "memory");
+#pragma unroll
+                for (int blk = 0; blk < 2; ++blk) {
+                    rf32x16 &c = blk ? c1 : c0;
+#pragma unroll
+                    for (int r = 0; r < 16; ++r) c[r] = ((maskh >> (8 * (r >> 2) + (r & 3))) & 1u) ? bwv[blk] : bb[blk];
+                }
+            } else {
+                const unsigned ad = atb + 256 * j;
+                rf32x4 t[2][4];
+                L2_READ4(t[0][0], t[0][1], t[0][2], t[0][3], ad, 0, 32, 64, 96);
+                L2_READ4(t[1][0], t[1][1], t[1][2], t[1][3], ad, 128, 160, 192, 224);
+#pragma unroll
+                for (int q = 0; q < 4; ++q)
+#pragma unroll
+                    for (int u = 0; u < 4; ++u) { c0[4 * q + u] = t[0][q][u]; c1[4 * q + u] = t[1][q][u]; }
+            }
+        };
+        bias_start(0);
+        SCP_WAIT_DMA(0);
+        auto steps = [&](auto sw, int ja, int jb) {
+        constexpr bool SW = decltype(sw)::value;
+        for (int j = ja; j < jb; ++j) {
+            const int jn = j + 1 < nsteps ? j + 1 : 0;
+#define L2_QUARTER(Q, N)                                                                                                                \
+            {                                                                                                                           \
+                L2_TOP(N);                                                                                                              \
+                const int sl2 = slot == 0 ? 2 : slot - 1;                    \
+                if (dma) l2_issue(L, wr_hi, wr_lo, Q < 2 ? j : jn, (Q + 2) & 3, smem + sl2 * L2_Q);                                       \
+                __builtin_amdgcn_sched_barrier(0);                                                                                      \
+                const unsigned a0 = af0 + slot * L2_Q, a1 = af1 + slot * L2_Q;                                                          \
+                l2_quarter<SW, Q>(a0, a1, c0, c1, Xh, Xl);                                                                              \
+                slot = slot == 2 ? 0 : slot + 1;                                                                                        \
+            }
+            L2_QUARTER(0, 12)
+            L2_QUARTER(1, 12)
+            L2_QUARTER(2, 4)
+            L2_QUARTER(3, 4)
+#undef L2_QUARTER
+            __builtin_amdgcn_sched_barrier(0);
+            if (!SW && j < nq) {
+#pragma unroll
+                for (int blk = 0; blk < 2; ++blk) {
+                    rf32x4 o[4];
+#pragma unroll
+                    for (int q = 0; q < 4; ++q)
+#pragma unroll
+                        for (int u = 0; u < 4; ++u) o[q][u] = (blk ? c1 : c0)[4 * q + u];
+                    rc_store_block(L, bounce, o, rs, ldo_bytes, voff, 64 * j + 32 * blk);
+                }
+            } else if (!SW) {
+                l2_store_k(L, bounce, c0, c1, prs, kvoff, pbytes, j - nq);
+            } else {
+                l2_store_v(L, bounce, c0, c1, prs, vblk, pbytes, j - nq - 4);
+            }
+            if (j + 1 < nsteps) bias_start(jn);
+        }
+        };
+        if (KV) { steps(std::false_type(), 0, nq + 4); steps(std::true_type(), nq + 4, nsteps); }
+        else steps(std::false_type(), 0, nsteps);
+    }
+    SCP_WAIT_DMA(0);
+}
diff --git a/scp_amd/csrc/lnlin2_xfrag.hip b/scp_amd/csrc/lnlin2_xfrag.hip
--- /dev/null
+++ b/scp_amd/csrc/lnlin2_xfrag.hip
@@ -0,0 +1,17 @@
+#include "lnlin2_kernel.h"
+
+template <bool KV>
+__global__ __launch_bounds__(256, 2) void ln2_proj_xfrag_kernel(const RcLnLinArgs a) { ln2_proj_body<KV, true>(a); }
+
+int scp_lnlin2_xfrag_launch(RcLnLinArgs a, bool kv, dim3 grid, int lds, hipStream_t stream) {
+    static int configured = 0;
+    if (configured != lds) {
+        HIP_TRY(hipFuncSetAttribute((const void *)ln2_proj_xfrag_kernel<false>, hipFuncAttributeMaxDynamicSharedMemorySize, lds));
+        HIP_TRY(hipFuncSetAttribute((const void *)ln2_proj_xfrag_kernel<true>, hipFuncAttributeMaxDynamicSharedMemorySize, lds));
+        configured = lds;
+    }
+    if (kv) hipLaunchKernelGGL(ln2_proj_xfrag_kernel<true>, grid, dim3(256), lds, stream, a);
+    else hipLaunchKernelGGL(ln2_proj_xfrag_kernel<false>, grid, dim3(256), lds, stream, a);
+    LAUNCH_CHECK();
+    return SCP_OK;
+}
diff --git a/scp_amd/csrc/rc_common.h b/scp_amd/csrc/rc_common.h
--- a/scp_amd/csrc/rc_common.h
+++ b/scp_amd/csrc/rc_common.h
@@ -69,6 +69,18 @@
     asm volatile("s_waitcnt lgkmcnt(0)" ::: "memory");
 }
 
+#define RC_XTILE_BYTES (RC_ROWS * 1024)
+__device__ __forceinline__ __amdgpu_buffer_rsrc_t rc_x_tile_rsrc(const float *x, int tile, int bytes) {
+    return __builtin_amdgcn_make_buffer_rsrc((void *)(x + (int64_t)tile * (RC_ROWS * 256)), 0, bytes, 0x00020000);
+}
+__device__ __forceinline__ int rc_x_lane_off(int row, int h) { return (row & (RC_ROWS - 1)) * 32 + 16 * h; }
+__device__ __forceinline__ rf32x4 rc_x_load(__amdgpu_buffer_rsrc_t r, int voff, int chunk) {
+    return __builtin_bit_cast(rf32x4, __builtin_amdgcn_raw_buffer_load_b128(r, voff, 4096 * chunk, 0));
+}
+__device__ __forceinline__ void rc_x_store(__amdgpu_buffer_rsrc_t r, int voff, int chunk, rf32x4 v) {
+    __builtin_amdgcn_raw_buffer_store_b128(__builtin_bit_cast(ri32x4, v), r, voff, 4096 * chunk, 0);
+}
+
 __device__ __forceinline__ void rc_ln_stats(const float *v , float eps, float &mean, float &rstd) {
     float s = 0.f;
 #pragma unroll
@@ -98,3 +110,4 @@
 
 int scp_lnlin2_mode();
 int scp_lnlin2_launch(RcLnLinArgs a, bool kv, int ncu, hipStream_t stream);
+int scp_lnlin2_xfrag_launch(RcLnLinArgs a, bool kv, dim3 grid, int lds, hipStream_t stream);
diff --git a/scp_amd/csrc/rowchain.hip b/scp_amd/csrc/rowchain.hip
--- a/scp_amd/csrc/rowchain.hip
+++ b/scp_amd/csrc/rowchain.hip
@@ -604,7 +604,7 @@
     for (int s = 0; s < 16; ++s) Bl[s] = __builtin_bit_cast(rbf16x8, __builtin_amdgcn_raw_buffer_load_b128(rl, v, 4096 * s, 0));
 }
 
-template <bool OFRAG>
+template <bool OFRAG, bool XFI, bool XFO>
 __global__ __launch_bounds__(256, 1) void rc_post_attn_kernel(const RcPostArgs a) {
     extern __shared__ __attribute__((aligned(1024))) char smem[];
     const RcLane L = rc_lane();
@@ -697,12 +697,16 @@
         rf32x16 Y[8];
         const int xrow = m0 + 32 * L.w + (L.lane >> 3);
         const float *xsrc = a.x + (L.lane & 7) * 4;
+        const __amdgpu_buffer_rsrc_t xr = rc_x_tile_rsrc(a.x, XFI ? tile : 0, XFI ? RC_XTILE_BYTES : 0);
+        const int xlast = a.M - 1 - m0;
+        const int xv = rc_x_lane_off(32 * L.w + L.col < xlast ? 32 * L.w + L.col : xlast, L.h);
         for (int j = 0; j < 4; ++j) {
             rf32x4 xc[2][4];
 #pragma unroll
             for (int b = 0; b < 2; ++b)
 #pragma unroll
                 for (int it = 0; it < 4; ++it) {
+                    if (XFI) { xc[b][it] = rc_x_load(xr, xv, 8 * j + 4 * b + it); continue; }
                     const int r = xrow + 8 * it;
                     xc[b][it] = *(const rf32x4 *)(xsrc + (int64_t)(r < a.M ? r : a.M - 1) * a.ldx + 64 * j + 32 * b);
                 }
@@ -713,15 +717,17 @@
             ++gstep;
 #pragma unroll
             for (int b = 0; b < 2; ++b) {
-#pragma unroll
-                for (int it = 0; it < 4; ++it) {
-                    const int rho = 8 * it + (L.lane >> 3), kap = L.lane & 7;
-                    *(rf32x4 *)(bounce + rho * 128 + ((kap ^ (rho & 7)) << 4)) = xc[b][it];
+                if (!XFI) {
+#pragma unroll
+                    for (int it = 0; it < 4; ++it) {
+                        const int rho = 8 * it + (L.lane >> 3), kap = L.lane & 7;
+                        *(rf32x4 *)(bounce + rho * 128 + ((kap ^ (rho & 7)) << 4)) = xc[b][it];
+                    }
+                    asm volatile("s_waitcnt lgkmcnt(0)" ::: "memory");
                 }
-                asm volatile("s_waitcnt lgkmcnt(0)" ::: "memory");
 #pragma unroll
                 for (int q = 0; q < 4; ++q) {
-                    const rf32x4 xq = *(const rf32x4 *)(bounce + L.col * 128 + (((2 * q + L.h) ^ (L.col & 7)) << 4));
+                    const rf32x4 xq = XFI ? xc[b][q] : *(const rf32x4 *)(bounce + L.col * 128 + (((2 * q + L.h) ^ (L.col & 7)) << 4));
                     const rf32x4 bq = *(const rf32x4 *)(sbp + 64 * j + 32 * b + 8 * q + 4 * L.h);
 #pragma unroll
                     for (int u = 0; u < 4; ++u) {
@@ -738,6 +744,10 @@
             case 2: Y[4] = c0; Y[5] = c1; break;
             default: Y[6] = c0; Y[7] = c1; break;
             }
+        }
+        if (XFI) {
+#pragma unroll
+            for (int b = 0; b < 8; ++b) asm volatile("" : "+v"(Y[b]));
         }
         stamp(t_p0);
         float sum = 0.f;
@@ -836,6 +846,16 @@
 #else
         const __amdgpu_buffer_rsrc_t rs = __builtin_amdgcn_make_buffer_rsrc(a.out + (int64_t)m0 * a.ldc, 0, (int)span, 0x00020000);
 #endif
+#ifdef RC_EPI_NOSTORE
+        const __amdgpu_buffer_rsrc_t xs = rc_x_tile_rsrc(a.out, 0, 0);
+#else
+        const __amdgpu_buffer_rsrc_t xs = rc_x_tile_rsrc(a.out, XFO ? tile : 0, XFO ? RC_XTILE_BYTES : 0);
+#endif
+        const int xsv = rc_x_lane_off(32 * L.w + L.col, L.h);
+        if (XFO || XFI) {
+#pragma unroll
+            for (int b = 0; b < 8; ++b) asm volatile("" : "+v"(Y[b]));
+        }
 #pragma unroll
         for (int b = 0; b < 8; ++b) {
             rf32x4 o[4];
@@ -843,7 +863,10 @@
             for (int q = 0; q < 4; ++q)
 #pragma unroll
                 for (int u = 0; u < 4; ++u) o[q][u] = Y[b][4 * q + u];
-            rc_store_block(L, bounce, o, rs, ldc_bytes, voff, 32 * b);
+            if (XFO) {
+#pragma unroll
+                for (int q = 0; q < 4; ++q) rc_x_store(xs, xsv, 4 * b + q, o[q]);
+            } else rc_store_block(L, bounce, o, rs, ldc_bytes, voff, 32 * b);
         }
         transpose_o();
         stamp(t_epi);
@@ -1511,11 +1534,25 @@
     return mode == 2 || (mode == 0 && 4 * (int64_t)ntiles >= 3 * (int64_t)ncu);
 }
 
+static int rc_dump_mode() { const char *e = getenv("SCP_RC_DUMP"); return e ? atoi(e) : 0; }
+static bool rc_post_wide_here(int ntiles, int ncu, int dbg_mode) {
+    return rc_wide_mode() == 1 || (rc_wide_mode() < 0 && !g_rc_dbg && !dbg_mode && 4 * (int64_t)ntiles <= (int64_t)ncu);
+}
+
+extern "C" SCP_API int scp_swin_x_frag_ok(int32_t M, int32_t n_tiles) {
+    if (M <= 0 || n_tiles < 0) return 0;
+    const int all = (M + RC_ROWS - 1) / RC_ROWS, ncu = rc_num_cu();
+    if (n_tiles > all) return 0;
+    return !rc_post_wide_here(n_tiles ? n_tiles : all, ncu, rc_dump_mode()) && rc_lnlin2_here(all, ncu) ? 1 : 0;
+}
+
 extern "C" SCP_API int scp_swin_ln_linear(const float *x, int64_t ldx, const float *valid, const void *Whi, const void *Wlo, const float *bias,
                                           const float *wbeta, float eps, float *out, int64_t ldo, int32_t M, int32_t N, void *stream) {
-    if (!x || !Whi || !Wlo || !out || M <= 0 || N <= 0 || (N & 127) || N > 1024 || ldx < 256 || (ldx & 3) || ldo < N || (ldo & 3) ||
+    const bool xf = ldx == SCP_LDX_FRAG;
+    if (!x || !Whi || !Wlo || !out || M <= 0 || N <= 0 || (N & 127) || N > 1024 || (!xf && (ldx < 256 || (ldx & 3))) || ldo < N || (ldo & 3) ||
         (((uintptr_t)x | (uintptr_t)out | (uintptr_t)Whi | (uintptr_t)Wlo) & 15) || (int64_t)RC_ROWS * ldo * 4 > 0x7fffffffLL)
         return SCP_EINVAL;
+    if (xf && !rc_lnlin2_here((M + RC_ROWS - 1) / RC_ROWS, rc_num_cu())) return SCP_EINVAL;
     static bool configured = false;
     if (!configured) {
         HIP_TRY(hipFuncSetAttribute((const void *)rc_ln_linear_kernel<0>, hipFuncAttributeMaxDynamicSharedMemorySize, RC_LDS));
@@ -1540,8 +1577,10 @@
 
 extern "C" SCP_API int scp_swin_ln_qkv(const float *x, int64_t ldx, const float *valid, const void *Whi, const void *Wlo, const float *bias,
                                        const float *wbeta, float eps, float *q, int64_t ldq, void *planes, int64_t Tp, int32_t M, int32_t N, void *stream) {
-    if (!x || !Whi || !Wlo || !planes || M <= 0 || (M & 127) || (N != 768 && N != 512) || (N == 768 && (!q || ldq < 256 || (ldq & 3))) || ldx < 256 ||
-        (ldx & 3) || Tp < M || (Tp & 31) || (((uintptr_t)x | (uintptr_t)q | (uintptr_t)Whi | (uintptr_t)Wlo | (uintptr_t)planes) & 15) ||
+    const bool xf = ldx == SCP_LDX_FRAG;
+    if (xf && (M <= 0 || !rc_lnlin2_here((M + RC_ROWS - 1) / RC_ROWS, rc_num_cu()))) return SCP_EINVAL;
+    if (!x || !Whi || !Wlo || !planes || M <= 0 || (M & 127) || (N != 768 && N != 512) || (N == 768 && (!q || ldq < 256 || (ldq & 3))) || (!xf && (ldx < 256 ||
+        (ldx & 3))) || Tp < M || (Tp & 31) || (((uintptr_t)x | (uintptr_t)q | (uintptr_t)Whi | (uintptr_t)Wlo | (uintptr_t)planes) & 15) ||
         (q && (int64_t)RC_ROWS * ldq * 4 > 0x7fffffffLL) || 4 * Tp * 512 > 0x7fffffffLL)
         return SCP_EINVAL;
     static bool configured = false;
@@ -1565,14 +1604,21 @@
 extern "C" SCP_API int scp_swin_post_attn(const void *Ohi, const void *Olo, int64_t ldo_in, const float *x, int64_t ldx, const void *W, const float *bp,
                                           const float *b1, const float *b2, float eps, float *out, int64_t ldc, int32_t M, const int32_t *tile_list,
                                           int32_t n_tiles, void *stream) {
-    if (!Ohi || !Olo || !x || !W || !bp || !b1 || !b2 || !out || M <= 0 || (tile_list && (n_tiles <= 0 || n_tiles > (M + RC_ROWS - 1) / RC_ROWS)) || (ldo_in != SCP_LDO_FRAG && (ldo_in < 256 || (ldo_in & 7))) || ldx < 256 || (ldx & 3) || ldc < 256 ||
-        (ldc & 3) || (((uintptr_t)Ohi | (uintptr_t)Olo | (uintptr_t)x | (uintptr_t)out | (uintptr_t)W) & 15) ||
+    const bool xfi = ldx == SCP_LDX_FRAG, xfo = ldc == SCP_LDX_FRAG;
+    if (!Ohi || !Olo || !x || !W || !bp || !b1 || !b2 || !out || M <= 0 || (tile_list && (n_tiles <= 0 || n_tiles > (M + RC_ROWS - 1) / RC_ROWS)) || (ldo_in != SCP_LDO_FRAG && (ldo_in < 256 || (ldo_in & 7))) ||
+        (!xfi && (ldx < 256 || (ldx & 3))) || (!xfo && (ldc < 256 || (ldc & 3))) || (((uintptr_t)Ohi | (uintptr_t)Olo | (uintptr_t)x | (uintptr_t)out | (uintptr_t)W) & 15) ||
         (int64_t)RC_ROWS * ldc * 4 > 0x7fffffffLL)
         return SCP_EINVAL;
+    if ((xfi || xfo) && (ldo_in != SCP_LDO_FRAG || rc_post_wide_here(tile_list ? n_tiles : (M + RC_ROWS - 1) / RC_ROWS, rc_num_cu(), rc_dump_mode()))) return SCP_EINVAL;
+    if (out == x && xfi != xfo && (xfi ? ldc : ldx) != 256) return SCP_EINVAL;
+    if (xfo && tile_list && out != x) return SCP_EINVAL;
     static bool configured = false;
     if (!configured) {
-        HIP_TRY(hipFuncSetAttribute((const void *)rc_post_attn_kernel<true>, hipFuncAttributeMaxDynamicSharedMemorySize, RC_LDS));
-        HIP_TRY(hipFuncSetAttribute((const void *)rc_post_attn_kernel<false>, hipFuncAttributeMaxDynamicSharedMemorySize, RC_LDS));
+        HIP_TRY(hipFuncSetAttribute((const void *)rc_post_attn_kernel<true, false, false>, hipFuncAttributeMaxDynamicSharedMemorySize, RC_LDS));
+        HIP_TRY(hipFuncSetAttribute((const void *)rc_post_attn_kernel<true, false, true>, hipFuncAttributeMaxDynamicSharedMemorySize, RC_LDS));
+        HIP_TRY(hipFuncSetAttribute((const void *)rc_post_attn_kernel<true, true, false>, hipFuncAttributeMaxDynamicSharedMemorySize, RC_LDS));
+        HIP_TRY(hipFuncSetAttribute((const void *)rc_post_attn_kernel<true, true, true>, hipFuncAttributeMaxDynamicSharedMemorySize, RC_LDS));
+        HIP_TRY(hipFuncSetAttribute((const void *)rc_post_attn_kernel<false, false, false>, hipFuncAttributeMaxDynamicSharedMemorySize, RC_LDS));
         HIP_TRY(hipFuncSetAttribute((const void *)rc_post_attn_wide_kernel<true>, hipFuncAttributeMaxDynamicSharedMemorySize, RC_LDS));
         HIP_TRY(hipFuncSetAttribute((const void *)rc_post_attn_wide_kernel<false>, hipFuncAttributeMaxDynamicSharedMemorySize, RC_LDS));
         configured = true;
@@ -1581,21 +1627,25 @@
     a.Ohi = (const __bf16 *)Ohi; a.Olo = (const __bf16 *)Olo; a.ldo_in = ldo_in; a.x = x; a.ldx = ldx; a.W = W;
     a.bp = bp; a.b1 = b1; a.b2 = b2; a.out = out; a.ldc = ldc; a.M = M; a.eps = eps;
     a.dbg = g_rc_dbg;
-    { const char *e = getenv("SCP_RC_DUMP"); a.dbg_mode = e ? atoi(e) : 0; }
+    a.dbg_mode = rc_dump_mode();
     a.tile_list = tile_list; a.n_list = tile_list ? n_tiles : 0;
     const bool frag = ldo_in == SCP_LDO_FRAG;
     const int ntiles = tile_list ? n_tiles : (M + RC_ROWS - 1) / RC_ROWS;
     const int ncu = rc_num_cu();
     SCP_PROF(SCP_PROF_POST_ATTN, stream, 2.0 * (tile_list ? (double)n_tiles * RC_ROWS : (double)M) * (256.0 * 256.0 + 2.0 * 256.0 * 1024.0));
-    if (rc_wide_mode() == 1 || (rc_wide_mode() < 0 && !g_rc_dbg && !a.dbg_mode && 4 * (int64_t)ntiles <= (int64_t)ncu)) {
+    if (rc_post_wide_here(ntiles, ncu, a.dbg_mode)) {
         const int items = 4 * ntiles;
         if (frag) hipLaunchKernelGGL(rc_post_attn_wide_kernel<true>, dim3((unsigned)(items < 2 * ncu ? items : 2 * ncu)), dim3(256), RC_LDS, (hipStream_t)stream, a);
         else hipLaunchKernelGGL(rc_post_attn_wide_kernel<false>, dim3((unsigned)(items < 2 * ncu ? items : 2 * ncu)), dim3(256), RC_LDS, (hipStream_t)stream, a);
         LAUNCH_CHECK();
         return SCP_OK;
     }
-    if (frag) hipLaunchKernelGGL(rc_post_attn_kernel<true>, dim3((unsigned)(ntiles < ncu ? ntiles : ncu)), dim3(256), RC_LDS, (hipStream_t)stream, a);
-    else hipLaunchKernelGGL(rc_post_attn_kernel<false>, dim3((unsigned)(ntiles < ncu ? ntiles : ncu)), dim3(256), RC_LDS, (hipStream_t)stream, a);
+    const dim3 grid((unsigned)(ntiles < ncu ? ntiles : ncu));
+    if (!frag) hipLaunchKernelGGL((rc_post_attn_kernel<false, false, false>), grid, dim3(256), RC_LDS, (hipStream_t)stream, a);
+    else if (xfi && xfo) hipLaunchKernelGGL((rc_post_attn_kernel<true, true, true>), grid, dim3(256), RC_LDS, (hipStream_t)stream, a);
+    else if (xfi) hipLaunchKernelGGL((rc_post_attn_kernel<true, true, false>), grid, dim3(256), RC_LDS, (hipStream_t)stream, a);
+    else if (xfo) hipLaunchKernelGGL((rc_post_attn_kernel<true, false, true>), grid, dim3(256), RC_LDS, (hipStream_t)stream, a);
+    else hipLaunchKernelGGL((rc_post_attn_kernel<true, false, false>), grid, dim3(256), RC_LDS, (hipStream_t)stream, a);
     LAUNCH_CHECK();
     return SCP_OK;
 }
diff --git a/scp_amd/models/packed.py b/scp_amd/models/packed.py
--- a/scp_amd/models/packed.py
+++ b/scp_amd/models/packed.py
@@ -142,7 +142,7 @@
     return out
 
 
-def _swin_layer_rowchain(layer, x, valid, wtab, shift, query=None, tiles=None, q_pre=None):
+def _swin_layer_rowchain(layer, x, valid, wtab, shift, query=None, tiles=None, q_pre=None, frag_out=False):
     cross = query is not None
     w, table, qbias, eps_b, eps_a = _block_consts(layer, cross)
     v1 = None if valid is None else valid.reshape(-1)
@@ -153,9 +153,13 @@
             q = q_pre if q_pre is not None else native.swin_ln_linear(query, w["q"], qbias, eps_b, v1)
             _, kvp = native.swin_ln_qkv(x, w["kv"], w["b"], eps_b, v1)
         o = native.swin_attention_packed_planes(q, kvp, table, wtab, shift, split=native.attn_o_split(), valid=v1 if tiles is not None else None)
+        frag_in = isinstance(x, native.FragRows)
         if tiles is not None and tiles.shape[0] > 0:
-            return native.swin_post_attn(o, x, w["post"], eps_a, out=x, tiles=tiles)
-        return native.swin_post_attn(o, x, w["post"], eps_a)
+            out = x if frag_in == frag_out else (native.FragRows.of(x) if frag_out else x.rows_view())
+            return native.swin_post_attn(o, x, w["post"], eps_a, out=out, tiles=tiles)
+        return native.swin_post_attn(o, x, w["post"], eps_a, out="frag" if frag_out else None)
+    if frag_out or isinstance(x, native.FragRows):
+        raise native.ScpError("the fragment-ordered residual stream belongs to the bf16x3 attention profile")
     att, lnb = layer.attention.self, layer.layernorm_before
     if not cross:
         qkv = native.swin_ln_linear(x, w["kv"], w["b"], lnb.eps, v1)
@@ -168,11 +172,11 @@
     return native.swin_post_attn(o, x, w["post"], layer.layernorm_after.eps)
 
 
-def _swin_layer(layer, x, valid, wtab, shift, query=None, tiles=None, q_pre=None):
+def _swin_layer(layer, x, valid, wtab, shift, query=None, tiles=None, q_pre=None, frag_out=False):
     fc1, fc2 = layer.intermediate.dense, layer.output.dense
     if x.shape[1] != 256 or fc1.weight.shape != (1024, 256) or fc2.weight.shape != (256, 1024):
         raise native.ScpError("EHEM's Swin blocks are 256 wide with a 1024-wide MLP (configs/model/ehem.yaml); other widths are not built")
-    return _swin_layer_rowchain(layer, x, valid, wtab, shift, query, tiles, q_pre)
+    return _swin_layer_rowchain(layer, x, valid, wtab, shift, query, tiles, q_pre, frag_out)
 
 
 def _merge(m, x, maps):
@@ -187,9 +191,14 @@
 def _encoder(enc, x, valids, tabs, merges, query=None, tiles=None, q_pre=None):
     hs = [x]
     for s, stage in enumerate(enc.layers):
+        ts = None if tiles is None else tiles[s]
+        nb = len(stage.blocks)
+        in_place = ts is not None and ts.shape[0] > 0
+        frag = (nb > 1 and native.attention_bf16x3() and native.swin_x_frag(x.shape[0], ts.shape[0] if in_place else 0)
+                and (not in_place or (x.is_contiguous() and x.shape[0] % 128 == 0)))
         for b, blk in enumerate(stage.blocks):
-            x = _swin_layer(blk, x, valids[s], tabs[s], SHIFT if b % 2 else 0, query, None if tiles is None else tiles[s],
-                            None if q_pre is None else q_pre[s][b])
+            x = _swin_layer(blk, x, valids[s], tabs[s], SHIFT if b % 2 else 0, query, ts, None if q_pre is None else q_pre[s][b],
+                            frag_out=frag and b < nb - 1)
         hs.append(x)
         if s < len(enc.layers) - 1:
             x = _merge(stage.downsample, x, merges[s])
diff --git a/scp_amd/native.py b/scp_amd/native.py
--- a/scp_amd/native.py
+++ b/scp_amd/native.py
@@ -88,6 +88,7 @@
         "scp_ctx_make_current": (C.c_int, [_vp]),
         "scp_rc_debug_buffer": (C.c_int, [_vp]),
         "scp_rc_set_wide": (C.c_int, [i32]),
+        "scp_swin_x_frag_ok": (C.c_int, [i32, i32]),
         "scp_prof_enable": (C.c_int, [i32]),
         "scp_prof_count": (C.c_int, []),
         "scp_prof_read": (C.c_int, [i32, _vp, _vp, _vp]),
@@ -485,6 +486,68 @@
         return self.rows().float()
 
 
+_SWIN_X = "rows" if os.environ.get("SCP_SWIN_X", "")[:1] == "r" else "frag"
+LDX_FRAG = 0
+
+
+def set_swin_x(mode):
+    global _SWIN_X
+    if mode not in ("frag", "rows"):
+        raise ScpError("residual stream hand-over: 'frag' or 'rows'")
+    prev, _SWIN_X = _SWIN_X, mode
+    return prev
+
+
+def swin_x_frag_ok(M, n_tiles=0):
+    return bool(lib().scp_swin_x_frag_ok(int(M), int(n_tiles)))
+
+
+def swin_x_frag(M, n_tiles=0):
+    return _SWIN_X == "frag" and _ATTN_O == "frag" and swin_x_frag_ok(M, n_tiles)
+
+
+class FragRows:
+
+    __slots__ = ("t", "M")
+
+    def __init__(self, t, M):
+        self.t, self.M = t, M
+
+    @property
+    def shape(self):
+        return (self.M, 256)
+
+    @property
+    def device(self):
+        return self.t.device
+
+    @staticmethod
+    def empty(M, device):
+        return FragRows(torch.empty((-(-M // 128), 32, 128, 8), dtype=torch.float32, device=device), M)
+
+    @staticmethod
+    def from_rows(x):
+        M = x.shape[0]
+        nt = -(-M // 128)
+        r = torch.zeros((nt * 128, 256), dtype=torch.float32, device=x.device)
+        r[:M] = x[:, :256]
+        return FragRows(r.view(nt, 128, 32, 8).permute(0, 2, 1, 3).contiguous(), M)
+
+    def to_rows(self):
+        nt = self.t.shape[0]
+        return self.t.permute(0, 2, 1, 3).reshape(nt * 128, 256)[:self.M].contiguous()
+
+    @staticmethod
+    def of(x):
+        M = x.shape[0]
+        if x.dtype != torch.float32 or x.dim() != 2 or x.shape[1] != 256 or not x.is_contiguous() or (M & 127):
+            raise ScpError("FragRows.of: compact fp32 [M, 256] rows in whole 128-row tiles expected")
+        return FragRows(x.view(M // 128, 32, 128, 8), M)
+
+    def rows_view(self):
+        return self.t.view(-1, 256)[:self.M]
+
+
 def swin_attention_packed_planes(q, kv, bias_table, wtab, shift, split=False, valid=None):
     T = q.shape[0]
     p = kv.t
@@ -1139,14 +1202,25 @@
         note_cache_fill()
 
 
+def _x_arg(x, what):
+    if isinstance(x, FragRows):
+        if x.t.numel() != -(-x.M // 128) * 128 * 256:
+            raise ScpError(what + ": a FragRows spans ceil(M / 128) whole tiles")
+        return _dev(x.t, torch.float32), LDX_FRAG
+    if x.shape[1] != 256 or x.stride(1) != 1:
+        raise ScpError(what + ": [M, 256] operands expected" if what == "swin_post_attn" else what + ": 256-channel rows expected")
+    return x.data_ptr(), x.stride(0)
+
+
 def swin_ln_linear(x, fw, bias, eps=1e-5, valid=None, out=None):
     M = x.shape[0]
-    if x.shape[1] != 256 or fw.K != 256 or x.stride(1) != 1:
+    xp, ldx = _x_arg(x, "swin_ln_linear")
+    if fw.K != 256:
         raise ScpError("swin_ln_linear: 256-channel rows expected")
     if out is None:
         out = torch.empty((M, fw.N), dtype=torch.float32, device=x.device)
     t = fw.planes
-    rc = lib().scp_swin_ln_linear(x.data_ptr(), x.stride(0), None if valid is None else _dev(valid, torch.float32), t[0].data_ptr(), t[1].data_ptr(),
+    rc = lib().scp_swin_ln_linear(xp, ldx, None if valid is None else _dev(valid, torch.float32), t[0].data_ptr(), t[1].data_ptr(),
                                   _opt(bias), _dev(fw.wbeta), float(eps), out.data_ptr(), out.stride(0), M, fw.N, _stream())
     _check(rc, "scp_swin_ln_linear")
     return out
@@ -1154,12 +1228,13 @@
 
 def swin_ln_qkv(x, fw, bias, eps=1e-5, valid=None):
     M = x.shape[0]
-    if x.shape[1] != 256 or fw.K != 256 or x.stride(1) != 1 or fw.N not in (512, 768) or (M & 127):
+    if (not isinstance(x, FragRows) and (x.shape[1] != 256 or x.stride(1) != 1)) or fw.K != 256 or fw.N not in (512, 768) or (M & 127):
         raise ScpError("swin_ln_qkv: 256-channel rows in multiples of 128, N = 768 or 512 expected")
+    xp, ldx = _x_arg(x, "swin_ln_qkv")
     q = torch.empty((M, 256), dtype=torch.float32, device=x.device) if fw.N == 768 else None
     pl = torch.empty((4, M, 256), dtype=torch.bfloat16, device=x.device)
     t = fw.planes
-    rc = lib().scp_swin_ln_qkv(x.data_ptr(), x.stride(0), None if valid is None else _dev(valid, torch.float32), t[0].data_ptr(), t[1].data_ptr(),
+    rc = lib().scp_swin_ln_qkv(xp, ldx, None if valid is None else _dev(valid, torch.float32), t[0].data_ptr(), t[1].data_ptr(),
                                _opt(bias), _dev(fw.wbeta), float(eps), None if q is None else q.data_ptr(), 256, pl.data_ptr(), M, M, fw.N, _stream())
     _check(rc, "scp_swin_ln_qkv")
     return q, KvPlanes(t=pl)
@@ -1296,14 +1371,22 @@
 
 def swin_post_attn(o, x, pw, eps=1e-5, out=None, tiles=None):
     M = x.shape[0]
-    if o.K != 256 or o.M != M or x.shape[1] != 256 or x.stride(1) != 1:
+    if o.K != 256 or o.M != M:
         raise ScpError("swin_post_attn: [M, 256] operands expected")
+    xp, ldx = _x_arg(x, "swin_post_attn")
     if out is None:
         out = torch.empty((M, 256), dtype=torch.float32, device=x.device)
+    elif isinstance(out, str):
+        if out != "frag":
+            raise ScpError("swin_post_attn: out is a tensor, a FragRows or 'frag'")
+        out = FragRows.empty(M, x.device)
+    if out.shape[0] != M:
+        raise ScpError("swin_post_attn: [M, 256] operands expected")
+    cp, ldc = _x_arg(out, "swin_post_attn")
     t = o.t
     ldo = LDO_FRAG if isinstance(o, FragAct) else t.stride(1)
-    rc = lib().scp_swin_post_attn(t[0].data_ptr(), t[1].data_ptr(), ldo, x.data_ptr(), x.stride(0), pw.packed.data_ptr(), _dev(pw.bp),
-                                  _dev(pw.b1), _dev(pw.b2), float(eps), out.data_ptr(), out.stride(0), M,
+    rc = lib().scp_swin_post_attn(t[0].data_ptr(), t[1].data_ptr(), ldo, xp, ldx, pw.packed.data_ptr(), _dev(pw.bp),
+                                  _dev(pw.b1), _dev(pw.b2), float(eps), cp, ldc, M,
                                   None if tiles is None else _dev(tiles, torch.int32), 0 if tiles is None else int(tiles.shape[0]), _stream())
     _check(rc, "scp_swin_post_attn")
     return out
```

New measurement: 16.06 frames/s (median of 2 runs). Within noise of the previous version (+0.0%).
